# artiom-matvei/RLAO

Hardware: NVIDIA B200
Metric: closed-loop AO env-steps/sec (batched envs) (higher is better)
Workload: dtype f32

## Files before the change

### include/aoenv.h

```cpp
#ifndef AOENV_H_
#define AOENV_H_

#include <stdint.h>

#ifdef __cplusplus
extern "C" {
#endif

#define AOENV_MAX_LAYERS 8
#define AOENV_ABI_VERSION 1

int aoenv_abi_version(void);
const char* aoenv_last_error(void);
uint64_t aoenv_launch_count(void);
int aoenv_set_pdl(int enabled);


int aoenv_atm_gather(const float* win, int B, int M, int pitch, int64_t env_stride, int sx, int sy,
                     const int32_t* inner_rc, int nI, int nO, const float* xi,
                     uint64_t seed, uint64_t stream_id, float* zx, int ldz, void* zx_planes, int parts, void* stream);

int aoenv_atm_ring(float* win, int B, int M, int pitch, int64_t env_stride, int64_t win_offset, int nO, const float* X,
                   int ldx, uint64_t* ext, int32_t* flag, int force_rescan, void* stream);

int aoenv_atm_gather_multi(const void* const* wins, const int32_t* sx, const int32_t* sy, const uint64_t* seeds,
                           const uint64_t* stream_ids, int G, int B, int M, int pitch, int64_t env_stride,
                           const int32_t* inner_rc, int nI, int nO, const float* xi, float* zx, int ldz,
                           void* zx_planes, int parts, void* stream);
int aoenv_atm_ring_multi(void* const* wins, const int64_t* win_offsets, void* const* exts, int G, int B, int M,
                         int pitch, int64_t env_stride, int nO, const float* X, int ldx, int32_t* flag,
                         int force_rescan, void* stream);

int aoenv_atm_compact(const float* src_win, float* dst_win, int B, int M, int pitch, int64_t env_stride, uint64_t* ext,
                      int64_t pos_delta, void* stream);

int aoenv_vk_screens(uint64_t seed, uint32_t screen0, int S, int N, const float* amp, const float* inject, const void* wa_planes,
                     const void* wb_planes, int Kp, int parts, const float* sh_ex, const float* sh_ey, const float* h_amp,
                     const float* h_mx, const float* h_my, void* work_planes, float* work_a, int lda, float* work_b, int ldb,
                     float* dst, int pitch, int64_t env_stride, void* stream);

int aoenv_atm_phase(const float* const* h_canvas, const uint64_t* const* h_ext, const int32_t* h_org, int nLayer, int B,
                    int R, int M, int Mc, int pitch, int fp_off, const int32_t* h_row_off, const int32_t* h_col_off,
                    const float* h_wrow, const float* h_wcol, const float* h_weight, float opd_scale, float* opd_out,
                    void* stream);

typedef struct {
  double ratio[2];
  double buff[2];
  double vX, vY;
  uint64_t events;
  uint64_t philox_seed;
  int32_t not_done_once;
  int32_t cur;
  int32_t org[2];
} aoenv_layer_state_t;

typedef struct {
  int32_t nLayer, B, R, M, Mc, pitch, S, nI, nO, ldz, ldx, group_max, parts, fp_off, warp_kernel, use_tc;
  int64_t env_stride;
  uint64_t env_offset;
  double sampling_time, ps_loop;
  float opd_scale, reserved;
  float weight[AOENV_MAX_LAYERS];
  void* maps[AOENV_MAX_LAYERS][2];
  void* ext[AOENV_MAX_LAYERS];
  const void* inner_rc;
  void* zx;
  void* zx_planes;
  void* X;
  void* flag;
  const void* w_f32;
  aoenv_layer_state_t layer[AOENV_MAX_LAYERS];
} aoenv_atm_state_t;

int aoenv_atm_update(aoenv_atm_state_t* state, const void* w_planes, float* opd_out, void* stream);

#define AOENV_SKINNY_MAX_ROWS 8
int aoenv_gemm_tn(const float* X, int ldx, const float* W, int ldw, float* D, int ldd,
                  int M, int N, int K, float alpha, void* stream);

int aoenv_split_bf16(const float* src, int lds, int rows, int K, int parts, void* dst, int ldk, void* stream);
int aoenv_gemm_tn_tc(const void* Xs, const void* Ws, int ldk, int parts, float* D, int ldd, int MX, int NW, int K,
                     float alpha, void* stream);

int aoenv_dm_surface_separable(const float* coefs, int ldc, const int32_t* act_pos, int nA, int nAct, const float* gx,
                               const float* gy, const int32_t* band_x, const int32_t* band_y, const float* wx,
                               const int32_t* j0x, const float* wyp, const int32_t* i0y, int W, int B, int R, float* opd,
                               void* stream);

typedef struct {
  int32_t photon_noise;
  int32_t sensor_emccd;
  int32_t has_fwc;
  int32_t bits;
  float qe;
  float dark_electrons;
  float fwc;
  float gain;
  float readout_noise;
  uint32_t reserved;
  uint64_t seed;
  uint64_t frame_counter;
} aoenv_detector_t;

int aoenv_detector_integrate(float* frame, int B, int rows, int cols, const aoenv_detector_t* det, void* stream);

int aoenv_shwfs_camera(float* frame, const uint8_t* valid, int B, int nS, int n, const aoenv_detector_t* det, int shared_max,
                       int32_t* envmax, void* stream);

int aoenv_set_wfs6_variant(int variant);

int aoenv_shwfs_frame(const float* opd_a, const float* opd_b, const float* pupil, const float* amp,
                      const uint8_t* valid, int B, int nS, int n, float phase_scale,
                      const aoenv_detector_t* det, int shared_max,
                      float* frame, int32_t* envmax, double* stats, void* stream);

int aoenv_shwfs_slopes(const float* frame, const int32_t* envmax, int shared_max, const int32_t* valid_idx,
                       int nV, const float* ref_xy, float inv_units, float threshold_cog, int B, int nS, int n,
                       float* slopes, int lds, void* slope_planes, int parts, void* stream);

typedef struct {
  const float* rows;
  const float* wlr;
  const int32_t* ilr;
  int32_t nActP;
  int32_t WL;
  int32_t t_rows;
  int32_t reserved;
} aoenv_dm_sep_t;

int aoenv_shwfs_fused(const float* opd_a, const float* opd_b, const aoenv_dm_sep_t* dm, const uint8_t* pupil8, float amp0,
                      const int32_t* h_row_start, const int32_t* order, const int32_t* nlit, const int32_t* slot_of, int B,
                      int nS, int n, int cluster, int groups, float phase_scale, const float* ref_xy, int nV, float inv_units,
                      float threshold_cog, float* frame, float* slopes, int lds, void* slope_planes, int parts,
                      int32_t* envmax, double* stats, void* stream);
int aoenv_shwfs_frame_dm(const float* opd_a, const float* opd_b, const aoenv_dm_sep_t* dm, const int32_t* order,
                         const float* pupil, const float* amp, const uint8_t* valid, int B, int nS, int n, float phase_scale,
                         const aoenv_detector_t* det, int shared_max, float* frame, int32_t* envmax, double* stats,
                         void* stream);
int aoenv_shwfs_fused_smem(int nS, int n, int rows_max, int groups, int t_rows, int WL);
int aoenv_dm_rows(const float* coefs, int ldc, const int32_t* act_pos, int nA, int nAct, int nActP, const float* wx,
                  const int32_t* j0x, int W, int B, int R, float* rows, void* stream);

typedef struct {
  int32_t B, nS, n, nV, lds, nA, nAct, nAct2, ldc, ldr, W, rec_parts, use_tc, reserved;
  float phase_scale, inv_units, threshold_cog, leak;
  double n_pupil;
  const void *pupil, *amp, *valid, *order, *valid_idx, *ref_xy;
  void *frame, *envmax, *stats, *slopes, *slope_planes;
  aoenv_dm_sep_t dm;
  const void *rec_planes, *rec_f32;
  void* rec;
  const void* act_idx;
  void* dm_prev;
  const void *act_pos, *wx, *j0x;
} aoenv_sh_step_t;

int aoenv_sh_step(const aoenv_sh_step_t* c, int parts, const float* opd_a, const float* dm_rows_cur, const aoenv_detector_t* det,
                  const float* action, float* coefs_next, float* dm_rows_next, float* obs, float* reward, float* strehl,
                  float* total, float* residual, void* stream);

int aoenv_shwfs_measure_f64(const float* opd, const float* pupil, const float* amp, const uint8_t* valid,
                            const int32_t* valid_idx, int nV, const double* ref_xy, double inv_units, double threshold_cog,
                            int F, int nS, int n, double phase_scale, int shared_max, double* frame, uint64_t* envmax,
                            double* slopes, int lds, void* stream);

int aoenv_pyramid_supported(int N);
int aoenv_pyramid_frames(const float* opd_a, const float* opd_b, const float* pupil, const float* amp, const float* lin,
                         const float* mod, const float* mask_s, int B, int R, int N, int nTheta, int bin, float phase_scale,
                         float* work_x1, float* work_yt, float* intensity, float* frame, void* stream);


int aoenv_command_update(const float* action, const int32_t* act_idx, int B, int nA, int nAct2, float leak,
                         float* coefs, float* dm_prev, int ldc, void* stream);

int aoenv_observe(const float* rec, int ldr, const int32_t* act_idx, int B, int nA, int nAct2,
                  const double* stats, double n_pupil, float phase_scale,
                  float* obs, float* reward, float* strehl, float* total, float* residual, void* stream);

int aoenv_normal_fill(uint64_t seed, uint64_t counter, int rows, int cols, int ld, float sigma, float* out, void* planes,
                      int parts, void* stream);
int aoenv_vec_to_img(const float* vec, int ldv, const int32_t* act_idx, int B, int nA, int nAct2, float scale, float* img,
                     void* stream);

int aoenv_psf_peak(const float* opd_a, const float* opd_b, const float* pupil, const float* amp,
                   const void* w1_planes, const float* g2, int B, int R, int N, int os, int win, float phase_scale,
                   void* field_planes, int ldk, float* scratch, float* psf_win, float* psf_max, void* stream);

int aoenv_psf_image(const float* opd_a, const float* opd_b, const float* pupil, const float* amp, const void* w_planes, int B,
                    int R, int N, int os, int win, float phase_scale, void* field_planes, int ldk, float* work_t, void* planes_u,
                    float* work_f, float* psf, float* psf_max, void* stream);

#ifdef __cplusplus
}
#endif
#endif
```

### rlao_b200/Atmosphere.py

```python
import ctypes as C
import math
import os
import time

import numpy as np
import torch
from numpy.random import RandomState

from . import _lib, gemm
from .tools import vonkarman as vk


class _LayerView:

    def __init__(self, atm, index):
        self._atm, self._i = atm, index
        self._c = atm._cstate.layer[index]
        self._ratio = np.ctypeslib.as_array(self._c.ratio)
        self._buff = np.ctypeslib.as_array(self._c.buff)
        self.altitude = atm.altitude[index]
        self.windSpeed = atm._windSpeed[index]
        self.direction = atm._windDirection[index]
        self.vY = self.windSpeed * np.cos(np.deg2rad(self.direction))
        self.vX = self.windSpeed * np.sin(np.deg2rad(self.direction))
# ... 60 lines not shown

class Atmosphere:
    def __init__(self, telescope, r0, L0, windSpeed, fractionalR0, windDirection, altitude, mode=2, param=None,
                 asterism=None, rng="philox", seed=0, warp_kernel="lagrange018", env_offset=0, canvas_slack=96):
        if asterism is not None or mode != 2:
            raise NotImplementedError("asterisms / screen modes other than 2 are out of scope")
        if telescope.src is None:
            raise AttributeError("The telescope was not coupled to any source object! Make sure to couple it with an src object using src*tel")
        if rng not in ("philox", "reference"):
            raise ValueError("rng must be 'philox' or 'reference'")
        self.hasNotBeenInitialized = True
        self.telescope = telescope
        self.device = telescope.device
        self.n_envs = telescope.n_envs
        self.r0_def = 0.15
        self._r0 = r0
        self._L0 = L0
        self.fractionalR0 = list(fractionalR0)
        self.altitude = list(altitude)
        self.nLayer = len(self.fractionalR0)
        if self.nLayer > 8:
            raise ValueError("at most 8 layers (AOENV_MAX_LAYERS)")
        self._windSpeed = list(windSpeed)
        self._windDirection = list(windDirection)
        self.tag = "atmosphere"
        self.nExtra = 2
        self.wavelength = 500e-9
        self.user_defined_opd = False
        self.native_update = os.environ.get("AOENV_ATM_NATIVE", "1") != "0"
        self.pipelined = False
        self._prefetched, self._prefetch_event, self._side_stream, self._opd_next = False, None, None, None
        self.sm_partition = None
        self.mode = mode
        self.seeingArcsec = 206265 * (self.wavelength / r0)
        self.rng = rng
        self.seed = int(seed)
        self.env_offset = int(env_offset)
        self.warp_kernel = warp_kernel
        self.canvas_slack = max(1, int(canvas_slack))
        self.xi_queue = None
        self.xi_log = None
        self.screen_inject = None

    def initializeAtmosphere(self, telescope):
        tel = telescope
        self.fov, self.fov_rad = tel.fov, tel.fov_rad
        if tel.fov != 0 and any(a != 0 for a in self.altitude):
            raise NotImplementedError("fov > 0 with layers in altitude is out of scope (ground layers only)")
        dev, B, R = self.device, self.n_envs, tel.resolution
        if self.hasNotBeenInitialized:
            self.initial_r0 = self._r0
            self._ops = vk.VKOperators(R, tel.D, self._L0, self._r0, self.r0_def, dev)
            ops = self._ops
            self._M = ops.layer_res + self.nExtra
            self._S = (self.canvas_slack + 3) // 4 * 4
            self._Mc = self._M + self._S
            self._pitch = (self._Mc + 3) // 4 * 4
            self._env_stride = self._Mc * self._pitch
            self._nO, self._nI = ops.outer_rc.shape[0], ops.inner_rc.shape[0]
            self._K = (self._nI + self._nO + 15) // 16 * 16
            self._ldx = (self._nO + 3) // 4 * 4
            self._W = torch.zeros((self._nO, self._K), dtype=torch.float32, device=dev)
            self._W[:, :self._nI] = ops.A.to(torch.float32)
            self._W_op = gemm.Operator(self._W, parts=3)
            self._upload_B()
            self._inner_rc = torch.as_tensor(ops.inner_rc, dtype=torch.int32, device=dev).contiguous()
            self._maps = torch.zeros((self.nLayer, 2, B, self._Mc, self._pitch), dtype=torch.float32, device=dev)
            self._cstate = _lib.AtmState()
            self._cur = _CurView(self._cstate)
            self._org = _OrgView(self._cstate)
            self._ext = torch.zeros((self.nLayer, 3, B, 2), dtype=torch.int64, device=dev)
            G = self._group_max = min(self.nLayer, _lib.MAX_LAYERS)
            self._flag = torch.zeros((G * B,), dtype=torch.int32, device=dev)
            self._zx = torch.zeros((G * B, self._K), dtype=torch.float32, device=dev)
            self._zx_planes = torch.zeros((self._W_op.parts * G * B, self._K), dtype=torch.bfloat16, device=dev)
            self._X = torch.zeros((G * B, self._ldx), dtype=torch.float32, device=dev)
            self._opd = torch.zeros((B, R, R), dtype=torch.float32, device=dev)
            self._fp_off = 1 + (ops.layer_res // 2 - R // 2)
            self.ps_loop = ops.layer_D / ops.layer_res
            st = self._cstate
            st.nLayer, st.B, st.R, st.M, st.Mc, st.pitch, st.S = self.nLayer, B, R, self._M, self._Mc, self._pitch, self._S
            st.nI, st.nO, st.ldz, st.ldx, st.group_max, st.parts = self._nI, self._nO, self._K, self._ldx, G, self._W_op.parts
            st.fp_off, st.use_tc = self._fp_off, int(gemm.uses_tensor_cores())
            st.warp_kernel = {"lagrange018": 0, "catmull_rom": 1}.get(self.warp_kernel, -1)
            st.env_stride, st.env_offset = self._env_stride, self.env_offset
            st.sampling_time, st.ps_loop = float(tel.samplingTime), float(self.ps_loop)
            st.opd_scale = self.wavelength / 2 / math.pi
            for i in range(self.nLayer):
                st.weight[i] = math.sqrt(self.fractionalR0[i])
                st.maps[i][0], st.maps[i][1] = self._maps[i, 0].data_ptr(), self._maps[i, 1].data_ptr()
                st.ext[i] = self._ext[i].data_ptr()
            st.inner_rc, st.zx, st.zx_planes = self._inner_rc.data_ptr(), self._zx.data_ptr(), self._zx_planes.data_ptr()
            st.X, st.flag, st.w_f32 = self._X.data_ptr(), self._flag.data_ptr(), self._W.data_ptr()
            self._layers = [_LayerView(self, i) for i in range(self.nLayer)]
            for i, ly in enumerate(self._layers):
                setattr(self, "layer_" + str(i + 1), ly)
            self._new_screens(screen_seed=lambda i: i, ring_seed=lambda i: 42 + i * 1000)
        else:
            raise NotImplementedError("re-initialising an Atmosphere is not supported; build a new one")
        self.hasNotBeenInitialized = False
        self.generateNewPhaseScreen(seed=0)
        self.update()

    def _upload_B(self):
        self._W[:, self._nI:self._nI + self._nO] = self._ops.B.to(torch.float32)
        self._W_op.invalidate()

    def _host_xi(self, layer_index):
        ly = self._layers[layer_index]
        xi = np.stack([rs.normal(size=self._nO) for rs in ly.host_rng])
        return torch.as_tensor(xi, dtype=torch.float32, device=self.device)

    def _new_screens(self, screen_seed, ring_seed):
        ops, B, dev = self._ops, self.n_envs, self.device
        N, delta = ops.layer_res, ops.layer_D / ops.layer_res
        for i, ly in enumerate(self._layers):
            if self.rng == "reference":
                ph = np.stack([vk.screen_reference_rng(self._r0, self._L0, N, delta, screen_seed(i) + 104729 * (self.env_offset + e))
                               for e in range(B)])
                phase = torch.as_tensor(ph, dtype=torch.float32, device=dev)
                ly.host_rng = [RandomState(ring_seed(i) + 104729 * (self.env_offset + e)) for e in range(B)]
            else:
                phase = None
                ly.philox_seed = (self.seed * 1000003 + ring_seed(i)) & 0xFFFFFFFFFFFFFFFF
                ly.events = 0
            self._cur[i] = 0
            self._org[i] = self._fresh_origin(i)
            oy, ox = self._org[i]
            if phase is not None:
                self._maps[i, 0, :, oy + 1:oy + self._M - 1, ox + 1:ox + self._M - 1] = phase
            else:
                key = (float(self._r0), float(self._L0))
                if getattr(self, "_synth_key", None) != key:
                    self._synth, self._synth_key = vk.ScreenSynth(self._r0, self._L0, N, delta, dev), key
                sseed = (self.seed * 1000003 + screen_seed(i) * 7919 + 12345) & 0xFFFFFFFFFFFFFFFF
                dst = self._maps[i, 0].data_ptr() + 4 * ((oy + 1) * self._pitch + ox + 1)
                self._synth.generate(sseed, self.env_offset, B, dst, self._pitch, self._env_stride,
                                     inject=self.screen_inject[i] if self.screen_inject is not None else None)
            self._extrude(i, 0, 0, force_rescan=True)
            ly.notDoneOnce = True

    def _fresh_origin(self, i):
        ly, S = self._layers[i], self._S

        def pick(v, align):
            o = S if v > 0 else (0 if v < 0 else S // 2)
            return o // align * align
        return [pick(ly.vY, 1), pick(ly.vX, 4)]

    def _win_ptr(self, i, buf=None, org=None):
        buf = self._cur[i] if buf is None else buf
        oy, ox = self._org[i] if org is None else org
        return self._maps[i, buf].data_ptr() + 4 * (oy * self._pitch + ox)

    def _compact(self, i):
        oy, ox = self._org[i]
        foy, fox = self._fresh_origin(i)
        cur = self._cur[i]
        _lib.check(_lib.load().aoenv_atm_compact(self._win_ptr(i, cur, (oy, ox)), self._win_ptr(i, 1 - cur, (foy, fox)),
                                                 self.n_envs, self._M, self._pitch, self._env_stride, _lib.ptr(self._ext[i]),
                                                 (foy - oy) * self._pitch + (fox - ox), _lib.stream_ptr(self.device)),
                   "atm_compact")
        self._cur[i], self._org[i] = 1 - cur, [foy, fox]

    def _rescan_extrema(self, i):
        B, M, pitch = self.n_envs, self._M, self._pitch
        oy, ox = self._org[i]
        win = self._maps[i, self._cur[i], :, oy:oy + M, ox:ox + M]
        ring = torch.cat([win[:, 0, :], torch.stack([win[:, 1:M - 1, 0], win[:, 1:M - 1, M - 1]], dim=2).reshape(B, -1),
                          win[:, M - 1, :]], dim=1)
        self._X[:B, :self._nO] = ring
        _lib.check(_lib.load().aoenv_atm_ring(self._win_ptr(i), B, M, pitch, self._env_stride, oy * pitch + ox, self._nO,
                                              _lib.ptr(self._X), self._ldx, self._ext[i].data_ptr(), _lib.ptr(self._flag), 1,
                                              _lib.stream_ptr(self.device)), "atm_ring")

    def _extrude(self, i, sx, sy, force_rescan=False):
        self._extrude_group([(i, sx, sy)], force_rescan)

    def _extrude_group(self, group, force_rescan=False):
        lib = _lib.load()
        B, M, pitch, S, G = self.n_envs, self._M, self._pitch, self._S, len(group)
        st = _lib.stream_ptr(self.device)
        tc = gemm.uses_tensor_cores(G * B)
        xi = None
        wins, sxs, sys_, seeds, ids = [], [], [], [], []
        for i, sx, sy in group:
            ly = self._layers[i]
            sx, sy = int(sx), int(sy)
            oy, ox = self._org[i]
            if not (0 <= oy - sy <= S and 0 <= ox - sx <= S):
                self._compact(i)
                oy, ox = self._org[i]
                if not (0 <= oy - sy <= S and 0 <= ox - sx <= S):
                    raise RuntimeError("canvas_slack too small for this wind direction change")
            if self.xi_queue is not None or self.rng == "reference":
                assert G == 1, "injected innovations are consumed in the reference's order, one layer at a time"
                if self.xi_queue is not None:
                    xi = torch.as_tensor(next(self.xi_queue), dtype=torch.float32, device=self.device).reshape(B, self._nO).contiguous()
                else:
                    xi = self._host_xi(i)
            if self.xi_log is not None:
                self.xi_log.append(None if xi is None else xi.clone())
            wins.append(self._win_ptr(i))
            sxs.append(sx)
            sys_.append(sy)
            seeds.append(getattr(ly, "philox_seed", 0))
            ids.append(((ly.events << 8) | i) + (self.env_offset << 40))
            ly.events += 1
        planes = _lib.ptr(self._zx_planes) if tc else None
        zx = None if tc else _lib.ptr(self._zx)
        if G == 1:
            _lib.check(lib.aoenv_atm_gather(wins[0], B, M, pitch, self._env_stride, sxs[0], sys_[0], _lib.ptr(self._inner_rc),
                                            self._nI, self._nO, _lib.ptr(xi), C.c_uint64(seeds[0]), C.c_uint64(ids[0]),
                                            zx, self._K, planes, self._W_op.parts, st), "atm_gather")
        else:
            _lib.check(lib.aoenv_atm_gather_multi((C.c_void_p * G)(*[w.value if hasattr(w, "value") else w for w in wins]),
                                                  (C.c_int32 * G)(*sxs), (C.c_int32 * G)(*sys_), (C.c_uint64 * G)(*seeds),
                                                  (C.c_uint64 * G)(*ids), G, B, M, pitch, self._env_stride,
                                                  _lib.ptr(self._inner_rc), self._nI, self._nO, None, zx, self._K,
                                                  planes, self._W_op.parts, st), "atm_gather_multi")
        gemm.gemm_tn(self._zx, self._W_op, self._X, G * B, self._nO, backend="tc" if tc else "simt",
                     x_planes=self._zx_planes if tc else None)
        wins, offs, exts = [], [], []
        for i, sx, sy in group:
            oy, ox = self._org[i]
            self._org[i] = [oy - int(sy), ox - int(sx)]
            noy, nox = self._org[i]
            wins.append(self._win_ptr(i))
            offs.append(noy * pitch + nox)
            exts.append(self._ext[i].data_ptr())
        if G == 1:
            _lib.check(lib.aoenv_atm_ring(wins[0], B, M, pitch, self._env_stride, offs[0], self._nO, _lib.ptr(self._X), self._ldx,
                                          exts[0], _lib.ptr(self._flag), int(force_rescan), st), "atm_ring")
        else:
            _lib.check(lib.aoenv_atm_ring_multi((C.c_void_p * G)(*[w.value if hasattr(w, "value") else w for w in wins]),
                                                (C.c_int64 * G)(*offs), (C.c_void_p * G)(*exts), G, B, M, pitch, self._env_stride,
                                                self._nO, _lib.ptr(self._X), self._ldx, _lib.ptr(self._flag), int(force_rescan), st),
                       "atm_ring_multi")

    def _plan_layer(self, i):
        ly = self._layers[i]
        steps = []
        if ly.vX == 0 and ly.vY == 0:
            return steps
        if ly.notDoneOnce:
            ly.notDoneOnce = False
            ly.ratio = np.array([ly.vX * self.telescope.samplingTime / self.ps_loop,
                                 ly.vY * self.telescope.samplingTime / self.ps_loop])
            ly.buff = np.zeros(2)
        ratio = ly.ratio
        n = np.abs(ratio)
        n[np.isinf(n)] = 0
        n = n.astype(int)
        sgn = np.sign(ratio)
        for _ in range(n.min()):
            steps.append((sgn[0], sgn[1]))
        for _ in range(n.max() - n.min()):
            step = sgn.copy()
            step[n == n.min()] = 0
            steps.append((step[0], step[1]))
        ly.buff = ly.buff + (np.abs(ratio) % 1) * sgn
        if abs(ly.buff[0]) >= 1 or abs(ly.buff[1]) >= 1:
            step = np.sign(ly.buff)
            step[np.abs(ly.buff) < 1] = 0
            steps.append((step[0], step[1]))
        ly.buff = (np.abs(ly.buff) % 1) * np.sign(ly.buff)
        return steps

    def _update_layer(self, i):
        for sx, sy in self._plan_layer(i):
            self._extrude(i, sx, sy)

    def _update_layers(self):
        if self.xi_queue is not None or self.rng == "reference" or self.nLayer == 1:
            for i in range(self.nLayer):
                self._update_layer(i)
            return
        plans = [self._plan_layer(i) for i in range(self.nLayer)]
        for r in range(max((len(p_) for p_ in plans), default=0)):
            group = [(i, *plans[i][r]) for i in range(self.nLayer) if len(plans[i]) > r]
            for k in range(0, len(group), self._group_max):
                self._extrude_group(group[k:k + self._group_max])

    def _publish(self, out=None):
        out = self._opd if out is None else out
        L = self.nLayer
        maps = (C.c_void_p * L)(*[self._maps[i, self._cur[i]].data_ptr() for i in range(L)])
        exts = (C.c_void_p * L)(*[self._ext[i].data_ptr() for i in range(L)])
        org = (C.c_int32 * (2 * L))(*[v for i in range(L) for v in self._org[i]])
        roff, coff = (C.c_int32 * L)(), (C.c_int32 * L)()
        wr, wc, wt = (C.c_float * (4 * L))(), (C.c_float * (4 * L))(), (C.c_float * L)()
        for i, ly in enumerate(self._layers):
            oc, wcol = vk.cubic_tap_weights(float(ly.buff[0]), self.warp_kernel)
            orow, wrow = vk.cubic_tap_weights(float(ly.buff[1]), self.warp_kernel)
            roff[i], coff[i] = orow, oc
            for k in range(4):
                wr[4 * i + k], wc[4 * i + k] = wrow[k], wcol[k]
            wt[i] = math.sqrt(self.fractionalR0[i])
        _lib.check(_lib.load().aoenv_atm_phase(maps, exts, org, L, self.n_envs, self.telescope.resolution, self._M, self._Mc,
                                               self._pitch, self._fp_off, roff, coff, wr, wc, wt,
                                               C.c_float(self.wavelength / 2 / math.pi), _lib.ptr(out),
                                               _lib.stream_ptr(self.device)), "atm_phase")

    def _advance(self, out):
        if (self.native_update and self.rng == "philox" and self.xi_queue is None and self.xi_log is None
                and self._cstate.warp_kernel >= 0):
            tc = self._cstate.use_tc
            self._cstate.sampling_time, self._cstate.env_offset = float(self.telescope.samplingTime), self.env_offset
            _lib.check(_lib.load().aoenv_atm_update(C.byref(self._cstate), _lib.ptr(self._W_op.planes()) if tc else None,
                                                    _lib.ptr(out), _lib.stream_ptr(self.device)), "atm_update")
        else:
            self._update_layers()
            self._publish(out)

    PREFETCH_MIN_PIXELS = 1 << 25

    def can_prefetch(self):
        if self.pipelined != "force" and (not self.pipelined or self._opd is None
                                          or self._opd.numel() < self.PREFETCH_MIN_PIXELS):
            return False
        return (self.rng == "philox" and self.xi_queue is None and self.xi_log is None
                and not self.user_defined_opd and self._opd is not None and self._opd.is_cuda)

    def prefetch(self):
        if self._prefetched:
            return True
        if not self.can_prefetch():
            return False
        dev = self.device
        if self._side_stream is None:
            if self.sm_partition is not None:
                self._side_stream = self.sm_partition.side
            else:
                self._side_stream = torch.cuda.Stream(dev, priority=int(os.environ.get("AOENV_ATM_PREFETCH_PRIORITY", "0")))
            self._opd_next = torch.empty_like(self._opd)
        main, side = torch.cuda.current_stream(dev), self._side_stream
        side.wait_event(main.record_event())
        with torch.cuda.stream(side):
            self._advance(self._opd_next)
            self._prefetch_event = side.record_event()
        self._prefetched = True
        return True

    def _join_prefetch(self, consume):
        if not self._prefetched:
            return False
        torch.cuda.current_stream(self.device).wait_event(self._prefetch_event)
        self._prefetched = False
        if consume:
            self._opd, self._opd_next = self._opd_next, self._opd
        return True

    def update(self, OPD=None):
        if OPD is None:
            self.user_defined_opd = False
            if not self._join_prefetch(consume=True):
                self._advance(self._opd)
        else:
            self.user_defined_opd = True
            t = torch.as_tensor(OPD, dtype=torch.float32, device=self.device)
            self._opd = (t if t.ndim == 3 else t.unsqueeze(0).expand(self.n_envs, -1, -1)).contiguous().clone()
        if self.telescope.isPaired:
            self * self.telescope

    def generateNewPhaseScreen(self, seed=None):
        if seed is None:
            t = time.localtime()
            seed = t.tm_hour * 3600 + t.tm_min * 60 + t.tm_sec
        self._join_prefetch(consume=False)
        self._new_screens(screen_seed=lambda i: seed + i, ring_seed=lambda i: seed + i * 1000)
        for ly in self._layers:
            ly.buff = np.zeros(2)
        self._publish()
        if self.telescope.isPaired:
            self * self.telescope

    def __mul__(self, obj):
        tag = getattr(obj, "tag", None)
        if tag == "source":
            if obj.coordinates[0] > self.fov / 2:
                raise ValueError(f"The source object zenith ({obj.coordinates[0]}\") is outside of the telescope fov ({self.fov // 2}\")! "
                                 "You can:\n - Reduce the zenith of the source \n - Re-initialize the atmosphere object using a telescope "
                                 "with a larger fov")
            if obj.coordinates[0] != 0 and any(a != 0 for a in self.altitude):
                raise NotImplementedError("off-axis sources through layers in altitude (anisoplanatism) are out of scope")
            obj * self.telescope
            obj = self.telescope
        elif tag != "telescope":
            raise AttributeError("The atmosphere can be multiplied only with a Telescope or a Source object!")
        self.telescope = obj
        obj._set_lazy(self._opd, None)
        obj.isPaired = True
        return obj

    @property
    def OPD_no_pupil(self):
        return self._opd[0] if self.n_envs == 1 else self._opd

    @property
    def OPD(self):
        o = self._opd * self.telescope._pupil_f
        return o[0] if self.n_envs == 1 else o

    @property
    def r0(self):
        return self._r0

    @r0.setter
    def r0(self, val):
        self._r0 = val
        if not self.hasNotBeenInitialized:
            if self._prefetched:
                torch.cuda.current_stream(self.device).wait_event(self._prefetch_event)
            self.seeingArcsec = 206265 * (self.wavelength / val)
            self._ops.B = self._ops.innovation_factor(val)
            self._upload_B()

    @property
    def L0(self):
        return self._L0

    @L0.setter
    def L0(self, val):
        if not self.hasNotBeenInitialized and val != self._L0:
            raise NotImplementedError("changing L0 rebuilds every operator: construct a new Atmosphere")
        self._L0 = val

    def _refresh_wind(self):
        for i, ly in enumerate(self._layers):
            ly.windSpeed, ly.direction = self._windSpeed[i], self._windDirection[i]
            ly.vY = ly.windSpeed * np.cos(np.deg2rad(ly.direction))
            ly.vX = ly.windSpeed * np.sin(np.deg2rad(ly.direction))
            ly.ratio[0] = ly.vX * self.telescope.samplingTime / self.ps_loop
            ly.ratio[1] = ly.vY * self.telescope.samplingTime / self.ps_loop

    @property
    def windSpeed(self):
        return self._windSpeed

    @windSpeed.setter
    def windSpeed(self, val):
        if not self.hasNotBeenInitialized and len(val) != self.nLayer:
            print("Error! Wrong value for the wind-speed! Make sure that you inpute a wind-speed for each layer")
            return
        self._windSpeed = list(val)
        if not self.hasNotBeenInitialized:
            self._refresh_wind()

    @property
    def windDirection(self):
        return self._windDirection

    @windDirection.setter
    def windDirection(self, val):
        if not self.hasNotBeenInitialized and len(val) != self.nLayer:
            print("Error! Wrong value for the wind-speed! Make sure that you inpute a wind-speed for each layer")
            return
        self._windDirection = list(val)
        if not self.hasNotBeenInitialized:
            self._refresh_wind()
```

### rlao_b200/OOPAOEnv/OOPAOEnvRazor.py

```python
import contextlib
import ctypes
import importlib
import math
import os
import types

import numpy as np
import torch

from .. import _lib, gemm
from ..Atmosphere import Atmosphere
from ..DeformableMirror import DeformableMirror, DMSurfaceRef
from ..MisRegistration import MisRegistration
from ..ShackHartmann import ShackHartmann
from ..Source import Source
from ..Telescope import Telescope
from ..Zernike import Zernike
from ..calibration.CalibrationVault import CalibrationVault
from ..calibration.InteractionMatrix import InteractionMatrix
from ..tools import linalg


_NVTX = os.environ.get("AOENV_NVTX", "0") not in ("", "0")


@contextlib.contextmanager
def _range(name):
    if _NVTX:
        torch.cuda.nvtx.range_push(name)
        try:
            yield
        finally:
            torch.cuda.nvtx.range_pop()
    else:
        yield


class OOPAO:
    metadata = {"render.modes": ["rgb_array"]}

    def __init__(self):
        self.gainCL = None
        self.atm = self.wfs = self.dm = self.misReg = self.tel = self.source = None
        self.M2C_CL = self.calib_CL = self.reconstructor = None
        self.SR = self.total = self.residual = self.wfsSignal = self.OPD = None
        self.action_buffer = []
        self.done = False
        self.param_file = ""
        self.oopao_path = ""
        self.delay = 1
        self.F = 1
        self.name = "OOPAO"
        self.dm_mask = self.nActuator = self.xvalid = self.yvalid = None
        self.leak = 0.99
        self.n_envs = 1
        self.device = None
        self.psf_reward = None
        self.native_step = os.environ.get("AOENV_STEP_NATIVE", "1") != "0"
        self.prefetch_early = os.environ.get("AOENV_PREFETCH_EARLY", "1") != "0"
        self._native_key, self._native = None, None

    def set_params_file(self, param_file, oopao_path):
        self.param_file = param_file
        self.oopao_path = oopao_path

    def _load_param(self, args):
        if isinstance(self.param_file, dict):
            return dict(self.param_file)
        name = self.param_file or "rlao_b200.Conf.parameter_file_synthetic_SHWFS"
        try:
            config = importlib.import_module(name)
        except ModuleNotFoundError:
            config = importlib.import_module("rlao_b200." + name)
        return config.initializeParameterFile(args)

    def set_params(self, args=None, wfs_type="shackhartmann", modal_basis="zernike", gainCL=0.5, n_envs=1, device=None,
                   rng="philox", seed=0, env_offset=0, warp_kernel="lagrange018", canvas_slack=96):
        if wfs_type not in ("shackhartmann", "pyramid"):
            raise NotImplementedError(f"wfs_type {wfs_type!r}: only 'shackhartmann' and 'pyramid' are implemented")
        self.wfs_type = wfs_type
        args = args if args is not None else types.SimpleNamespace()
        self.gainCL = gainCL
        self.n_envs = int(n_envs)
        self.env_offset = int(env_offset)
        param = self._load_param(args)
        self.param = param
        self.tel = Telescope(resolution=param["resolution"], diameter=param["diameter"], samplingTime=param["samplingTime"],
                             centralObstruction=param["centralObstruction"], fov=param.get("fov", 0), n_envs=n_envs,
                             device=device)
        self.device = self.tel.device
        self.source = Source(optBand=param["opticalBand"], magnitude=param["magnitude"])
        self.source * self.tel
        self.atm = Atmosphere(telescope=self.tel, r0=param["r0"], L0=param["L0"], windSpeed=param["windSpeed"],
                              fractionalR0=param["fractionalR0"], windDirection=param["windDirection"],
                              altitude=param["altitude"], rng=rng, seed=seed, env_offset=env_offset,
                              warp_kernel=warp_kernel, canvas_slack=canvas_slack)
        self.atm.initializeAtmosphere(self.tel)
        self.atm.update()
        self.tel + self.atm
        nAct = param["nActuator"]
        self.nActuator = nAct
        if param.get("dm_geometry", "razor") == "cartesian":
            self.dm = DeformableMirror(telescope=self.tel, nSubap=param["nSubaperture"], mechCoupling=param["mechanicalCoupling"],
                                       misReg=MisRegistration(param))
            self.dm_mask = np.reshape(self.dm.validAct, (nAct, nAct)).astype(int)
        else:
            x = np.linspace(-self.tel.D / 2, self.tel.D / 2, nAct)
            X, Y = np.meshgrid(x, x)
            keep = np.asarray(param["boolActMask"]).astype(bool).reshape(-1)
            coords = np.stack([X.reshape(-1)[keep], Y.reshape(-1)[keep]], axis=1)
            self.dm = DeformableMirror(telescope=self.tel, nSubap=nAct, mechCoupling=param["mechanicalCoupling"],
                                       M4_param=param, coordinates=coords)
            self.dm_mask = np.asarray(param["boolActMask"]).astype(int)
        self.xvalid, self.yvalid = np.nonzero(self.dm_mask)
        self.tel - self.atm
        if wfs_type == "pyramid":
            from ..Pyramid import Pyramid
            self.wfs = Pyramid(nSubap=param["nSubaperture"], telescope=self.tel, lightRatio=param.get("lightThreshold", 0.1),
                               modulation=param.get("modulation", 3), binning=1,
                               n_pix_separation=param.get("n_pix_separation", 4), n_pix_edge=2,
                               postProcessing=param.get("postProcessing", "slopesMaps"))
        else:
            self.wfs = ShackHartmann(telescope=self.tel, nSubap=param["nSubaperture"], lightRatio=param.get("lightRatio", 0.5),
                                     threshold_cog=param.get("threshold_cog", 0.01), is_geometric=False,
                                     shannon_sampling=param.get("shannon_sampling", True))
        cam = self.wfs.cam
        cam.sensor = param.get("cam_sensor", cam.sensor)
        cam.FWC = param.get("cam_FWC", cam.FWC)
        cam.bits = param.get("cam_bits", cam.bits)
        cam.QE = param.get("cam_QE", cam.QE)
        cam.darkCurrent = param.get("cam_darkCurrent", cam.darkCurrent)
        cam.integrationTime = param["samplingTime"]
        cam.seed = seed
        self.wfs.env_offset = self.env_offset
        pf = os.environ.get("AOENV_ATM_PREFETCH", "1")
        self.atm.pipelined = "force" if pf == "force" else pf != "0"
        if wfs_type != "pyramid" and getattr(self.wfs, "inline_dm", False) and self.dm.fused_tables() is not None \
                and self.wfs._dm_windows(self.dm.fused_tables()) is not None:
            self.dm.lazy_surface = True
        self.tel * self.wfs
        nZ = param.get("nZernike", 50)
        if nZ and nZ > 0:
            Z = Zernike(self.tel, nZ)
            Z.computeZernike(self.tel)
            M2C = linalg.pinv(self.dm.modes[self.tel._pupil_idx, :].double()) @ Z.modes
        else:
            M2C = torch.eye(self.dm.nValidAct, dtype=torch.float64, device=self.device)
        calib_zonal = InteractionMatrix(ngs=self.source, atm=self.atm, tel=self.tel, dm=self.dm, wfs=self.wfs,
                                        M2C=torch.eye(self.dm.nValidAct, dtype=torch.float64, device=self.device),
                                        stroke=1e-9, nMeasurements=param.get("nMeasurements", 25), noise="off")
        self.calib_zonal = calib_zonal
        calib = CalibrationVault(calib_zonal.D @ M2C)
        self.tel.resetOPD()
        self.dm.coefs = 0
        self._dm_prev = torch.zeros((self.n_envs, self.dm._Kp), dtype=torch.float32, device=self.device)
        self._coefs_buf = torch.zeros((2, self.n_envs, self.dm._Kp), dtype=torch.float32, device=self.device)
        self._coefs_slot = 0
        self.source * self.tel * self.dm * self.wfs
        self.tel + self.atm
        self.calib_CL = calib
        self.M2C_CL = M2C
        nLoop = param.get("nLoop", None)
        self.SR = []
        self._nLoop = nLoop
        self.total = torch.zeros((nLoop, self.n_envs), dtype=torch.float32, device=self.device) if nLoop else None
        self.residual = torch.zeros((nLoop, self.n_envs), dtype=torch.float32, device=self.device) if nLoop else None
        cam.photonNoise = param.get("cam_photonNoise", True)
        cam.readoutNoise = param.get("cam_readoutNoise", 14 if wfs_type == "shackhartmann" else 0)
        self.set_reconstructor(M2C @ calib.M)
        self.F = M2C @ linalg.pinv(M2C)
        nA_, Kp_ = self.dm.nValidAct, self.dm._Kp
        self._F32 = torch.zeros((nA_, Kp_), dtype=torch.float32, device=self.device)
        self._F32[:, :nA_] = self.F.to(torch.float32)
        self._F_op = gemm.Operator(self._F32, parts=2)
        self.dm.free_float64()
        B, nA = self.n_envs, self.dm.nValidAct
        self._act_idx = torch.as_tensor((self.xvalid * nAct + self.yvalid).astype(np.int32), device=self.device)
        self._rec = torch.zeros((B, (nA + 3) // 4 * 4), dtype=torch.float32, device=self.device)
        self._obs = torch.zeros((B, nAct, nAct), dtype=torch.float32, device=self.device)
        self._reward = torch.zeros((B,), dtype=torch.float32, device=self.device)
        self._strehl = torch.zeros((B,), dtype=torch.float32, device=self.device)
        self._total_now = torch.zeros((B,), dtype=torch.float32, device=self.device)
        self._residual_now = torch.zeros((B,), dtype=torch.float32, device=self.device)
        self._phase_scale = 2 * math.pi / self.source.wavelength
        self._noise_seed = (seed * 7919 + 5) & 0xFFFFFFFFFFFFFFFF
        self._noise_calls = 0
        self._noise_z = torch.zeros((B, self.dm._Kp), dtype=torch.float32, device=self.device)
        self._noise_planes = torch.zeros((2, B, self.dm._Kp), dtype=torch.bfloat16, device=self.device)
        self._noise_vec = torch.zeros((B, (nA + 3) // 4 * 4), dtype=torch.float32, device=self.device)

    def set_reconstructor(self, R):
        self.reconstructor = torch.as_tensor(R, dtype=torch.float64, device=self.device)
        nA, nSig = self.reconstructor.shape
        self._Rm = torch.zeros((nA, self.wfs._lds), dtype=torch.float32, device=self.device)
        self._Rm[:, :nSig] = self.reconstructor.to(torch.float32)
        self._Rm_op = gemm.Operator(self._Rm, parts=2)

    @property
    def dm_prev(self):
        d = self._dm_prev[:, :self.dm.nValidAct]
        return d[0] if self.n_envs == 1 else d

    @dm_prev.setter
    def dm_prev(self, val):
        t = torch.as_tensor(val, dtype=torch.float32, device=self.device)
        self._dm_prev.zero_()
        self._dm_prev[:, :self.dm.nValidAct] = t

    def _sq(self, t):
        return t[0] if self.n_envs == 1 else t

    def _observe(self, with_stats):
        lib, st, B, nA = _lib.load(), _lib.stream_ptr(self.device), self.n_envs, self.dm.nValidAct
        sig = self.wfs._signal
        gemm.gemm_tn(sig, self._Rm_op, self._rec, B, nA,
                     x_planes=self.wfs._signal_planes if gemm.uses_tensor_cores(B) else None)
        _lib.check(lib.aoenv_observe(_lib.ptr(self._rec), self._rec.stride(0), _lib.ptr(self._act_idx), B, nA,
                                     self.nActuator ** 2, _lib.ptr(self.wfs._stats) if with_stats else None,
                                     float(self.tel.pixelArea), self._phase_scale, _lib.ptr(self._obs), _lib.ptr(self._reward),
                                     _lib.ptr(self._strehl), _lib.ptr(self._total_now), _lib.ptr(self._residual_now), st),
                   "observe")

    def _action_tensor(self, action):
        a = torch.as_tensor(action, dtype=torch.float32, device=self.device)
        nAct = self.nActuator
        if a.ndim == 2:
            a = a.unsqueeze(0).expand(self.n_envs, -1, -1)
        return a.reshape(self.n_envs, nAct * nAct).contiguous()

    def reset_soft(self):
        self.action_buffer = []
        self._observe(False)
        return self._sq(self._obs).clone()

    def reset(self):
        raise NotImplementedError("reset() rebuilds the whole simulation in the reference (set_params without arguments, "
                                  "OOPAOEnvRazor.py:66-71, which raises there too); use set_params(...) then reset_soft()")

    def reset_soft_wfs(self):
        self.action_buffer = []
        return self.wfs.cam.frame.clone()

    def _native_cfg(self):
        wfs, dm, tel = self.wfs, self.dm, self.tel
        if (not self.native_step or _NVTX or self.psf_reward is not None or type(wfs) is not ShackHartmann or wfs.use_fused
                or not wfs.inline_dm or not dm.lazy_surface or self.atm.user_defined_opd or dm._multi is not None
                or dm._coefs_matrix is not None):
            return None
        src = tel.src
        if wfs._flux_version != getattr(src, "_flux_version", 0) or wfs.current_nPhoton != src.nPhoton:
            return None
        key = (wfs._flux_version, id(wfs._amp), id(wfs._ref_xy), wfs.slopes_units, wfs.threshold_cog, float(self.leak),
               id(self._Rm_op), id(dm._sep), src.wavelength, id(self._coefs_buf))
        if self._native_key == key:
            return self._native
        self._native_key, self._native = key, None
        tables = dm.fused_tables()
        win = wfs._dm_windows(tables) if tables is not None else None
        if win is None or 2 * math.pi / src.wavelength != self._phase_scale:
            return None
        tc = gemm.uses_tensor_cores(self.n_envs)
        dm._rows_of(dm._slot)
        c = _lib.ShStepStruct()
        c.B, c.nS, c.n, c.nV, c.lds = self.n_envs, wfs.nSubap, wfs.n_pix_subap, wfs.nValidSubaperture, wfs._signal.stride(0)
        c.nA, c.nAct, c.nAct2 = dm.nValidAct, dm.nAct, self.nActuator ** 2
        c.ldc, c.ldr, c.W, c.rec_parts, c.use_tc = self._coefs_buf.stride(1), self._rec.stride(0), tables["W"], self._Rm_op.parts, int(tc)
        c.phase_scale, c.inv_units, c.threshold_cog, c.leak = self._phase_scale, 1.0 / wfs.slopes_units, wfs.threshold_cog, self.leak
        c.n_pupil = float(tel.pixelArea)
        keep = [tel._pupil_f, wfs._amp, wfs._valid_u8, wfs._lit_first, wfs._valid_idx, wfs._ref_xy, wfs._frame, wfs._envmax,
                wfs._stats, wfs._signal, wfs._signal_planes, win, self._Rm, self._Rm_op, self._rec, self._act_idx, self._dm_prev,
                tables]
        c.pupil, c.amp, c.valid, c.order = tel._pupil_f.data_ptr(), wfs._amp.data_ptr(), wfs._valid_u8.data_ptr(), wfs._lit_first.data_ptr()
        c.valid_idx, c.ref_xy, c.frame, c.envmax = wfs._valid_idx.data_ptr(), wfs._ref_xy.data_ptr(), wfs._frame.data_ptr(), wfs._envmax.data_ptr()
        c.stats, c.slopes, c.slope_planes = wfs._stats.data_ptr(), wfs._signal.data_ptr(), wfs._signal_planes.data_ptr()
        c.dm.wlr, c.dm.ilr, c.dm.nActP, c.dm.WL = win[2].data_ptr(), win[1].data_ptr(), dm._rows.shape[2], win[0]
        c.rec_planes = self._Rm_op.planes().data_ptr() if tc else None
        c.rec_f32, c.rec, c.act_idx, c.dm_prev = self._Rm.data_ptr(), self._rec.data_ptr(), self._act_idx.data_ptr(), self._dm_prev.data_ptr()
        c.act_pos, c.wx, c.j0x = tables["act_pos"].data_ptr(), tables["wx"].data_ptr(), tables["j0x"].data_ptr()
        self._native = (c, keep)
        return self._native

    def _step_native(self, i, action, native, action_ready=None, after_observe=None):
        c = native[0]
        dm, wfs, atm, B, dev = self.dm, self.wfs, self.atm, self.n_envs, self.device
        slot = dm._slot
        atm.update()
        self.tel._set_lazy(atm._opd, DMSurfaceRef(dm, slot))
        det = wfs.cam.as_struct(self.env_offset)
        nAct = self.nActuator
        obs = torch.empty((B, nAct, nAct), dtype=torch.float32, device=dev)
        reward = torch.empty((B,), dtype=torch.float32, device=dev)
        strehl = torch.empty((B,), dtype=torch.float32, device=dev)
        coefs = self._coefs_buf[self._coefs_slot]
        args = [atm._opd.data_ptr(), dm._rows[slot].data_ptr(), ctypes.byref(det) if det is not None else None, None,
                coefs.data_ptr(), dm._rows[slot ^ 1].data_ptr(), obs.data_ptr(), reward.data_ptr(), strehl.data_ptr(),
                self._total_now.data_ptr(), self._residual_now.data_ptr(), _lib.stream_ptr(dev)]
        step, cref = _lib.load().aoenv_sh_step, ctypes.byref(c)
        if atm.can_prefetch() or after_observe is not None or action_ready is not None:
            early = atm.sm_partition is not None or (self.prefetch_early and after_observe is None and action_ready is None)
            if early:
                atm.prefetch()
            _lib.check(step(cref, 1, *args), "sh_step")
            if not early:
                atm.prefetch()
            _lib.check(step(cref, 2, *args), "sh_step")
            if after_observe is not None:
                after_observe(self._sq(obs), self._sq(reward), self._sq(strehl))
            if action_ready is not None:
                torch.cuda.current_stream(dev).wait_event(action_ready)
            args[3] = self._action_tensor(action).data_ptr()
            _lib.check(step(cref, 4, *args), "sh_step")
        else:
            act = self._action_tensor(action)
            args[3] = act.data_ptr()
            _lib.check(step(cref, 7, *args), "sh_step")
        self._coefs_slot ^= 1
        dm._coefs, dm._multi, dm._coefs_matrix, dm._slot = coefs, None, None, slot ^ 1
        dm._coefs_of[slot ^ 1], dm._rows_valid[slot ^ 1], dm._valid[slot ^ 1] = coefs, True, False
        wfs.cam.frame = wfs._frame[0] if B == 1 else wfs._frame
        wfs._signal_is_multi = False
        self._obs, self._reward, self._strehl = obs, reward, strehl
        if self.total is not None and i is not None and 0 <= i < self._nLoop:
            self.total[i] = self._total_now
            self.residual[i] = self._residual_now
        s = self._sq(strehl)
        self.SR.append(s)
        self.wfsSignal = wfs.signal
        return self._sq(obs), self._sq(reward), s, False, {"strehl": s}

    def step(self, i, action):
        native = self._native_cfg()
        if native is not None and self.dm._rows_valid[self.dm._slot]:
            return self._step_native(i, action, native)
        obs, reward, strehl, done, info = self._measure_frame(i)
        self._apply_command(action)
        strehl = strehl.clone()
        self.SR[-1] = strehl
        return obs.clone(), reward.clone(), strehl, done, {"strehl": strehl}

    def _step_views(self, i, action, action_ready=None, after_observe=None):
        native = self._native_cfg()
        if native is not None and self.dm._rows_valid[self.dm._slot]:
            return self._step_native(i, action, native, action_ready, after_observe)
        out = self._measure_frame(i, after_observe)
        self._apply_command(action, action_ready)
        return out

    def _measure_frame(self, i, after_observe=None, atmosphere_done=False):
        if not atmosphere_done:
            with _range("aoenv.atmosphere"):
                self.atm.update()
        else:
            self.atm._join_prefetch(consume=True)
        dm_surface = self.dm.surface_ref()
        self.tel._set_lazy(self.atm._opd, dm_surface)
        with _range("aoenv.wfs"):
            self.wfs._measure_terms(self.atm._opd, dm_surface, self.env_offset)
        if not atmosphere_done:
            with _range("aoenv.atmosphere_next"):
                self.atm.prefetch()
        with _range("aoenv.reconstruct"):
            self._observe(True)
        if self.total is not None and i is not None and 0 <= i < self._nLoop:
            self.total[i] = self._total_now
            self.residual[i] = self._residual_now
        strehl = self._sq(self._strehl)
        if self.psf_reward is not None:
            strehl = self.psf_strehl(*self.psf_reward)
        if after_observe is not None:
            after_observe(self._sq(self._obs), self._sq(self._reward), strehl)
        self.SR.append(strehl if self.psf_reward is not None else strehl.clone())
        self.wfsSignal = self.wfs.signal
        return self._sq(self._obs), self._sq(self._reward), strehl, False, {"strehl": strehl}

    def _apply_command(self, action, action_ready=None):
        lib, st, B = _lib.load(), _lib.stream_ptr(self.device), self.n_envs
        if action_ready is not None:
            torch.cuda.current_stream(self.device).wait_event(action_ready)
        action = self._action_tensor(action)
        coefs = self._coefs_buf[self._coefs_slot]
        self._coefs_slot ^= 1
        with _range("aoenv.command"):
            _lib.check(lib.aoenv_command_update(_lib.ptr(action), _lib.ptr(self._act_idx), B, self.dm.nValidAct,
                                                self.nActuator ** 2, ctypes.c_float(self.leak), _lib.ptr(coefs), _lib.ptr(self._dm_prev),
                                                coefs.stride(0), st), "command_update")
            self.dm._set_coefs_batch(coefs)

    def state_dict(self):
        atm = self.atm
        nxt = None
        if atm._prefetched:
            torch.cuda.current_stream(self.device).wait_event(atm._prefetch_event)
            nxt = atm._opd_next.detach().cpu().clone()
        layers = []
        for i, ly in enumerate(atm._layers):
            layers.append(dict(map=ly.mapShift.detach().cpu().clone(), buff=ly.buff.copy(), ratio=ly.ratio.copy(),
                               notDoneOnce=ly.notDoneOnce, events=ly.events, philox_seed=getattr(ly, "philox_seed", 0),
                               ext=None))
        return dict(version=1, n_envs=self.n_envs, rng=atm.rng, layers=layers, atm_opd=atm._opd.detach().cpu().clone(),
                    atm_opd_next=nxt,
                    coefs=self.dm._coefs.detach().cpu().clone(), dm_prev=self._dm_prev.detach().cpu().clone(),
                    cam_frame_counter=self.wfs.cam.frame_counter, noise_calls=self._noise_calls,
                    SR=[s.detach().cpu().clone() for s in self.SR],
                    total=None if self.total is None else self.total.detach().cpu().clone(),
                    residual=None if self.residual is None else self.residual.detach().cpu().clone())

    def load_state_dict(self, st):
        if st.get("version") != 1 or st["n_envs"] != self.n_envs or st["rng"] != self.atm.rng:
            raise ValueError("state_dict of another environment (n_envs / rng / version differ)")
        if self.atm.rng != "philox":
            raise NotImplementedError("host MT19937 streams (rng='reference') are not checkpointed; use rng='philox'")
        atm, dev = self.atm, self.device
        atm._join_prefetch(consume=False)
        for i, (ly, s_) in enumerate(zip(atm._layers, st["layers"])):
            atm._cur[i] = 0
            atm._org[i] = atm._fresh_origin(i)
            oy, ox = atm._org[i]
            m = s_["map"].to(dev)
            atm._maps[i, 0, :, oy:oy + atm._M, ox:ox + atm._M] = m if m.ndim == 3 else m.unsqueeze(0)
            ly.buff, ly.ratio, ly.notDoneOnce = s_["buff"].copy(), s_["ratio"].copy(), s_["notDoneOnce"]
            ly.events, ly.philox_seed = s_["events"], s_["philox_seed"]
            atm._rescan_extrema(i)
        atm._opd.copy_(st["atm_opd"].to(dev))
        if st.get("atm_opd_next") is not None:
            if atm._opd_next is None:
                atm._opd_next = torch.empty_like(atm._opd)
                atm._side_stream = torch.cuda.Stream(dev)
            atm._opd_next.copy_(st["atm_opd_next"].to(dev))
            atm._prefetched, atm._prefetch_event = True, torch.cuda.current_stream(dev).record_event()
        coefs = st["coefs"].to(dev)
        self._dm_prev.copy_(st["dm_prev"].to(dev))
        self._coefs_buf[self._coefs_slot].copy_(coefs)
        self.dm._set_coefs_batch(self._coefs_buf[self._coefs_slot])
        self._coefs_slot ^= 1
        self.wfs.cam.frame_counter, self._noise_calls = st["cam_frame_counter"], st["noise_calls"]
        self.SR = [s.to(dev) for s in st["SR"]]
        if st["total"] is not None and self.total is not None:
            self.total.copy_(st["total"].to(dev))
            self.residual.copy_(st["residual"].to(dev))
        self.tel._set_lazy(atm._opd, self.dm.surface_ref())

    def step_wfs(self, i, action):
        self._measure_frame(i)
        frame = self.wfs.cam.frame.clone()
        leak, self.leak = self.leak, 1.0
        try:
            self._apply_command(torch.as_tensor(action, dtype=torch.float32, device=self.device) * 1e6)
        finally:
            self.leak = leak
        strehl = self.SR[-1]
        reward = self._sq(-torch.linalg.vector_norm(frame.reshape(self.n_envs, -1).float(), dim=1))
        return frame, reward, strehl, False, {"strehl": strehl}

    def _get_reward(self, slopes=None, type="volt"):
        if getattr(self, "S2V", None) is not None and type != "sh":
            v = torch.as_tensor(slopes, dtype=torch.float64, device=self.device) @ torch.as_tensor(self.S2V, dtype=torch.float64, device=self.device).T
            return -torch.linalg.vector_norm(v, dim=-1)
        return self.get_strehl()

    def compute_dm_proj(self):
        modes = self.dm.modes.double()
        self.dm_proj = torch.linalg.solve(modes.T @ modes, modes.T)
        return self.dm_proj

    def OPD_on_dm(self):
        if getattr(self, "dm_proj", None) is None:
            self.compute_dm_proj()
        res = self.tel.resolution
        opd = (self.tel._materialise() * self.tel._pupil_f).double().reshape(self.n_envs, res * res)
        out = ((opd @ self.dm_proj.T) @ self.dm.modes.double().T).reshape(self.n_envs, res, res)
        return self._sq(out)

    def set_modalBasis(self, mode="zernike"):
        if mode != "zernike":
            raise NotImplementedError("only the Zernike basis is built by the reference (OOPAOEnvRazor.py:394)")
        paired = self.tel.isPaired
        self.tel - self.atm
        Z = Zernike(self.tel, 50)
        Z.computeZernike(self.tel)
        M2C = linalg.pinv(self.dm.modes[self.tel._pupil_idx, :].double()) @ Z.modes
        eye = torch.eye(self.dm.nValidAct, dtype=torch.float64, device=self.device)
        self.imat = InteractionMatrix(ngs=self.source, atm=self.atm, tel=self.tel, dm=self.dm, wfs=self.wfs, M2C=eye,
                                      stroke=1e-9, nMeasurements=25, noise="off")
        self.calib_CL = CalibrationVault(self.imat.D @ M2C)
        self.M2C_CL = M2C
        self.tel.resetOPD()
        self.dm.coefs = 0
        self.source * self.tel * self.dm * self.wfs
        if paired:
            self.tel + self.atm

    def set_wfs(self, param, type="pyramid"):
        self.tel - self.atm
        if type == "pyramid":
            from ..Pyramid import Pyramid
            if param.get("psfCentering", True) is not True:
                raise NotImplementedError("Pyramid(psfCentering=False) is out of scope")
            self.wfs = Pyramid(nSubap=param["nSubaperture"], telescope=self.tel, modulation=param["modulation"],
                               lightRatio=param["lightThreshold"], n_pix_separation=param["n_pix_separation"],
                               postProcessing=param["postProcessing"])
        elif type == "shackhartmann":
            self.wfs = ShackHartmann(telescope=self.tel, nSubap=param["nSubaperture"], lightRatio=param.get("lightRatio", 0.5),
                                     threshold_cog=param.get("threshold_cog", 0.01), is_geometric=False,
                                     shannon_sampling=param.get("shannon_sampling", True))
        else:
            raise NotImplementedError(f"wfs type {type!r}")
        self.wfs_type = type
        self.tel * self.wfs

    def calculate_strehl_AVG(self):
        if len(self.SR) == 0:
            return float("nan")
        s = torch.stack([x.reshape(-1) for x in self.SR]).double()
        tot = torch.stack([s.sum(), torch.tensor(float(s.numel()), dtype=torch.float64, device=s.device)])
        import torch.distributed as dist
        if dist.is_available() and dist.is_initialized():
            dist.all_reduce(tot)
        self.SR = []
        return float(tot[0] / tot[1])

    def integrator(self):
        return -self.gainCL * self.vec_to_img(self.wfs.signal.double() @ self.reconstructor.T)

    def get_slopes(self):
        return self.wfs.signal

    def get_strehl(self):
        ph = self.tel._materialise() * self.tel._pupil_f * self._phase_scale
        v = ph.reshape(ph.shape[0], -1)[:, self.tel._pupil_idx].double().var(dim=1, unbiased=False)
        return self._sq(torch.exp(-v).float())

    def sample_noise(self, sigma, use_torch=True):
        lib, st, B, nA = _lib.load(), _lib.stream_ptr(self.device), self.n_envs, self.dm.nValidAct
        tc = gemm.uses_tensor_cores(B)
        _lib.check(lib.aoenv_normal_fill(ctypes.c_uint64(self._noise_seed + (self.env_offset << 20)), ctypes.c_uint64(self._noise_calls),
                                         B, nA, self.dm._Kp, ctypes.c_float(float(sigma)), _lib.ptr(self._noise_z),
                                         _lib.ptr(self._noise_planes) if tc else None, 2, st), "normal_fill")
        self._noise_calls += 1
        gemm.gemm_tn(self._noise_z, self._F_op, self._noise_vec, B, nA, x_planes=self._noise_planes if tc else None)
        img = torch.empty((B, self.nActuator, self.nActuator), dtype=torch.float32, device=self.device)
        _lib.check(lib.aoenv_vec_to_img(_lib.ptr(self._noise_vec), self._noise_vec.stride(0), _lib.ptr(self._act_idx), B, nA,
                                        self.nActuator ** 2, ctypes.c_float(1.0), _lib.ptr(img), st), "vec_to_img")
        return self._sq(img)

    def vec_to_img(self, action_vec, use_torch=True):
        v = torch.as_tensor(action_vec, device=self.device)
        lead = v.shape[:-1]
        img = torch.zeros(lead + (self.nActuator, self.nActuator), dtype=v.dtype, device=self.device)
        img[..., torch.as_tensor(self.xvalid, device=self.device), torch.as_tensor(self.yvalid, device=self.device)] = v
        return img

    def img_to_vec(self, action):
        a = torch.as_tensor(action, device=self.device)
        return a[..., torch.as_tensor(self.xvalid, device=self.device), torch.as_tensor(self.yvalid, device=self.device)]

    def change_mag(self, mag):
        self.source.nPhoton = self.source.zeroPoint * 10 ** (-0.4 * mag)
        self.source.magnitude = mag
        self.source * self.tel * self.wfs

    def psf_strehl(self, zeroPaddingFactor=4, window=32):
        from ..psf import psf_peak
        if not hasattr(self, "_psf_model_max") or self._psf_model_key != (zeroPaddingFactor, window):
            zero = torch.zeros((1, self.tel.resolution, self.tel.resolution), dtype=torch.float32, device=self.device)
            self._psf_model_max = psf_peak(self.tel, zero, None, zeroPaddingFactor, window)[0]
            self._psf_model_key = (zeroPaddingFactor, window)
        a, b = self.tel._terms()
        return self._sq(psf_peak(self.tel, a, b, zeroPaddingFactor, window) / self._psf_model_max)
```

### rlao_b200/_lib.py

```python
import ctypes as C
import os

import torch

_HERE = os.path.dirname(os.path.abspath(__file__))
LIB_PATH = os.path.join(_HERE, "libaoenv_b200.so")


class AOEnvLibraryError(RuntimeError):
    pass


class DetectorStruct(C.Structure):
    _fields_ = [
        ("photon_noise", C.c_int32), ("sensor_emccd", C.c_int32), ("has_fwc", C.c_int32), ("bits", C.c_int32),
        ("qe", C.c_float), ("dark_electrons", C.c_float), ("fwc", C.c_float), ("gain", C.c_float),
        ("readout_noise", C.c_float), ("reserved", C.c_uint32), ("seed", C.c_uint64), ("frame_counter", C.c_uint64),
    ]


class DmSepStruct(C.Structure):
    _fields_ = [
        ("rows", C.c_void_p), ("wlr", C.c_void_p), ("ilr", C.c_void_p),
        ("nActP", C.c_int32), ("WL", C.c_int32), ("t_rows", C.c_int32), ("reserved", C.c_int32),
    ]


MAX_LAYERS = 8


class LayerState(C.Structure):
    _fields_ = [
        ("ratio", C.c_double * 2), ("buff", C.c_double * 2), ("vX", C.c_double), ("vY", C.c_double),
        ("events", C.c_uint64), ("philox_seed", C.c_uint64),
        ("not_done_once", C.c_int32), ("cur", C.c_int32), ("org", C.c_int32 * 2),
    ]


class ShStepStruct(C.Structure):
    _fields_ = [(k, C.c_int32) for k in ("B", "nS", "n", "nV", "lds", "nA", "nAct", "nAct2", "ldc", "ldr", "W", "rec_parts",
                                         "use_tc", "reserved")] + [
        ("phase_scale", C.c_float), ("inv_units", C.c_float), ("threshold_cog", C.c_float), ("leak", C.c_float),
        ("n_pupil", C.c_double)] + [(k, C.c_void_p) for k in ("pupil", "amp", "valid", "order", "valid_idx", "ref_xy", "frame",
                                                              "envmax", "stats", "slopes", "slope_planes")] + [
        ("dm", DmSepStruct)] + [(k, C.c_void_p) for k in ("rec_planes", "rec_f32", "rec", "act_idx", "dm_prev", "act_pos",
                                                           "wx", "j0x")]


class AtmState(C.Structure):
    _fields_ = [(k, C.c_int32) for k in ("nLayer", "B", "R", "M", "Mc", "pitch", "S", "nI", "nO", "ldz", "ldx", "group_max",
                                         "parts", "fp_off", "warp_kernel", "use_tc")] + [
        ("env_stride", C.c_int64), ("env_offset", C.c_uint64), ("sampling_time", C.c_double), ("ps_loop", C.c_double),
        ("opd_scale", C.c_float), ("reserved", C.c_float), ("weight", C.c_float * MAX_LAYERS),
        ("maps", (C.c_void_p * 2) * MAX_LAYERS), ("ext", C.c_void_p * MAX_LAYERS), ("inner_rc", C.c_void_p),
        ("zx", C.c_void_p), ("zx_planes", C.c_void_p), ("X", C.c_void_p), ("flag", C.c_void_p), ("w_f32", C.c_void_p),
        ("layer", LayerState * MAX_LAYERS),
    ]

_vp, _i, _f, _u64, _d, _i64 = C.c_void_p, C.c_int, C.c_float, C.c_uint64, C.c_double, C.c_int64

PROTOTYPES = {
    "aoenv_atm_gather": [_vp, _i, _i, _i, _i64, _i, _i, _vp, _i, _i, _vp, _u64, _u64, _vp, _i, _vp, _i, _vp],
    "aoenv_atm_ring": [_vp, _i, _i, _i, _i64, _i64, _i, _vp, _i, _vp, _vp, _i, _vp],
    "aoenv_atm_gather_multi": [_vp, _vp, _vp, _vp, _vp, _i, _i, _i, _i, _i64, _vp, _i, _i, _vp, _vp, _i, _vp, _i, _vp],
    "aoenv_atm_ring_multi": [_vp, _vp, _vp, _i, _i, _i, _i, _i64, _i, _vp, _i, _vp, _i, _vp],
    "aoenv_atm_compact": [_vp, _vp, _i, _i, _i, _i64, _vp, _i64, _vp],
    "aoenv_vk_screens": [_u64, C.c_uint32, _i, _i, _vp, _vp, _vp, _vp, _i, _i, _vp, _vp, _vp, _vp, _vp, _vp, _vp, _i, _vp, _i,
                         _vp, _i, _i64, _vp],
    "aoenv_atm_update": [_vp, _vp, _vp, _vp],
    "aoenv_sh_step": [_vp, _i] + [_vp] * 12,
    "aoenv_atm_phase": [_vp, _vp, _vp, _i, _i, _i, _i, _i, _i, _i, _vp, _vp, _vp, _vp, _vp, _f, _vp, _vp],
    "aoenv_gemm_tn": [_vp, _i, _vp, _i, _vp, _i, _i, _i, _i, _f, _vp],
    "aoenv_split_bf16": [_vp, _i, _i, _i, _i, _vp, _i, _vp],
    "aoenv_gemm_tn_tc": [_vp, _vp, _i, _i, _vp, _i, _i, _i, _i, _f, _vp],
    "aoenv_dm_surface_separable": [_vp, _i, _vp, _i, _i, _vp, _vp, _vp, _vp, _vp, _vp, _vp, _vp, _i, _i, _i, _vp, _vp],
    "aoenv_set_wfs6_variant": [_i],
    "aoenv_detector_integrate": [_vp, _i, _i, _i, _vp, _vp],
    "aoenv_shwfs_camera": [_vp, _vp, _i, _i, _i, _vp, _i, _vp, _vp],
    "aoenv_shwfs_frame": [_vp, _vp, _vp, _vp, _vp, _i, _i, _i, _f, _vp, _i, _vp, _vp, _vp, _vp],
    "aoenv_shwfs_frame_dm": [_vp, _vp, _vp, _vp, _vp, _vp, _vp, _i, _i, _i, _f, _vp, _i, _vp, _vp, _vp, _vp],
    "aoenv_shwfs_slopes": [_vp, _vp, _i, _vp, _i, _vp, _f, _f, _i, _i, _i, _vp, _i, _vp, _i, _vp],
    "aoenv_shwfs_fused": [_vp, _vp, _vp, _vp, _f, _vp, _vp, _vp, _vp, _i, _i, _i, _i, _i, _f, _vp, _i, _f, _f, _vp, _vp, _i, _vp, _i,
                          _vp, _vp, _vp],
    "aoenv_shwfs_fused_smem": [_i, _i, _i, _i, _i, _i],
    "aoenv_dm_rows": [_vp, _i, _vp, _i, _i, _i, _vp, _vp, _i, _i, _i, _vp, _vp],
    "aoenv_shwfs_measure_f64": [_vp, _vp, _vp, _vp, _vp, _i, _vp, _d, _d, _i, _i, _i, _d, _i, _vp, _vp, _vp, _i, _vp],
    "aoenv_normal_fill": [_u64, _u64, _i, _i, _i, _f, _vp, _vp, _i, _vp],
    "aoenv_vec_to_img": [_vp, _i, _vp, _i, _i, _i, _f, _vp, _vp],
    "aoenv_pyramid_supported": [_i],
    "aoenv_pyramid_frames": [_vp, _vp, _vp, _vp, _vp, _vp, _vp, _i, _i, _i, _i, _i, _f, _vp, _vp, _vp, _vp, _vp],
    "aoenv_command_update": [_vp, _vp, _i, _i, _i, _f, _vp, _vp, _i, _vp],
    "aoenv_observe": [_vp, _i, _vp, _i, _i, _i, _vp, _d, _f, _vp, _vp, _vp, _vp, _vp, _vp],
    "aoenv_psf_image": [_vp, _vp, _vp, _vp, _vp, _i, _i, _i, _i, _i, _f, _vp, _i, _vp, _vp, _vp, _vp, _vp, _vp],
    "aoenv_psf_peak": [_vp, _vp, _vp, _vp, _vp, _vp, _i, _i, _i, _i, _i, _f, _vp, _i, _vp, _vp, _vp, _vp],
}

_lib = None


def load():
    global _lib
    if _lib is not None:
        return _lib
    if not os.path.exists(LIB_PATH):
        raise AOEnvLibraryError(
            f"{LIB_PATH} not found: the CUDA extension has not been built. Build it with "
            "`bash rlao_b200/csrc/build.sh` (needs nvcc with sm_100a support). rlao_b200 has no CPU fallback.")
    lib = C.CDLL(LIB_PATH)
    lib.aoenv_abi_version.restype = C.c_int
    lib.aoenv_last_error.restype = C.c_char_p
    lib.aoenv_launch_count.restype = C.c_uint64
    lib.aoenv_set_pdl.argtypes, lib.aoenv_set_pdl.restype = [C.c_int], C.c_int
    for name, args in PROTOTYPES.items():
        fn = getattr(lib, name)
        fn.argtypes = args
        fn.restype = C.c_int
    _lib = lib
    return lib


def check(rc, what=""):
    if rc != 0:
        raise RuntimeError(f"libaoenv_b200 {what} failed ({rc}): {load().aoenv_last_error().decode()}")


def ptr(t):
    return None if t is None else t.data_ptr()


_raw_stream = getattr(torch._C, "_cuda_getCurrentRawStream", None)


def stream_ptr(device=None):
    if _raw_stream is not None:
        if device is None:
            idx = torch.cuda.current_device()
        else:
            idx = device.index if isinstance(device, torch.device) else torch.device(device).index
            if idx is None:
                idx = torch.cuda.current_device()
        return _raw_stream(idx)
    return torch.cuda.current_stream(device).cuda_stream


def launch_count():
    return int(load().aoenv_launch_count())


def require_cuda(device):
    if not torch.cuda.is_available():
        raise AOEnvLibraryError("rlao_b200 needs a CUDA device (B200, sm_100a); there is no CPU fallback")
    dev = torch.device(device if device is not None else "cuda:0")
    if dev.type != "cuda":
        raise AOEnvLibraryError(f"rlao_b200 objects live on CUDA devices, got {dev}")
    return dev
```

### rlao_b200/csrc/atm.cu

```cuda
#include "common.cuh"
#include "tma.cuh"

namespace aoenv {

struct AtmGroup {
  float* win[AOENV_MAX_LAYERS];
  unsigned long long* ext[AOENV_MAX_LAYERS];
  unsigned long long seed[AOENV_MAX_LAYERS], stream_id[AOENV_MAX_LAYERS];
  uint32_t win_offset[AOENV_MAX_LAYERS];
  int sx[AOENV_MAX_LAYERS], sy[AOENV_MAX_LAYERS];
};

__global__ void __launch_bounds__(256)
atm_gather_kernel(const __grid_constant__ AtmGroup grp, int M, int pitch, size_t env_stride,
                  const int2* __restrict__ inner_rc, int nI, int nO, const float* __restrict__ xi,
                  float* __restrict__ zx, int ldz, __nv_bfloat16* __restrict__ planes, int parts) {
  pdl_enter();
  const int b = blockIdx.y, g = blockIdx.z;
  const int k = blockIdx.x * blockDim.x + threadIdx.x;
  if (k >= ldz) return;
  const size_t row = (size_t)g * gridDim.y + b;
  float v = 0.f;
  if (k < nI) {
    const int2 rc = __ldg(&inner_rc[k]);
    const float* __restrict__ map = grp.win[g];
    v = __ldg(&map[(size_t)b * env_stride + (size_t)(rc.x - grp.sy[g]) * pitch + (rc.y - grp.sx[g])]);
  } else if (k < nI + nO) {
    const int j = k - nI;
    if (xi != nullptr) {
      v = __ldg(&xi[row * nO + j]);
    } else {
      const unsigned long long stream_id = grp.stream_id[g];
      Philox rng(grp.seed[g]);
      const uint4 r = rng((uint32_t)j, (uint32_t)b, (uint32_t)stream_id, (uint32_t)(stream_id >> 32));
      v = box_muller(r.x, r.y).x;
    }
  }
  if (zx != nullptr) zx[row * ldz + k] = v;
  if (planes != nullptr) store_bf16_planes(planes, (size_t)gridDim.z * gridDim.y * ldz, row * ldz + k, parts, v);
}

__device__ __forceinline__ uint32_t key_of(float f) { return (uint32_t)float_to_ordered(f) ^ 0x80000000u; }
__device__ __forceinline__ float value_of(unsigned long long packed) {
  return ordered_to_float((int32_t)((uint32_t)(packed >> 32) ^ 0x80000000u));
}
__device__ __forceinline__ unsigned long long pack(float f, uint32_t pos) { return ((unsigned long long)key_of(f) << 32) | pos; }

__device__ __forceinline__ void block_reduce_ext(unsigned long long& lo, unsigned long long& hi) {
  __shared__ unsigned long long s_lo[32], s_hi[32];
#pragma unroll
  for (int o = 16; o > 0; o >>= 1) {
    const unsigned long long l2 = __shfl_xor_sync(0xffffffffu, lo, o), h2 = __shfl_xor_sync(0xffffffffu, hi, o);
    lo = l2 < lo ? l2 : lo;
    hi = h2 > hi ? h2 : hi;
  }
  const int w = threadIdx.x >> 5, l = threadIdx.x & 31;
  if (l == 0) { s_lo[w] = lo; s_hi[w] = hi; }
  __syncthreads();
  if (w == 0) {
    const int nw = (blockDim.x + 31) >> 5;
    lo = l < nw ? s_lo[l] : ~0ull;
    hi = l < nw ? s_hi[l] : 0ull;
#pragma unroll
    for (int o = 16; o > 0; o >>= 1) {
      const unsigned long long l2 = __shfl_xor_sync(0xffffffffu, lo, o), h2 = __shfl_xor_sync(0xffffffffu, hi, o);
      lo = l2 < lo ? l2 : lo;
      hi = h2 > hi ? h2 : hi;
    }
  }
}

__global__ void __launch_bounds__(256)
atm_ring_kernel(const __grid_constant__ AtmGroup grp, int M, int pitch, size_t env_stride,
                const float* __restrict__ X, int ldx, int32_t* __restrict__ flag, int force_rescan) {
  pdl_enter();
  const int b = blockIdx.x, g = blockIdx.y;
  const size_t row = (size_t)g * gridDim.x + b;
  const uint32_t win_offset = grp.win_offset[g];
  unsigned long long* __restrict__ ext = grp.ext[g];
  float* __restrict__ w = grp.win[g] + (size_t)b * env_stride;
  const float* __restrict__ xb = X + row * ldx;
  const int nO = 4 * M - 4;
  unsigned long long* __restrict__ ext_prev = ext + 4 * (size_t)gridDim.x + 2 * b;
  const unsigned long long prev = *ext_prev;
  const int oy = win_offset / pitch, ox = win_offset % pitch;
  int line_r[2], line_c[2], nr = 0, nc = 0;
  {
    const int py = (int)((uint32_t)prev / (uint32_t)pitch), px = (int)((uint32_t)prev % (uint32_t)pitch);
    const int dy = oy - py, dx = ox - px;
    if ((prev >> 32) != 1ull || force_rescan || dy < -1 || dy > 1 || dx < -1 || dx > 1) {
      line_r[0] = 1; line_r[1] = M - 2; nr = 2;
      line_c[0] = 1; line_c[1] = M - 2; nc = 2;
    } else {
      if (dy != 0) line_r[nr++] = dy < 0 ? 1 : M - 2;
      if (dx != 0) line_c[nc++] = dx < 0 ? 1 : M - 2;
    }
  }
  const int nE = (nr + nc) * (M - 2);
  constexpr int kEdge = 8;
  float ev[kEdge];
  uint32_t erel[kEdge];
#pragma unroll
  for (int i = 0; i < kEdge; ++i) {
    const int k = threadIdx.x + i * 256;
    erel[i] = 0;
    ev[i] = 0.f;
    if (k < nE) {
      const int side = k / (M - 2), t = 1 + k % (M - 2);
      const int r = side < nr ? line_r[side] : t, c = side < nr ? t : line_c[side - nr];
      erel[i] = (uint32_t)(r * pitch + c);
      ev[i] = w[erel[i]];
    }
  }
  unsigned long long lo = ~0ull, hi = 0ull;
  for (int k = threadIdx.x; k < nO; k += blockDim.x) {
    int r, c;
    if (k < M) { r = 0; c = k; }
    else if (k >= M + 2 * (M - 2)) { r = M - 1; c = k - (M + 2 * (M - 2)); }
    else { const int t = k - M; r = 1 + (t >> 1); c = (t & 1) ? M - 1 : 0; }
    const float v = __ldg(&xb[k]);
    const uint32_t rel = (uint32_t)(r * pitch + c);
    w[rel] = v;
    const unsigned long long pk = pack(v, win_offset + rel);
    lo = pk < lo ? pk : lo;
    hi = pk > hi ? pk : hi;
  }
  unsigned long long ilo = ~0ull, ihi = 0ull;
#pragma unroll
  for (int i = 0; i < kEdge; ++i) {
    if (threadIdx.x + i * 256 < nE) {
      const unsigned long long pk = pack(ev[i], win_offset + erel[i]);
      ilo = pk < ilo ? pk : ilo;
      ihi = pk > ihi ? pk : ihi;
    }
  }
  for (int k = threadIdx.x + kEdge * 256; k < nE; k += 256) {
    const int side = k / (M - 2), t = 1 + k % (M - 2);
    const int r = side < nr ? line_r[side] : t, c = side < nr ? t : line_c[side - nr];
    const uint32_t rel = (uint32_t)(r * pitch + c);
    const unsigned long long pk = pack(w[rel], win_offset + rel);
    ilo = pk < ilo ? pk : ilo;
    ihi = pk > ihi ? pk : ihi;
  }
  block_reduce_ext(lo, hi);
  __syncthreads();
  block_reduce_ext(ilo, ihi);
  if (threadIdx.x == 0) {
    unsigned long long* __restrict__ ext_in = ext + 2 * (size_t)gridDim.x;
    const unsigned long long old_lo = ext_in[2 * b], old_hi = ext_in[2 * b + 1];
    *ext_prev = (1ull << 32) | win_offset;
    auto retained = [&](unsigned long long pk) {
      const uint32_t pos = (uint32_t)pk;
      const int r = (int)(pos / pitch) - oy, c = (int)(pos % pitch) - ox;
      return r >= 1 && r <= M - 2 && c >= 1 && c <= M - 2;
    };
    const bool ok = !force_rescan && retained(old_lo) && retained(old_hi);
    if (ok) {
      ilo = old_lo < ilo ? old_lo : ilo;
      ihi = old_hi > ihi ? old_hi : ihi;
    }
    ext_in[2 * b] = ilo;
    ext_in[2 * b + 1] = ihi;
    ext[2 * b] = ilo < lo ? ilo : lo;
    ext[2 * b + 1] = ihi > hi ? ihi : hi;
    flag[row] = ok ? 0 : 1;
  }
}

__global__ void __launch_bounds__(256)
atm_rescan_kernel(const __grid_constant__ AtmGroup grp, int M, int pitch, size_t env_stride,
                  const int32_t* __restrict__ flag, int rows_per_block) {
  pdl_enter();
  const int b = blockIdx.y, g = blockIdx.z;
  if (__ldg(&flag[(size_t)g * gridDim.y + b]) == 0) return;
  const uint32_t win_offset = grp.win_offset[g];
  unsigned long long* __restrict__ ext = grp.ext[g];
  const float* __restrict__ w = grp.win[g] + (size_t)b * env_stride;
  const int r_begin = 1 + blockIdx.x * rows_per_block;
  const int r_end = min(M - 1, r_begin + rows_per_block);
  const int mis = (int)((reinterpret_cast<uintptr_t>(w) >> 2) & 3);
  const int nvec = (M - 1 + mis + 3) >> 2;
  const int tx = threadIdx.x & 63, ty = threadIdx.x >> 6;
  float vlo = INFINITY, vhi = -INFINITY;
  uint32_t plo = 0, phi = 0;
  constexpr int kRows = 4;
  for (int r0 = r_begin + ty * kRows; r0 < r_end; r0 += 4 * kRows) {
    for (int v4 = tx; v4 < nvec; v4 += 64) {
      const int c0 = 4 * v4 - mis;
      float4 q[kRows];
#pragma unroll
      for (int i = 0; i < kRows; ++i)
        q[i] = (r0 + i < r_end) ? __ldg(reinterpret_cast<const float4*>(w + (size_t)(r0 + i) * pitch + c0)) : make_float4(0.f, 0.f, 0.f, 0.f);
#pragma unroll
      for (int i = 0; i < kRows; ++i) {
        if (r0 + i >= r_end) break;
        const uint32_t base = (uint32_t)((r0 + i) * pitch + c0);
        const float e[4] = {q[i].x, q[i].y, q[i].z, q[i].w};
#pragma unroll
        for (int k = 0; k < 4; ++k) {
          const int c = c0 + k;
          if (c >= 1 && c < M - 1) {
            if (e[k] < vlo) { vlo = e[k]; plo = base + k; }
            if (e[k] > vhi) { vhi = e[k]; phi = base + k; }
          }
        }
      }
    }
  }
  unsigned long long lo = vlo < INFINITY ? pack(vlo, win_offset + plo) : ~0ull;
  unsigned long long hi = vhi > -INFINITY ? pack(vhi, win_offset + phi) : 0ull;
  block_reduce_ext(lo, hi);
  if (threadIdx.x == 0 && r_begin < r_end) {
    unsigned long long* __restrict__ ext_in = ext + 2 * (size_t)gridDim.y;
    atomicMin(&ext_in[2 * b], lo);
    atomicMax(&ext_in[2 * b + 1], hi);
    atomicMin(&ext[2 * b], lo);
    atomicMax(&ext[2 * b + 1], hi);
  }
}

__global__ void __launch_bounds__(256)
atm_compact_kernel(const float* __restrict__ src, float* __restrict__ dst, int M, int pitch, size_t env_stride,
                   unsigned long long* __restrict__ ext, int pos_delta, int rows_per_block) {
  pdl_enter();
  const int b = blockIdx.y;
  const float* __restrict__ s = src + (size_t)b * env_stride;
  float* __restrict__ d = dst + (size_t)b * env_stride;
  const int r_begin = blockIdx.x * rows_per_block;
  const int r_end = min(M, r_begin + rows_per_block);
  const int nvec = (M + 3) >> 2;
  const int tx = threadIdx.x & 63, ty = threadIdx.x >> 6;
  for (int r = r_begin + ty; r < r_end; r += 4) {
    const float* __restrict__ sr = s + (size_t)r * pitch;
    float* __restrict__ dr = d + (size_t)r * pitch;
    for (int v4 = tx; v4 < nvec; v4 += 64) {
      const int c = v4 << 2;
      if (c + 3 < M) {
        *reinterpret_cast<float4*>(dr + c) = make_float4(__ldg(sr + c), __ldg(sr + c + 1), __ldg(sr + c + 2), __ldg(sr + c + 3));
      } else {
        for (int k = 0; c + k < M; ++k) dr[c + k] = __ldg(sr + c + k);
      }
    }
  }
  if (blockIdx.x == 0 && threadIdx.x < 5) {
    const size_t i = (size_t)(threadIdx.x >> 1) * 2 * gridDim.y + 2 * b + (threadIdx.x & 1);
    const unsigned long long e = ext[i];
    ext[i] = (e & 0xffffffff00000000ull) | (uint32_t)((int)(uint32_t)e + pos_delta);
  }
}

struct AtmPhaseParams {
  CUtensorMap map[AOENV_MAX_LAYERS];
  const unsigned long long* ext[AOENV_MAX_LAYERS];
  int row0[AOENV_MAX_LAYERS];
  int col0[AOENV_MAX_LAYERS];
  float wrow[AOENV_MAX_LAYERS][4];
  float wcol[AOENV_MAX_LAYERS][4];
  float weight[AOENV_MAX_LAYERS];
  int nLayer;
};

constexpr int kPhTileW = 128, kPhTileH = 32, kPhThreadsX = 32, kPhThreadsY = 4, kPhRows = 8;
constexpr int kPhBoxW = kPhTileW + 8, kPhBoxH = kPhTileH + 3;
constexpr uint32_t kPhBoxBytes = kPhBoxW * kPhBoxH * sizeof(float);
constexpr int kPhBufFloats = (kPhBoxW * kPhBoxH + 31) / 32 * 32;

__device__ __forceinline__ const CUtensorMap* layer_map(const AtmPhaseParams& p, int l) {
  switch (l) {
    case 0: return &p.map[0];
    case 1: return &p.map[1];
    case 2: return &p.map[2];
    case 3: return &p.map[3];
    case 4: return &p.map[4];
    case 5: return &p.map[5];
    case 6: return &p.map[6];
    default: return &p.map[7];
  }
}

template <int MIS>
__device__ __forceinline__ void phase_rows(const float* __restrict__ tbase, float wc0, float wc1, float wc2, float wc3,
                                           float (&h)[kPhRows + 3][4]) {
#pragma unroll
  for (int t = 0; t < kPhRows + 3; ++t) {
    const float* __restrict__ trow = tbase + t * kPhBoxW;
    const float4 a = *reinterpret_cast<const float4*>(trow);
    const float4 b = *reinterpret_cast<const float4*>(trow + 4);
    const float4 c = *reinterpret_cast<const float4*>(trow + 8);
    const float v[12] = {a.x, a.y, a.z, a.w, b.x, b.y, b.z, b.w, c.x, c.y, c.z, c.w};
#pragma unroll
    for (int k = 0; k < 4; ++k)
      h[t][k] = wc0 * v[MIS + k] + wc1 * v[MIS + k + 1] + wc2 * v[MIS + k + 2] + wc3 * v[MIS + k + 3];
  }
}

__global__ void __launch_bounds__(kPhThreadsX * kPhThreadsY)
atm_phase_kernel(const __grid_constant__ AtmPhaseParams p, int R, float opd_scale, float* __restrict__ opd_out) {
  pdl_enter();
  __shared__ __align__(128) float tile[2][kPhBufFloats];
  __shared__ __align__(8) uint64_t bar[2];
  const int b = blockIdx.z;
  const int j0 = blockIdx.x * kPhTileW, i0 = blockIdx.y * kPhTileH;
  const int tx = threadIdx.x, ty = threadIdx.y;
  const bool leader = (tx == 0 && ty == 0);
  if (leader) {
    tma::mbar_init(&bar[0], 1);
    tma::mbar_init(&bar[1], 1);
    tma::mbar_fence_init();
  }
  __syncthreads();
  if (leader) {
    tma::mbar_expect_tx(&bar[0], kPhBoxBytes);
    tma::load_3d(layer_map(p, 0), &bar[0], &tile[0][0], (p.col0[0] + j0) & ~3, p.row0[0] + i0, b);
  }
  float acc[kPhRows][4];
#pragma unroll
  for (int r = 0; r < kPhRows; ++r)
#pragma unroll
    for (int c = 0; c < 4; ++c) acc[r][c] = 0.f;

  for (int l = 0; l < p.nLayer; ++l) {
    const int buf = l & 1;
    if (leader && l + 1 < p.nLayer) {
      tma::mbar_expect_tx(&bar[buf ^ 1], kPhBoxBytes);
      tma::load_3d(layer_map(p, l + 1), &bar[buf ^ 1], &tile[buf ^ 1][0], (p.col0[l + 1] + j0) & ~3, p.row0[l + 1] + i0, b);
    }
    const float lo = value_of(__ldg(&p.ext[l][2 * b + 0]));
    const float hi = value_of(__ldg(&p.ext[l][2 * b + 1]));
    const float wc0 = p.wcol[l][0], wc1 = p.wcol[l][1], wc2 = p.wcol[l][2], wc3 = p.wcol[l][3];
    const float wr0 = p.wrow[l][0], wr1 = p.wrow[l][1], wr2 = p.wrow[l][2], wr3 = p.wrow[l][3];
    const float w = p.weight[l];
    tma::mbar_wait(&bar[buf], (l >> 1) & 1);
    float h[kPhRows + 3][4];
    const float* __restrict__ tbase = &tile[buf][(ty * kPhRows) * kPhBoxW + tx * 4];
    switch ((p.col0[l] + j0) & 3) {
      case 0: phase_rows<0>(tbase, wc0, wc1, wc2, wc3, h); break;
      case 1: phase_rows<1>(tbase, wc0, wc1, wc2, wc3, h); break;
      case 2: phase_rows<2>(tbase, wc0, wc1, wc2, wc3, h); break;
      default: phase_rows<3>(tbase, wc0, wc1, wc2, wc3, h); break;
    }
#pragma unroll
    for (int t = 0; t < kPhRows; ++t)
#pragma unroll
      for (int c = 0; c < 4; ++c) {
        float v = wr0 * h[t][c] + wr1 * h[t + 1][c] + wr2 * h[t + 2][c] + wr3 * h[t + 3][c];
        v = fminf(fmaxf(v, lo), hi);
        acc[t][c] += w * v;
      }
    __syncthreads();
  }
  float* __restrict__ out = opd_out + (size_t)b * R * R;
  const int jc = j0 + tx * 4;
#pragma unroll
  for (int t = 0; t < kPhRows; ++t) {
    const int i = i0 + ty * kPhRows + t;
    if (i >= R || jc >= R) continue;
    float* __restrict__ o = out + (size_t)i * R + jc;
    if (jc + 3 < R && ((R & 3) == 0)) {
      *reinterpret_cast<float4*>(o) = make_float4(acc[t][0] * opd_scale, acc[t][1] * opd_scale, acc[t][2] * opd_scale, acc[t][3] * opd_scale);
    } else {
#pragma unroll
      for (int c = 0; c < 4; ++c)
        if (jc + c < R) o[c] = acc[t][c] * opd_scale;
    }
  }
}

}

using namespace aoenv;

static int rows_per_block_for(int B, int M) {
  int chunks = (4 * kNumSMs + B - 1) / B;
  if (chunks < 1) chunks = 1;
  if (chunks > M) chunks = M;
  return (M + chunks - 1) / chunks;
}

extern "C" {

int aoenv_atm_gather_multi(const void* const* wins, const int32_t* sx, const int32_t* sy, const uint64_t* seeds,
                           const uint64_t* stream_ids, int G, int B, int M, int pitch, int64_t env_stride,
                           const int32_t* inner_rc, int nI, int nO, const float* xi, float* zx, int ldz, void* zx_planes,
                           int parts, void* stream) {
  AOENV_CHECK_ARG(G > 0 && G <= AOENV_MAX_LAYERS, "atm_gather: %d layers in one group (max %d)", G, AOENV_MAX_LAYERS);
  AOENV_CHECK_ARG(B > 0 && B <= 65535 && M > 6 && pitch >= M && env_stride >= (int64_t)M * pitch, "atm_gather: bad shape B=%d M=%d pitch=%d", B, M, pitch);
  AOENV_CHECK_ARG(ldz >= nI + nO, "atm_gather: ldz=%d < nI+nO=%d", ldz, nI + nO);
  AOENV_CHECK_ARG(zx_planes == nullptr || parts == 2 || parts == 3, "atm_gather: parts must be 2 or 3");
  AOENV_CHECK_ARG(zx != nullptr || zx_planes != nullptr, "atm_gather: neither zx nor zx_planes given");
  AtmGroup grp{};
  for (int g = 0; g < G; ++g) {
    AOENV_CHECK_ARG(sx[g] >= -1 && sx[g] <= 1 && sy[g] >= -1 && sy[g] <= 1, "atm_gather: shift must be in {-1,0,1}");
    grp.win[g] = (float*)wins[g];
    grp.sx[g] = sx[g];
    grp.sy[g] = sy[g];
    grp.seed[g] = seeds ? seeds[g] : 0;
    grp.stream_id[g] = stream_ids ? stream_ids[g] : 0;
  }
  dim3 grid((ldz + 255) / 256, B, G);
  AOENV_LAUNCH(atm_gather_kernel, grid, 256, 0, (cudaStream_t)stream, grp, M, pitch, (size_t)env_stride, (const int2*)inner_rc, nI, nO,
                                                            xi, zx, ldz, (__nv_bfloat16*)zx_planes, parts);
  AOENV_LAUNCH_CHECK("atm_gather");
  return 0;
}

int aoenv_atm_gather(const float* win, int B, int M, int pitch, int64_t env_stride, int sx, int sy,
                     const int32_t* inner_rc, int nI, int nO, const float* xi, uint64_t seed, uint64_t stream_id,
                     float* zx, int ldz, void* zx_planes, int parts, void* stream) {
  const void* wins[1] = {win};
  const int32_t sxs[1] = {sx}, sys[1] = {sy};
  const uint64_t seeds[1] = {seed}, ids[1] = {stream_id};
  return aoenv_atm_gather_multi(wins, sxs, sys, seeds, ids, 1, B, M, pitch, env_stride, inner_rc, nI, nO, xi, zx, ldz,
                                zx_planes, parts, stream);
}

int aoenv_atm_ring_multi(void* const* wins, const int64_t* win_offsets, void* const* exts, int G, int B, int M, int pitch,
                         int64_t env_stride, int nO, const float* X, int ldx, int32_t* flag, int force_rescan, void* stream) {
  AOENV_CHECK_ARG(G > 0 && G <= AOENV_MAX_LAYERS, "atm_ring: %d layers in one group (max %d)", G, AOENV_MAX_LAYERS);
  AOENV_CHECK_ARG(B > 0 && B <= 65535 && M > 6 && pitch >= M && pitch % 4 == 0 && env_stride % 4 == 0,
                  "atm_ring: bad shape (pitch and env_stride must be multiples of 4 floats)");
  AOENV_CHECK_ARG(nO == 4 * M - 4 && ldx >= nO, "atm_ring: ring has %d pixels, got nO=%d ldx=%d", 4 * M - 4, nO, ldx);
  AtmGroup grp{};
  for (int g = 0; g < G; ++g) {
    AOENV_CHECK_ARG(win_offsets[g] >= 0 && win_offsets[g] + (int64_t)M * pitch <= env_stride + pitch && env_stride < (1ll << 32),
                    "atm_ring: window leaves the canvas");
    grp.win[g] = (float*)wins[g];
    grp.ext[g] = (unsigned long long*)exts[g];
    grp.win_offset[g] = (uint32_t)win_offsets[g];
  }
  cudaStream_t s = (cudaStream_t)stream;
  AOENV_LAUNCH(atm_ring_kernel, dim3(B, G), 256, 0, s, grp, M, pitch, (size_t)env_stride, X, ldx, flag, force_rescan);
  AOENV_LAUNCH_CHECK("atm_ring");
  const int rpb = 32;
  dim3 grid((M - 2 + rpb - 1) / rpb, B, G);
  AOENV_LAUNCH(atm_rescan_kernel, grid, 256, 0, s, grp, M, pitch, (size_t)env_stride, flag, rpb);
  AOENV_LAUNCH_CHECK("atm_rescan");
  return 0;
}

int aoenv_atm_ring(float* win, int B, int M, int pitch, int64_t env_stride, int64_t win_offset, int nO, const float* X,
                   int ldx, uint64_t* ext, int32_t* flag, int force_rescan, void* stream) {
  void* wins[1] = {win};
  void* exts[1] = {ext};
  const int64_t offs[1] = {win_offset};
  return aoenv_atm_ring_multi(wins, offs, exts, 1, B, M, pitch, env_stride, nO, X, ldx, flag, force_rescan, stream);
}

int aoenv_atm_compact(const float* src_win, float* dst_win, int B, int M, int pitch, int64_t env_stride, uint64_t* ext,
                      int64_t pos_delta, void* stream) {
  AOENV_CHECK_ARG(B > 0 && B <= 65535 && M > 6 && pitch >= M && pitch % 4 == 0, "atm_compact: bad shape");
  AOENV_CHECK_ARG((reinterpret_cast<uintptr_t>(dst_win) & 15) == 0, "atm_compact: destination window must be 16-byte aligned");
  const int rpb = rows_per_block_for(B, M);
  dim3 grid((M + rpb - 1) / rpb, B);
  AOENV_LAUNCH(atm_compact_kernel, grid, 256, 0, (cudaStream_t)stream, src_win, dst_win, M, pitch, (size_t)env_stride,
                                                             reinterpret_cast<unsigned long long*>(ext), (int)pos_delta, rpb);
  AOENV_LAUNCH_CHECK("atm_compact");
  return 0;
}

int aoenv_atm_phase(const float* const* h_canvas, const uint64_t* const* h_ext, const int32_t* h_org, int nLayer, int B,
                    int R, int M, int Mc, int pitch, int fp_off, const int32_t* h_row_off, const int32_t* h_col_off,
                    const float* h_wrow, const float* h_wcol, const float* h_weight, float opd_scale, float* opd_out,
                    void* stream) {
  AOENV_CHECK_ARG(nLayer >= 1 && nLayer <= AOENV_MAX_LAYERS, "atm_phase: nLayer=%d out of range", nLayer);
  AOENV_CHECK_ARG(B > 0 && B <= 65535, "atm_phase: B=%d out of range (1..65535)", B);
  AOENV_CHECK_ARG(pitch % 4 == 0 && pitch >= Mc && Mc >= M, "atm_phase: bad canvas Mc=%d pitch=%d", Mc, pitch);
  tma::EncodeTiledFn enc = tma::get_encode();
  if (!enc) return fail(-4, "cuTensorMapEncodeTiled is not available from the CUDA driver");
  AtmPhaseParams p;
  p.nLayer = nLayer;
  for (int l = 0; l < nLayer; ++l) {
    const int oy = h_org[2 * l], ox = h_org[2 * l + 1];
    AOENV_CHECK_ARG(oy >= 0 && ox >= 0 && oy + M <= Mc && ox + M <= pitch, "atm_phase: window of layer %d leaves the canvas", l);
    const int lo_r = fp_off + h_row_off[l], hi_r = fp_off + R - 1 + h_row_off[l] + 3;
    const int lo_c = fp_off + h_col_off[l], hi_c = fp_off + R - 1 + h_col_off[l] + 3;
    AOENV_CHECK_ARG(lo_r >= 0 && lo_c >= 0 && hi_r < M && hi_c < M, "atm_phase: taps of layer %d leave the map", l);
    AOENV_CHECK_ARG((reinterpret_cast<uintptr_t>(h_canvas[l]) & 15) == 0, "atm_phase: canvas must be 16-byte aligned");
    static thread_local tma::MapCache<2 * AOENV_MAX_LAYERS> cache;
    const tma::MapKey key{h_canvas[l], ((unsigned long long)(unsigned)pitch << 32) | (unsigned)Mc, (unsigned long long)(unsigned)B};
    const int mrc = cache.get(key, &p.map[l], [&](CUtensorMap* out) {
      cuuint64_t dims[3] = {(cuuint64_t)pitch, (cuuint64_t)Mc, (cuuint64_t)B};
      cuuint64_t strides[2] = {(cuuint64_t)pitch * 4, (cuuint64_t)Mc * pitch * 4};
      cuuint32_t box[3] = {(cuuint32_t)kPhBoxW, (cuuint32_t)kPhBoxH, 1};
      cuuint32_t estr[3] = {1, 1, 1};
      CUresult r = enc(out, CU_TENSOR_MAP_DATA_TYPE_FLOAT32, 3, const_cast<float*>(h_canvas[l]), dims, strides, box, estr,
                       CU_TENSOR_MAP_INTERLEAVE_NONE, CU_TENSOR_MAP_SWIZZLE_NONE, CU_TENSOR_MAP_L2_PROMOTION_L2_128B,
                       CU_TENSOR_MAP_FLOAT_OOB_FILL_NONE);
      if (r != CUDA_SUCCESS) return fail(-4, "atm_phase: cuTensorMapEncodeTiled failed (%d)", (int)r);
      return 0;
    });
    if (mrc) return mrc;
    p.ext[l] = reinterpret_cast<const unsigned long long*>(h_ext[l]);
    p.row0[l] = oy + fp_off + h_row_off[l];
    p.col0[l] = ox + fp_off + h_col_off[l];
    for (int k = 0; k < 4; ++k) {
      p.wrow[l][k] = h_wrow[4 * l + k];
      p.wcol[l][k] = h_wcol[4 * l + k];
    }
    p.weight[l] = h_weight[l];
  }
  dim3 block(kPhThreadsX, kPhThreadsY);
  dim3 grid((R + kPhTileW - 1) / kPhTileW, (R + kPhTileH - 1) / kPhTileH, B);
  AOENV_LAUNCH(atm_phase_kernel, grid, block, 0, (cudaStream_t)stream, p, R, opd_scale, opd_out);
  AOENV_LAUNCH_CHECK("atm_phase");
  return 0;
}

}
```

### rlao_b200/csrc/step.cu

```cuda
#include <math.h>
#include <string.h>

#include "common.cuh"

using namespace aoenv;

namespace {

struct Step { int sx, sy; };

inline double sign_of(double v) { return v > 0 ? 1.0 : (v < 0 ? -1.0 : 0.0); }

int plan_layer(const aoenv_atm_state_t& st, aoenv_layer_state_t& ly, Step* steps, int max_steps) {
  int count = 0;
  if (ly.vX == 0.0 && ly.vY == 0.0) return 0;
  if (ly.not_done_once) {
    ly.not_done_once = 0;
    ly.ratio[0] = ly.vX * st.sampling_time / st.ps_loop;
    ly.ratio[1] = ly.vY * st.sampling_time / st.ps_loop;
    ly.buff[0] = ly.buff[1] = 0.0;
  }
  double a[2] = {fabs(ly.ratio[0]), fabs(ly.ratio[1])};
  long n[2];
  for (int k = 0; k < 2; ++k) n[k] = isinf(a[k]) ? 0 : (long)a[k];
  const double sg[2] = {sign_of(ly.ratio[0]), sign_of(ly.ratio[1])};
  const long nmin = n[0] < n[1] ? n[0] : n[1], nmax = n[0] < n[1] ? n[1] : n[0];
  for (long r = 0; r < nmin && count < max_steps; ++r) steps[count++] = {(int)sg[0], (int)sg[1]};
  for (long r = 0; r < nmax - nmin && count < max_steps; ++r)
    steps[count++] = {n[0] == nmin ? 0 : (int)sg[0], n[1] == nmin ? 0 : (int)sg[1]};
  if (nmax > max_steps) return -1;
  for (int k = 0; k < 2; ++k) ly.buff[k] += fmod(fabs(ly.ratio[k]), 1.0) * sg[k];
  if (fabs(ly.buff[0]) >= 1.0 || fabs(ly.buff[1]) >= 1.0) {
    if (count >= max_steps) return -1;
    steps[count++] = {fabs(ly.buff[0]) < 1.0 ? 0 : (int)sign_of(ly.buff[0]), fabs(ly.buff[1]) < 1.0 ? 0 : (int)sign_of(ly.buff[1])};
  }
  for (int k = 0; k < 2; ++k) ly.buff[k] = fmod(fabs(ly.buff[k]), 1.0) * sign_of(ly.buff[k]);
  return count;
}

inline int pick_origin(double v, int S, int align) {
  const int o = v > 0 ? S : (v < 0 ? 0 : S / 2);
  return o / align * align;
}

inline float* window(const aoenv_atm_state_t& st, int i, int buf, int oy, int ox) {
  return (float*)st.maps[i][buf] + ((size_t)oy * st.pitch + ox);
}

void tap_weights(double buff, int kernel, int* off, float* w) {
  const double f = floor(-buff), frac = -buff - f;
  *off = (int)f - 1;
  double x, v[4];
  if (kernel == 0) {
    x = (frac + 1.0) / 3.0;
    v[0] = 1.0 + x * (-5.5 + x * (9.0 + x * -4.5));
    v[1] = x * (9.0 + x * (-22.5 + x * 13.5));
    v[2] = x * (-4.5 + x * (18.0 + x * -13.5));
    v[3] = x * (1.0 + x * (-4.5 + x * 4.5));
  } else {
    x = frac;
    v[0] = 0.5 * x * (-1.0 + x * (2.0 - x));
    v[1] = 1.0 + 0.5 * x * x * (-5.0 + 3.0 * x);
    v[2] = 0.5 * x * (1.0 + x * (4.0 - 3.0 * x));
    v[3] = 0.5 * x * x * (x - 1.0);
  }
  for (int k = 0; k < 4; ++k) w[k] = (float)v[k];
}

int extrude_group(aoenv_atm_state_t& st, const int* layers, const Step* steps, int G, const void* w_planes, void* stream) {
  const void* wins[AOENV_MAX_LAYERS];
  int32_t sxs[AOENV_MAX_LAYERS], sys_[AOENV_MAX_LAYERS];
  uint64_t seeds[AOENV_MAX_LAYERS], ids[AOENV_MAX_LAYERS];
  const int S = st.S;
  for (int g = 0; g < G; ++g) {
    const int i = layers[g];
    aoenv_layer_state_t& ly = st.layer[i];
    const int sx = steps[g].sx, sy = steps[g].sy;
    if (!(0 <= ly.org[0] - sy && ly.org[0] - sy <= S && 0 <= ly.org[1] - sx && ly.org[1] - sx <= S)) {
      const int foy = pick_origin(ly.vY, S, 1), fox = pick_origin(ly.vX, S, 4);
      int rc = aoenv_atm_compact(window(st, i, ly.cur, ly.org[0], ly.org[1]), window(st, i, 1 - ly.cur, foy, fox), st.B, st.M,
                                 st.pitch, st.env_stride, (uint64_t*)st.ext[i],
                                 (int64_t)(foy - ly.org[0]) * st.pitch + (fox - ly.org[1]), stream);
      if (rc) return rc;
      ly.cur = 1 - ly.cur;
      ly.org[0] = foy;
      ly.org[1] = fox;
      if (!(0 <= foy - sy && foy - sy <= S && 0 <= fox - sx && fox - sx <= S))
        return fail(-2, "atm_update: canvas slack too small for this wind direction change");
    }
    wins[g] = window(st, i, ly.cur, ly.org[0], ly.org[1]);
    sxs[g] = sx;
    sys_[g] = sy;
    seeds[g] = ly.philox_seed;
    ids[g] = ((ly.events << 8) | (uint64_t)i) + (st.env_offset << 40);
    ly.events += 1;
  }
  const bool tc = st.use_tc && G * st.B > AOENV_SKINNY_MAX_ROWS;
  int rc = aoenv_atm_gather_multi(wins, sxs, sys_, seeds, ids, G, st.B, st.M, st.pitch, st.env_stride, (const int32_t*)st.inner_rc,
                                  st.nI, st.nO, nullptr, tc ? nullptr : (float*)st.zx, st.ldz, tc ? st.zx_planes : nullptr,
                                  st.parts, stream);
  if (rc) return rc;
  if (tc)
    rc = aoenv_gemm_tn_tc(st.zx_planes, w_planes, st.ldz, st.parts, (float*)st.X, st.ldx, G * st.B, st.nO, st.ldz, 1.0f, stream);
  else
    rc = aoenv_gemm_tn((const float*)st.zx, st.ldz, (const float*)st.w_f32, st.ldz, (float*)st.X, st.ldx, G * st.B, st.nO, st.ldz,
                       1.0f, stream);
  if (rc) return rc;
  void* wins2[AOENV_MAX_LAYERS];
  int64_t offs[AOENV_MAX_LAYERS];
  void* exts[AOENV_MAX_LAYERS];
  for (int g = 0; g < G; ++g) {
    aoenv_layer_state_t& ly = st.layer[layers[g]];
    ly.org[0] -= steps[g].sy;
    ly.org[1] -= steps[g].sx;
    wins2[g] = window(st, layers[g], ly.cur, ly.org[0], ly.org[1]);
    offs[g] = (int64_t)ly.org[0] * st.pitch + ly.org[1];
    exts[g] = st.ext[layers[g]];
  }
  return aoenv_atm_ring_multi(wins2, offs, exts, G, st.B, st.M, st.pitch, st.env_stride, st.nO, (const float*)st.X, st.ldx,
                              (int32_t*)st.flag, 0, stream);
}

}

extern "C" {

int aoenv_atm_update(aoenv_atm_state_t* state, const void* w_planes, float* opd_out, void* stream) {
  AOENV_CHECK_ARG(state != nullptr && opd_out != nullptr, "atm_update: null state / output");
  aoenv_atm_state_t& st = *state;
  const int L = st.nLayer;
  AOENV_CHECK_ARG(L >= 1 && L <= AOENV_MAX_LAYERS && st.group_max >= 1, "atm_update: %d layers", L);
  AOENV_CHECK_ARG(!st.use_tc || w_planes != nullptr, "atm_update: the operator planes are missing");
  constexpr int kMaxSteps = 64;
  static thread_local Step plans[AOENV_MAX_LAYERS][kMaxSteps];
  int count[AOENV_MAX_LAYERS], rounds = 0;
  for (int i = 0; i < L; ++i) {
    count[i] = plan_layer(st, st.layer[i], plans[i], kMaxSteps);
    if (count[i] < 0) return fail(-2, "atm_update: more than %d add_row steps in one frame (layer %d)", kMaxSteps, i);
    if (count[i] > rounds) rounds = count[i];
  }
  for (int r = 0; r < rounds; ++r) {
    int layers[AOENV_MAX_LAYERS], G = 0;
    Step steps[AOENV_MAX_LAYERS];
    for (int i = 0; i < L; ++i)
      if (count[i] > r) {
        layers[G] = i;
        steps[G++] = plans[i][r];
      }
    for (int k = 0; k < G; k += st.group_max) {
      const int g = G - k < st.group_max ? G - k : st.group_max;
      const int rc = extrude_group(st, layers + k, steps + k, g, w_planes, stream);
      if (rc) return rc;
    }
  }
  const float* canv[AOENV_MAX_LAYERS];
  const uint64_t* exts[AOENV_MAX_LAYERS];
  int32_t org[2 * AOENV_MAX_LAYERS], roff[AOENV_MAX_LAYERS], coff[AOENV_MAX_LAYERS];
  float wr[4 * AOENV_MAX_LAYERS], wc[4 * AOENV_MAX_LAYERS];
  for (int i = 0; i < L; ++i) {
    const aoenv_layer_state_t& ly = st.layer[i];
    canv[i] = (const float*)st.maps[i][ly.cur];
    exts[i] = (const uint64_t*)st.ext[i];
    org[2 * i] = ly.org[0];
    org[2 * i + 1] = ly.org[1];
    tap_weights(ly.buff[0], st.warp_kernel, &coff[i], &wc[4 * i]);
    tap_weights(ly.buff[1], st.warp_kernel, &roff[i], &wr[4 * i]);
  }
  return aoenv_atm_phase(canv, exts, org, L, st.B, st.R, st.M, st.Mc, st.pitch, st.fp_off, roff, coff, wr, wc, st.weight,
                         st.opd_scale, opd_out, stream);
}

}

extern "C" int aoenv_sh_step(const aoenv_sh_step_t* c, int parts, const float* opd_a, const float* dm_rows_cur,
                             const aoenv_detector_t* det, const float* action, float* coefs_next, float* dm_rows_next,
                             float* obs, float* reward, float* strehl, float* total, float* residual, void* stream) {
  AOENV_CHECK_ARG(c != nullptr && parts >= 1 && parts <= 7, "sh_step: bad arguments");
  AOENV_CHECK_ARG(!(parts & 1) || (opd_a != nullptr && dm_rows_cur != nullptr), "sh_step: null wavefront argument");
  AOENV_CHECK_ARG(!(parts & 2) || (obs != nullptr && reward != nullptr && strehl != nullptr), "sh_step: null output argument");
  AOENV_CHECK_ARG(!(parts & 4) || (action != nullptr && coefs_next != nullptr && dm_rows_next != nullptr), "sh_step: null command argument");
  const bool tc = c->use_tc && c->B > AOENV_SKINNY_MAX_ROWS;
  int rc = 0;
  if (parts & 1) {
    aoenv_dm_sep_t dm = c->dm;
    dm.rows = dm_rows_cur;
    rc = aoenv_shwfs_frame_dm(opd_a, nullptr, &dm, (const int32_t*)c->order, (const float*)c->pupil, (const float*)c->amp,
                              (const uint8_t*)c->valid, c->B, c->nS, c->n, c->phase_scale, det, 0, (float*)c->frame,
                              (int32_t*)c->envmax, (double*)c->stats, stream);
    if (rc) return rc;
    rc = aoenv_shwfs_slopes((const float*)c->frame, (const int32_t*)c->envmax, 0, (const int32_t*)c->valid_idx, c->nV,
                            (const float*)c->ref_xy, c->inv_units, c->threshold_cog, c->B, c->nS, c->n, (float*)c->slopes, c->lds,
                            tc ? c->slope_planes : nullptr, 2, stream);
    if (rc) return rc;
  }
  if (parts & 2) {
    if (tc)
      rc = aoenv_gemm_tn_tc(c->slope_planes, c->rec_planes, c->lds, c->rec_parts, (float*)c->rec, c->ldr, c->B, c->nA, c->lds,
                            1.0f, stream);
    else
      rc = aoenv_gemm_tn((const float*)c->slopes, c->lds, (const float*)c->rec_f32, c->lds, (float*)c->rec, c->ldr, c->B, c->nA,
                         c->lds, 1.0f, stream);
    if (rc) return rc;
    rc = aoenv_observe((const float*)c->rec, c->ldr, (const int32_t*)c->act_idx, c->B, c->nA, c->nAct2, (const double*)c->stats,
                       c->n_pupil, c->phase_scale, obs, reward, strehl, total, residual, stream);
    if (rc) return rc;
  }
  if (parts & 4) {
    rc = aoenv_command_update(action, (const int32_t*)c->act_idx, c->B, c->nA, c->nAct2, c->leak, coefs_next, (float*)c->dm_prev,
                              c->ldc, stream);
    if (rc) return rc;
    rc = aoenv_dm_rows(coefs_next, c->ldc, (const int32_t*)c->act_pos, c->nA, c->nAct, c->dm.nActP, (const float*)c->wx,
                       (const int32_t*)c->j0x, c->W, c->B, c->nS * c->n, dm_rows_next, stream);
  }
  return rc;
}
```

### rlao_b200/csrc/wfs.cu

```cuda
#include <stdlib.h>
#include <mutex>

#include "common.cuh"
#include "wfs_twiddles.inc"

namespace aoenv {

constexpr int kMaxN = 8;
__constant__ float2 c_tw[2 * kMaxN * kMaxN];
__constant__ double2 c_twd[2 * kMaxN * kMaxN];
static int g_tw_n[64] = {0};
static std::mutex g_tw_mutex;

static int ensure_twiddles(int n, cudaStream_t stream) {
  int dev = 0;
  cudaGetDevice(&dev);
  std::lock_guard<std::mutex> lock(g_tw_mutex);
  if (dev < 64 && g_tw_n[dev] == n) return 0;
  const int N = 2 * n;
  float2 h[2 * kMaxN * kMaxN];
  double2 hd[2 * kMaxN * kMaxN];
  for (int u = 0; u < N; ++u)
    for (int a = 0; a < n; ++a) {
      const long m = ((long)(a + n / 2) * (2 * u + N + 1)) % (2L * N);
      const double ang = -M_PI * (double)m / (double)N;
      hd[u * n + a] = make_double2(cos(ang), sin(ang));
      h[u * n + a] = make_float2((float)cos(ang), (float)sin(ang));
    }
  cudaError_t e = cudaMemcpyToSymbol(c_tw, h, sizeof(float2) * N * n);
  if (e == cudaSuccess) e = cudaMemcpyToSymbol(c_twd, hd, sizeof(double2) * N * n);
  if (e != cudaSuccess) return fail(-3, "twiddle upload: %s", cudaGetErrorString(e));
  if (dev < 64) g_tw_n[dev] = n;
  (void)stream;
  return 0;
}

struct PixelRng {
  Philox ph;
  uint32_t c0, c1, c2, c3hi;
  __device__ __forceinline__ PixelRng(uint64_t seed, uint32_t pixel, uint32_t env, uint64_t frame)
      : ph(seed), c0(pixel), c1(env), c2((uint32_t)frame), c3hi(((uint32_t)(frame >> 32)) << 16) {}
  __device__ __forceinline__ uint4 block(uint32_t i) const { return ph(c0, c1, c2, c3hi | (i & 0xffffu)); }
};

__constant__ float c_logfact[10] = {0.f, 0.f, 0.6931471806f, 1.7917594692f, 3.1780538303f, 4.7874917428f,
                                    6.5792512120f, 8.5251613611f, 10.6046029027f, 12.8018274801f};
__device__ __forceinline__ float log_factorial(float k) {
  if (k < 10.f) return c_logfact[(int)k];
  const float r = __frcp_rn(k);
  return (k + 0.5f) * __logf(k) - k + 0.9189385332f + r * (0.0833333333f - 0.00277777778f * r * r);
}

struct RcpTable { float v[64]; };
constexpr RcpTable make_rcp() {
  RcpTable t{};
  t.v[0] = 0.f;
  for (int k = 1; k < 64; ++k) t.v[k] = 1.0f / (float)k;
  return t;
}
__constant__ RcpTable c_rcp_table = make_rcp();

__device__ __forceinline__ float poisson_small(float lam, float u) {
  if (!(lam > 0.f)) return 0.f;
  float p = __expf(-lam), F = p;
#pragma unroll
  for (int j = 1; j <= 16; ++j) {
    if (!(u > F)) return (float)(j - 1);
    p *= lam * (1.0f / (float)j);
    F += p;
  }
  int k = 16;
  while (u > F && k < 63) {
    ++k;
    p *= lam * c_rcp_table.v[k];
    F += p;
  }
  return (float)k;
}
__device__ __noinline__ float poisson_small_loop(float lam, float u) {
  float p = __expf(-lam), F = p;
  int k = 0;
  while (u > F && k < 63) {
    ++k;
    p *= lam * c_rcp_table.v[k];
    F += p;
  }
  return (float)k;
}

struct Ptrs {
  float lam, loglam, bb, a, invalpha, vr;
  __device__ __forceinline__ explicit Ptrs(float l) : lam(l) {
    const float slam = sqrtf(l);
    loglam = __logf(l);
    bb = 0.931f + 2.53f * slam;
    a = -0.059f + 0.02483f * bb;
    invalpha = 1.1239f + __fdividef(1.1328f, bb - 3.4f);
    vr = 0.9277f - __fdividef(3.6224f, bb - 2.f);
  }
  __device__ __forceinline__ bool attempt(uint32_t w0, uint32_t w1, float& k) const {
    const float U = u32_to_unit(w0) - 0.5f;
    const float V = u32_to_unit(w1);
    const float us = 0.5f - fabsf(U);
    k = floorf((__fdividef(2.f * a, us) + bb) * U + lam + 0.43f);
    if (us >= 0.07f && V <= vr) return true;
    if (k < 0.f || (us < 0.013f && V > us)) return false;
    return __logf(V * invalpha * __frcp_rn(__fdividef(a, us * us) + bb)) <= -lam + k * loglam - log_factorial(k);
  }
};
constexpr int kPtrsMaxAttempts = 15;

__device__ __forceinline__ float poisson_draw(float lam, uint32_t w0, uint32_t w1, const PixelRng& rng, uint32_t retry_block) {
  if (!(lam > 0.f)) return 0.f;
  if (lam < 12.f) return poisson_small_loop(lam, u32_to_unit(w0) * 0.99999994f);
  const Ptrs pt(lam);
  for (int it = 0; it < kPtrsMaxAttempts; ++it) {
    if (it > 0) {
      const uint4 r = rng.block(retry_block + (uint32_t)it);
      w0 = r.x;
      w1 = r.y;
    }
    float k;
    if (pt.attempt(w0, w1, k)) return k;
  }
  return rintf(lam);
}

__device__ __forceinline__ float detector_finish(float photons, float dark, float ron, const aoenv_detector_t& d, uint32_t stages) {
  float x = photons;
  if (stages & 1u) x *= d.qe;
  if (stages & 2u) {
    x += dark;
    if (d.has_fwc) x = fminf(fmaxf(x, 0.f), d.fwc);
    if (d.sensor_emccd) x *= d.gain;
  }
  if (stages & 4u) {
    x += ron;
    if (!d.sensor_emccd) x *= d.gain;
    if (d.bits > 0) {
      const float full = (float)((1u << d.bits) - 1u);
      x = truncf(x / d.fwc * full);
      x = fminf(x, full);
    }
  }
  return x;
}

constexpr int kDetPerLane = 8;
struct DetQueued { float lam, ron; uint32_t w0, w1; int pix; };

__device__ __forceinline__ uint32_t spare_word(const uint4& r) {
  return (r.x & 0xffu) | ((r.y & 0xffu) << 8) | ((r.z & 0xffu) << 16) | (r.w << 24);
}

__global__ void __launch_bounds__(256)
shwfs_detector_kernel(float* __restrict__ frame, const uint8_t* __restrict__ valid, int nS, int n, float inv_R, float inv_n,
                      const __grid_constant__ aoenv_detector_t det, int shared_max, int32_t* __restrict__ envmax,
                      int n_pixels) {
  pdl_enter();
  __shared__ DetQueued queue[8][kDetPerLane * 32];
  const int R = nS * n, P = n_pixels > 0 ? n_pixels : R * R;
  const int b = blockIdx.y, lane = threadIdx.x & 31, warp = threadIdx.x >> 5;
  const int first = (blockIdx.x * 8 + warp) * (kDetPerLane * 32);
  float* __restrict__ img = frame + (size_t)b * P;
  DetQueued* __restrict__ q = queue[warp];
  int queued = 0;
  float vmax = -INFINITY;
  const uint32_t stages = det.reserved ? det.reserved : 7u;
  const bool photon_noise = det.photon_noise && (stages & 1u);
  const bool has_dark = det.dark_electrons > 0.f && (stages & 2u);
  const bool has_ron = det.readout_noise != 0.f && (stages & 4u);
  const float dark_p0 = has_dark ? __expf(-det.dark_electrons) : 1.f;

  auto is_lit = [&](int pix) {
    if (valid == nullptr) return envmax != nullptr;
    const int y = (int)(((float)pix + 0.5f) * inv_R);
    const int x = pix - y * R;
    const int li = (int)(((float)y + 0.5f) * inv_n), lj = (int)(((float)x + 0.5f) * inv_n);
    return valid[li * nS + lj] != 0;
  };
  auto track = [&](int pix, float val) {
    if (val > vmax && is_lit(pix)) vmax = val;
  };
  auto dark_draw = [&](const uint4& r0, const PixelRng& rng) {
    if (!has_dark) return 0.f;
    const uint32_t w = spare_word(r0);
    const float u = u32_to_unit(w) * 0.99999994f;
    if (!(u > dark_p0)) return 0.f;
    if (det.dark_electrons < 12.f) return poisson_small_loop(det.dark_electrons, u);
    const uint4 r1 = rng.block(1);
    return poisson_draw(det.dark_electrons, r1.x, r1.y, rng, 32);
  };

#pragma unroll 2
  for (int j = 0; j < kDetPerLane; ++j) {
    const int pix = first + j * 32 + lane;
    const bool in = pix < P;
    const float lam = in ? img[pix] : 0.f;
    const PixelRng rng(det.seed, (uint32_t)pix, (uint32_t)b, det.frame_counter);
    const uint4 r0 = rng.block(0);
    float ron = 0.f;
    if (has_ron)
      ron = rintf(sqrtf(-2.0f * __logf(u32_to_unit(r0.z))) * __cosf(6.283185307179586f * u32_to_unit(r0.w)) * det.readout_noise);
    const float dark = dark_draw(r0, rng);
    const bool ptrs = in && photon_noise && lam >= 12.f;
    if (!ptrs && in) {
      const float photons = photon_noise ? poisson_small(lam, u32_to_unit(r0.x) * 0.99999994f) : lam;
      const float val = detector_finish(photons, dark, ron, det, stages);
      img[pix] = val;
      track(pix, val);
    }
    const unsigned m = __ballot_sync(0xffffffffu, ptrs);
    if (ptrs) {
      const uint32_t dk = (uint32_t)fminf(dark, 65535.f);
      q[queued + __popc(m & ((1u << lane) - 1u))] = {lam, ron, (r0.x & ~0xffu) | (dk & 0xffu), (r0.y & ~0xffu) | (dk >> 8), pix};
    }
    queued += __popc(m);
  }
  __syncwarp();
  for (int round = 0; queued > 0; ++round) {
    int kept = 0;
    for (int e0 = 0; e0 < queued; e0 += 32) {
      const int e = e0 + lane;
      const bool have = e < queued;
      DetQueued it = q[have ? e : 0];
      bool rejected = false;
      if (have) {
        const float dark = (float)((it.w0 & 0xffu) | ((it.w1 & 0xffu) << 8));
        if (round > 0) {
          const PixelRng rng(det.seed, (uint32_t)it.pix, (uint32_t)b, det.frame_counter);
          const uint4 r = rng.block(16u + (uint32_t)round);
          it.w0 = (r.x & ~0xffu) | (it.w0 & 0xffu);
          it.w1 = (r.y & ~0xffu) | (it.w1 & 0xffu);
        }
        const Ptrs pt(it.lam);
        float photons;
        bool ok = pt.attempt(it.w0, it.w1, photons);
        if (!ok && round == kPtrsMaxAttempts - 1) { photons = rintf(it.lam); ok = true; }
        if (ok) {
          const float val = detector_finish(photons, dark, it.ron, det, stages);
          img[it.pix] = val;
          track(it.pix, val);
        }
        rejected = !ok;
      }
      __syncwarp();
      const unsigned m = __ballot_sync(0xffffffffu, rejected);
      if (rejected) q[kept + __popc(m & ((1u << lane) - 1u))] = it;
      kept += __popc(m);
    }
    __syncwarp();
    queued = kept;
  }
  if (envmax != nullptr) {
    vmax = warp_max(vmax);
    if (lane == 0 && vmax > -INFINITY) atomicMax(&envmax[shared_max ? 0 : b], float_to_ordered(vmax));
  }
}

template <int n, int WL = 0>
__global__ void __launch_bounds__(128)
shwfs_frame_kernel(const float* __restrict__ opd_a, const float* __restrict__ opd_b, const float* __restrict__ pupil,
                   const float* __restrict__ amp, const uint8_t* __restrict__ valid, int nS, float phase_scale,
                   int track_max, int shared_max, float* __restrict__ frame,
                   int32_t* __restrict__ envmax, double* __restrict__ stats, const __grid_constant__ aoenv_dm_sep_t dm,
                   const int32_t* __restrict__ order) {
  constexpr int N = 2 * n;
  pdl_enter();
  const int R = nS * n;
  const int b = blockIdx.y;
  const int k0 = blockIdx.x * blockDim.x + threadIdx.x;
  const bool active = k0 < nS * nS;
  const int k = (active && order != nullptr) ? __ldg(&order[k0]) : k0;
  const int li = active ? k / nS : 0, lj = active ? k % nS : 0;
  const bool lit = active && valid[k] != 0;
  const float phase_turns = phase_scale * 0.15915494309189535f;

  float2 er2[n][n / 2], ei2[n][n / 2];
  float f0 = 0.f, f1 = 0.f, f2 = 0.f, f3 = 0.f;
  if (active) {
    const size_t tile = (size_t)(li * n) * R + lj * n;
    const float* __restrict__ pa = opd_a + (size_t)b * R * R + tile;
    const float* __restrict__ pb = (WL == 0 && opd_b) ? opd_b + (size_t)b * R * R + tile : nullptr;
    const size_t centre = (size_t)b * R * R + (size_t)(R / 2) * R + R / 2;
    const float ka = stats ? __ldg(opd_a + centre) : 0.f;
    const float kt = stats ? (pb ? ka + __ldg(opd_b + centre) : ka) : 0.f;
    float2 dmv[WL > 0 ? n : 1][n / 2];
    if (WL > 0) {
      constexpr int half = (WL + 1) / 2, hp = (half + 3) / 4 * 4;
#pragma unroll
      for (int bb = 0; bb < n; ++bb)
#pragma unroll
        for (int a2 = 0; a2 < n / 2; ++a2) dmv[WL > 0 ? bb : 0][a2] = make_float2(0.f, 0.f);
      const float* __restrict__ trow = dm.rows + ((size_t)b * dm.nActP + __ldg(&dm.ilr[li])) * R + lj * n;
      const float* __restrict__ wrow = dm.wlr + (size_t)(li * n) * (2 * hp);
#pragma unroll
      for (int g = 0; g < 2 * hp / 4; ++g) {
        float4 w4[n];
#pragma unroll
        for (int bb = 0; bb < n; ++bb) w4[bb] = __ldg(reinterpret_cast<const float4*>(wrow + (size_t)bb * (2 * hp)) + g);
#pragma unroll
        for (int e = 0; e < 4; ++e) {
          const int j = 4 * g + e, hh = j / hp, kk = j % hp;
          if (kk >= half) continue;
          const int t = hh * half + kk;
          if (t >= WL) continue;
          float2 tv[n / 2];
#pragma unroll
          for (int a2 = 0; a2 < n / 2; ++a2) tv[a2] = __ldg(reinterpret_cast<const float2*>(trow + (size_t)t * R) + a2);
#pragma unroll
          for (int bb = 0; bb < n; ++bb) {
            const float w = e == 0 ? w4[bb].x : (e == 1 ? w4[bb].y : (e == 2 ? w4[bb].z : w4[bb].w));
#pragma unroll
            for (int a2 = 0; a2 < n / 2; ++a2) dmv[WL > 0 ? bb : 0][a2] = fma2(dup2(w), tv[a2], dmv[WL > 0 ? bb : 0][a2]);
          }
        }
      }
    }
#pragma unroll
    for (int bb = 0; bb < n; ++bb) {
#pragma unroll
      for (int a2 = 0; a2 < n / 2; ++a2) {
        const int o2 = bb * R + 2 * a2;
        const float2 av = __ldg(reinterpret_cast<const float2*>(pa + o2));
        const float2 bv = WL > 0 ? dmv[WL > 0 ? bb : 0][a2]
                                 : (pb ? __ldg(reinterpret_cast<const float2*>(pb + o2)) : make_float2(0.f, 0.f));
        const float2 pv = __ldg(reinterpret_cast<const float2*>(pupil + tile + o2));
        const float2 mv = lit ? __ldg(reinterpret_cast<const float2*>(amp + tile + o2)) : make_float2(0.f, 0.f);
#pragma unroll
        for (int e = 0; e < 2; ++e) {
          const int aa = 2 * a2 + e;
          const float a = e ? av.y : av.x;
          const float t = a + (e ? bv.y : bv.x);
          const float pu = e ? pv.y : pv.x;
          const float in_pupil = pu > 0.f ? 1.f : 0.f;
          const float da = (a - ka) * in_pupil, dt = (t - kt) * in_pupil;
          f0 += da; f1 = fmaf(da, da, f1); f2 += dt; f3 = fmaf(dt, dt, f3);
          const float turns = t * pu * phase_turns;
          const float ang = (turns - ((turns + 12582912.0f) - 12582912.0f)) * 6.283185307179586f;
          const float sn = __sinf(ang), cs = __cosf(ang);
          const float am = e ? mv.y : mv.x;
          if ((bb & 1) == 0) { er2[aa][bb >> 1].x = am * cs; ei2[aa][bb >> 1].x = am * sn; }
          else { er2[aa][bb >> 1].y = am * cs; ei2[aa][bb >> 1].y = am * sn; }
        }
      }
    }
  }
  double s0 = (double)f0, s1 = (double)f1, s2 = (double)f2, s3 = (double)f3;

  if (stats != nullptr) {
    s0 = warp_sum(s0); s1 = warp_sum(s1); s2 = warp_sum(s2); s3 = warp_sum(s3);
    if ((threadIdx.x & 31) == 0) {
      double* __restrict__ st = stats + (size_t)b * 4;
      atomicAdd(st, s0); atomicAdd(st + 1, s1); atomicAdd(st + 2, s2); atomicAdd(st + 3, s3);
    }
  }

  float vmax = -INFINITY;
  if (active) {
    float* __restrict__ fout = frame + (size_t)b * R * R + (size_t)(li * n) * R + lj * n;
    const float norm = 1.0f / (float)(N * N);
    constexpr int h = n / 2;
#pragma unroll 1
    for (int pp = 0; pp < h; ++pp) {
      float2 acc[n];
#pragma unroll
      for (int q = 0; q < n; ++q) acc[q] = make_float2(0.f, 0.f);
      if (lit) {
#pragma unroll
        for (int du = 0; du < 2; ++du) {
          const int u = 2 * pp + du;
          float2 pr[h], pi[h], qr[h], qi[h];
#pragma unroll
          for (int k = 0; k < h; ++k) { pr[k] = pi[k] = qr[k] = qi[k] = make_float2(0.f, 0.f); }
#pragma unroll
          for (int aa = 0; aa < n; ++aa) {
            const float2 g = c_tw[u * n + aa];
            const float2 gx = dup2(g.x), gy = dup2(g.y), ngy = dup2(-g.y);
            if (((aa + h) & 1) == 0) {
#pragma unroll
              for (int k = 0; k < h; ++k) {
                pr[k] = fma2(gx, er2[aa][k], fma2(ngy, ei2[aa][k], pr[k]));
                pi[k] = fma2(gx, ei2[aa][k], fma2(gy, er2[aa][k], pi[k]));
              }
            } else {
#pragma unroll
              for (int k = 0; k < h; ++k) {
                qr[k] = fma2(gx, er2[aa][k], fma2(ngy, ei2[aa][k], qr[k]));
                qi[k] = fma2(gx, ei2[aa][k], fma2(gy, er2[aa][k], qi[k]));
              }
            }
          }
          float2 yr[n], yi[n];
#pragma unroll
          for (int bb = 0; bb < n; ++bb) {
            const float p_r = (bb & 1) ? pr[bb >> 1].y : pr[bb >> 1].x, q_r = (bb & 1) ? qr[bb >> 1].y : qr[bb >> 1].x;
            const float p_i = (bb & 1) ? pi[bb >> 1].y : pi[bb >> 1].x, q_i = (bb & 1) ? qi[bb >> 1].y : qi[bb >> 1].x;
            yr[bb] = make_float2(p_r + q_r, p_r - q_r);
            yi[bb] = make_float2(p_i + q_i, p_i - q_i);
          }
#pragma unroll
          for (int v = 0; v < n; ++v) {
            float2 er_ = make_float2(0.f, 0.f), ei_ = er_, or_ = er_, oi_ = er_;
#pragma unroll
            for (int bb = 0; bb < n; ++bb) {
              const float gx = WfsTw<n>::re(v * n + bb), gy = WfsTw<n>::im(v * n + bb);
              if (((bb + h) & 1) == 0) {
                er_ = fma2(yr[bb], dup2(gx), fma2(yi[bb], dup2(-gy), er_));
                ei_ = fma2(yr[bb], dup2(gy), fma2(yi[bb], dup2(gx), ei_));
              } else {
                or_ = fma2(yr[bb], dup2(gx), fma2(yi[bb], dup2(-gy), or_));
                oi_ = fma2(yr[bb], dup2(gy), fma2(yi[bb], dup2(gx), oi_));
              }
            }
            const float2 f0r = add2(er_, or_), f0i = add2(ei_, oi_);
            const float2 f1r = sub2(er_, or_), f1i = sub2(ei_, oi_);
            acc[v >> 1] = add2(acc[v >> 1], fma2(f0r, f0r, mul2(f0i, f0i)));
            acc[(v >> 1) + h] = add2(acc[(v >> 1) + h], fma2(f1r, f1r, mul2(f1i, f1i)));
          }
        }
      }
#pragma unroll
      for (int r2 = 0; r2 < 2; ++r2) {
        const int p = pp + r2 * h;
#pragma unroll
        for (int q = 0; q < n; ++q) {
          const float val = (r2 == 0 ? acc[q].x : acc[q].y) * norm;
          fout[(size_t)p * R + q] = val;
          if (lit) vmax = fmaxf(vmax, val);
        }
      }
    }
  }
  if (track_max) {
    vmax = warp_max(vmax);
    if ((threadIdx.x & 31) == 0 && vmax > -INFINITY) atomicMax(&envmax[shared_max ? 0 : b], float_to_ordered(vmax));
  }
}

struct C2 { float2 r, i; };
__device__ __forceinline__ C2 cadd(const C2& a, const C2& b) { return {add2(a.r, b.r), add2(a.i, b.i)}; }
__device__ __forceinline__ C2 csub(const C2& a, const C2& b) { return {sub2(a.r, b.r), sub2(a.i, b.i)}; }
__device__ __forceinline__ C2 cmulc(const C2& a, float wr, float wi) {
  return {fma2(a.r, dup2(wr), mul2(a.i, dup2(-wi))), fma2(a.r, dup2(wi), mul2(a.i, dup2(wr)))};
}
__device__ __forceinline__ void dft3(const C2& z0, const C2& z1, const C2& z2, C2& y0, C2& y1, C2& y2) {
  constexpr float c = 0.8660254037844386f;
  const C2 t = cadd(z1, z2), d = csub(z1, z2);
  y0 = cadd(z0, t);
  const C2 m = {fma2(dup2(-0.5f), t.r, z0.r), fma2(dup2(-0.5f), t.i, z0.i)};
  y1 = {fma2(dup2(c), d.i, m.r), fma2(dup2(-c), d.r, m.i)};
  y2 = {fma2(dup2(-c), d.i, m.r), fma2(dup2(c), d.r, m.i)};
}
template <int K1>
__device__ __forceinline__ void dft6_half(const C2 (&z)[6], C2& y0, C2& y1, C2& y2) {
  const C2 s0 = K1 == 0 ? cadd(z[0], z[3]) : csub(z[0], z[3]);
  const C2 s1 = K1 == 0 ? cadd(z[2], z[5]) : csub(z[2], z[5]);
  const C2 s2 = K1 == 0 ? cadd(z[4], z[1]) : csub(z[4], z[1]);
  dft3(s0, s1, s2, y0, y1, y2);
}
__device__ __forceinline__ void twiddle6(const C2 (&z)[6], C2 (&w)[6]) {
  constexpr float c = 0.8660254037844386f;
  w[0] = z[0];
  w[1] = cmulc(z[1], c, -0.5f);
  w[2] = cmulc(z[2], 0.5f, -c);
  w[3] = {z[3].i, mul2(z[3].r, dup2(-1.0f))};
  w[4] = cmulc(z[4], -0.5f, -c);
  w[5] = cmulc(z[5], -c, -0.5f);
}
__host__ __device__ constexpr int dft6_row(int k1, int k2) { return (3 * k1 + 4 * k2) % 6; }

template <int K1>
__device__ __forceinline__ void wfs6_pass1(const float* __restrict__ sF, C2 (&Hp)[3][6]) {
  constexpr float c = 0.8660254037844386f;
#pragma unroll
  for (int b = 0; b < 6; ++b) {
    C2 z[6];
#pragma unroll
    for (int a = 0; a < 6; ++a) {
      const float xr = sF[(2 * (a * 6 + b)) * 128], xi = sF[(2 * (a * 6 + b) + 1) * 128];
      float wr, wi;
      if (a == 0) { wr = xr; wi = xi; }
      else if (a == 1) { wr = fmaf(xr, c, xi * 0.5f); wi = fmaf(xi, c, xr * -0.5f); }
      else if (a == 2) { wr = fmaf(xr, 0.5f, xi * c); wi = fmaf(xi, 0.5f, xr * -c); }
      else if (a == 3) { wr = xi; wi = -xr; }
      else if (a == 4) { wr = fmaf(xr, -0.5f, xi * c); wi = fmaf(xi, -0.5f, xr * -c); }
      else { wr = fmaf(xr, -c, xi * 0.5f); wi = fmaf(xi, -c, xr * -0.5f); }
      z[a] = {make_float2(xr, wr), make_float2(xi, wi)};
    }
    dft6_half<K1>(z, Hp[0][b], Hp[1][b], Hp[2][b]);
  }
}

template <int K1>
__device__ __forceinline__ void wfs6_pass2(const C2 (&Hp)[3][6], float norm, float* __restrict__ fout, int R, float& vmax) {
#pragma unroll
  for (int k2 = 0; k2 < 3; ++k2) {
    const int p = dft6_row(K1, k2);
    C2 yw[6];
    twiddle6(Hp[k2], yw);
    float row[6];
#pragma unroll
    for (int q1 = 0; q1 < 2; ++q1) {
      C2 e[3], o[3];
      if (q1 == 0) { dft6_half<0>(Hp[k2], e[0], e[1], e[2]); dft6_half<0>(yw, o[0], o[1], o[2]); }
      else { dft6_half<1>(Hp[k2], e[0], e[1], e[2]); dft6_half<1>(yw, o[0], o[1], o[2]); }
#pragma unroll
      for (int q2 = 0; q2 < 3; ++q2) {
        const float2 i0 = fma2(e[q2].r, e[q2].r, mul2(e[q2].i, e[q2].i));
        const float2 i1 = fma2(o[q2].r, o[q2].r, mul2(o[q2].i, o[q2].i));
        const float2 t = add2(i0, i1);
        row[dft6_row(q1, q2)] = (t.x + t.y) * norm;
      }
    }
#pragma unroll
    for (int q = 0; q < 6; ++q) {
      fout[(size_t)p * R + q] = row[q];
      vmax = fmaxf(vmax, row[q]);
    }
  }
}

__global__ void __launch_bounds__(128, 3)
shwfs_frame6_kernel(const float* __restrict__ opd_a, const float* __restrict__ opd_b, const float* __restrict__ pupil,
                    const float* __restrict__ amp, const uint8_t* __restrict__ valid, int nS, float phase_scale,
                    int track_max, int shared_max, float* __restrict__ frame, int32_t* __restrict__ envmax,
                    double* __restrict__ stats) {
  constexpr int n = 6, N = 12;
  __shared__ float sF_all[2 * n * n * 128];
  float* __restrict__ sF = sF_all + threadIdx.x;
  const int R = nS * n;
  const int b = blockIdx.y;
  const int k = blockIdx.x * blockDim.x + threadIdx.x;
  const bool active = k < nS * nS;
  const int li = active ? k / nS : 0, lj = active ? k % nS : 0;
  const bool lit = active && valid[k] != 0;
  const float phase_turns = phase_scale * 0.15915494309189535f;
  float f0 = 0.f, f1 = 0.f, f2 = 0.f, f3 = 0.f;
  if (active) {
    const size_t tile = (size_t)(li * n) * R + lj * n;
    const float* __restrict__ pa = opd_a + (size_t)b * R * R + tile;
    const float* __restrict__ pb = opd_b ? opd_b + (size_t)b * R * R + tile : nullptr;
    const size_t centre = (size_t)b * R * R + (size_t)(R / 2) * R + R / 2;
    const float ka = stats ? __ldg(opd_a + centre) : 0.f;
    const float kt = stats ? (opd_b ? ka + __ldg(opd_b + centre) : ka) : 0.f;
#pragma unroll
    for (int bb = 0; bb < n; ++bb) {
#pragma unroll
      for (int aa = 0; aa < n; ++aa) {
        const int o = bb * R + aa;
        const float a = __ldg(pa + o);
        const float t = pb ? a + __ldg(pb + o) : a;
        const float pu = __ldg(pupil + tile + o);
        const float in_pupil = pu > 0.f ? 1.f : 0.f;
        const float da = (a - ka) * in_pupil, dt = (t - kt) * in_pupil;
        f0 += da; f1 = fmaf(da, da, f1); f2 += dt; f3 = fmaf(dt, dt, f3);
        if (lit) {
          constexpr double kTurn = -13.0 / 24.0;
          const double cst = kTurn * (double)(aa + bb + n);
          const float cfrac = (float)(cst - (double)(long long)(cst - 0.5));
          const float turns = fmaf(t * pu, phase_turns, cfrac);
          const float ang = (turns - ((turns + 12582912.0f) - 12582912.0f)) * 6.283185307179586f;
          const float am = __ldg(amp + tile + o);
          sF[(2 * (aa * n + bb)) * 128] = am * __cosf(ang);
          sF[(2 * (aa * n + bb) + 1) * 128] = am * __sinf(ang);
        }
      }
    }
  }
  if (stats != nullptr) {
    double s0 = warp_sum((double)f0), s1 = warp_sum((double)f1), s2 = warp_sum((double)f2), s3 = warp_sum((double)f3);
    if ((threadIdx.x & 31) == 0) {
      double* __restrict__ st = stats + (size_t)b * 4;
      atomicAdd(st, s0); atomicAdd(st + 1, s1); atomicAdd(st + 2, s2); atomicAdd(st + 3, s3);
    }
  }
  float vmax = -INFINITY;
  if (active) {
    float* __restrict__ fout = frame + (size_t)b * R * R + (size_t)(li * n) * R + lj * n;
    if (lit) {
      const float norm = 1.0f / (float)(N * N);
      C2 Hp[3][6];
      wfs6_pass1<0>(sF, Hp);
      wfs6_pass2<0>(Hp, norm, fout, R, vmax);
      wfs6_pass1<1>(sF, Hp);
      wfs6_pass2<1>(Hp, norm, fout, R, vmax);
    } else {
#pragma unroll
      for (int p = 0; p < n; ++p)
#pragma unroll
        for (int q = 0; q < n; ++q) fout[(size_t)p * R + q] = 0.f;
    }
  }
  if (track_max) {
    vmax = warp_max(vmax);
    if ((threadIdx.x & 31) == 0 && vmax > -INFINITY) atomicMax(&envmax[shared_max ? 0 : b], float_to_ordered(vmax));
  }
}

constexpr int kS6Lenslets = 10;
constexpr int kS6Warps = 4;

__device__ __forceinline__ void dft6_both(const C2 (&z)[6], C2 (&y)[2][3]) {
  dft6_half<0>(z, y[0][0], y[0][1], y[0][2]);
  dft6_half<1>(z, y[1][0], y[1][1], y[1][2]);
}

__global__ void __launch_bounds__(kS6Warps * 32, 4)
shwfs_frame6s_kernel(const float* __restrict__ opd_a, const float* __restrict__ opd_b, const float* __restrict__ pupil,
                     const float* __restrict__ amp, const uint8_t* __restrict__ valid, int nS, float phase_scale,
                     int track_max, int shared_max, float* __restrict__ frame, int32_t* __restrict__ envmax,
                     double* __restrict__ stats) {
  constexpr int n = 6, N = 12;
  constexpr float c = 0.8660254037844386f;
  __shared__ float xch[kS6Warps][48][33];
  const int R = nS * n;
  const int b = blockIdx.y;
  const int lane = threadIdx.x & 31, warp = threadIdx.x >> 5;
  const int slot = lane / 3, t = lane - slot * 3;
  const int k = (blockIdx.x * kS6Warps + warp) * kS6Lenslets + slot;
  const bool active = slot < kS6Lenslets && k < nS * nS;
  const int li = active ? k / nS : 0, lj = active ? k - li * nS : 0;
  const bool lit = active && valid[k] != 0;
  const float phase_turns = phase_scale * 0.15915494309189535f;
  const size_t tile = (size_t)(li * n) * R + lj * n;
  float f0 = 0.f, f1 = 0.f, f2 = 0.f, f3 = 0.f;
  C2 y[2][2][3];
// ... 122 lines not shown
                         const float* __restrict__ amp, const uint8_t* __restrict__ valid, int nS, float phase_scale,
                         int track_max, int shared_max, float* __restrict__ frame, int32_t* __restrict__ envmax,
                         double* __restrict__ stats) {
  constexpr int N = 2 * n, T = n / 2, h = n / 2, LPW = 32 / T, S = LPW + 1;
  __shared__ float2 xch[4][4 * T * n][S];
  const int R = nS * n;
  const int b = blockIdx.y;
  const int lane = threadIdx.x & 31, warp = threadIdx.x >> 5;
  const int slot = lane / T, t = lane - slot * T;
  const int k = (blockIdx.x * 4 + warp) * LPW + slot;
  const bool active = slot < LPW && k < nS * nS;
  const int li = active ? k / nS : 0, lj = active ? k - li * nS : 0;
  const bool lit = active && valid[k] != 0;
  const float phase_turns = phase_scale * 0.15915494309189535f;
  const size_t tile = (size_t)(li * n) * R + lj * n;
  float f0 = 0.f, f1 = 0.f, f2 = 0.f, f3 = 0.f;
  float2 er2[n], ei2[n];
  if (active) {
    const float* __restrict__ pa = opd_a + (size_t)b * R * R + tile;
    const float* __restrict__ pb = opd_b ? opd_b + (size_t)b * R * R + tile : nullptr;
    const size_t centre = (size_t)b * R * R + (size_t)(R / 2) * R + R / 2;
    const float ka = stats ? __ldg(opd_a + centre) : 0.f;
    const float kt = stats ? (opd_b ? ka + __ldg(opd_b + centre) : ka) : 0.f;
#pragma unroll
    for (int e = 0; e < 2; ++e) {
      const int bb = 2 * t + e;
#pragma unroll
      for (int a2 = 0; a2 < h; ++a2) {
        const int o2 = bb * R + 2 * a2;
        const float2 av = __ldg(reinterpret_cast<const float2*>(pa + o2));
        const float2 bv = pb ? __ldg(reinterpret_cast<const float2*>(pb + o2)) : make_float2(0.f, 0.f);
        const float2 pv = __ldg(reinterpret_cast<const float2*>(pupil + tile + o2));
        const float2 mv = lit ? __ldg(reinterpret_cast<const float2*>(amp + tile + o2)) : make_float2(0.f, 0.f);
#pragma unroll
        for (int h2 = 0; h2 < 2; ++h2) {
          const int aa = 2 * a2 + h2;
          const float a = h2 ? av.y : av.x;
          const float tt = a + (h2 ? bv.y : bv.x);
          const float pu = h2 ? pv.y : pv.x;
          const float in_pupil = pu > 0.f ? 1.f : 0.f;
          const float da = (a - ka) * in_pupil, dt = (tt - kt) * in_pupil;
          f0 += da; f1 = fmaf(da, da, f1); f2 += dt; f3 = fmaf(dt, dt, f3);
          const float turns = tt * pu * phase_turns;
          const float ang = (turns - ((turns + 12582912.0f) - 12582912.0f)) * 6.283185307179586f;
          const float am = h2 ? mv.y : mv.x;
          const float cs = am * __cosf(ang), sn = am * __sinf(ang);
          if (e == 0) { er2[aa].x = cs; ei2[aa].x = sn; } else { er2[aa].y = cs; ei2[aa].y = sn; }
        }
      }
    }
  }
  if (stats != nullptr) {
    double s0 = warp_sum((double)f0), s1 = warp_sum((double)f1), s2 = warp_sum((double)f2), s3 = warp_sum((double)f3);
    if (lane == 0) {
      double* __restrict__ st = stats + (size_t)b * 4;
      atomicAdd(st, s0); atomicAdd(st + 1, s1); atomicAdd(st + 2, s2); atomicAdd(st + 3, s3);
    }
  }
  float2 (*x)[S] = xch[warp];
  const bool any_lit = __any_sync(0xffffffffu, lit);
  float vmax = -INFINITY;
  if (any_lit) {
    if (lit) {
#pragma unroll
      for (int u = 0; u < n; ++u) {
        float2 pr = make_float2(0.f, 0.f), pi = pr, qr = pr, qi = pr;
#pragma unroll
        for (int aa = 0; aa < n; ++aa) {
          const float gx = WfsTw<n>::re(u * n + aa), gy = WfsTw<n>::im(u * n + aa);
          if (((aa + h) & 1) == 0) {
            pr = fma2(dup2(gx), er2[aa], fma2(dup2(-gy), ei2[aa], pr));
            pi = fma2(dup2(gx), ei2[aa], fma2(dup2(gy), er2[aa], pi));
          } else {
            qr = fma2(dup2(gx), er2[aa], fma2(dup2(-gy), ei2[aa], qr));
            qi = fma2(dup2(gx), ei2[aa], fma2(dup2(gy), er2[aa], qi));
          }
        }
        x[(0 * T + t) * n + u][slot] = pr;
        x[(1 * T + t) * n + u][slot] = pi;
        x[(2 * T + t) * n + u][slot] = qr;
        x[(3 * T + t) * n + u][slot] = qi;
      }
    }
    __syncwarp();
    if (lit) {
      float* __restrict__ fout = frame + (size_t)b * R * R + tile;
      const float norm = 1.0f / (float)(N * N);
      float2 acc[n];
#pragma unroll
      for (int q = 0; q < n; ++q) acc[q] = make_float2(0.f, 0.f);
#pragma unroll
      for (int du = 0; du < 2; ++du) {
        const int u = 2 * t + du;
        float2 yr[n], yi[n];
#pragma unroll
        for (int kk = 0; kk < T; ++kk) {
          const float2 pr = x[(0 * T + kk) * n + u][slot], pi = x[(1 * T + kk) * n + u][slot];
          const float2 qr = x[(2 * T + kk) * n + u][slot], qi = x[(3 * T + kk) * n + u][slot];
          yr[2 * kk] = make_float2(pr.x + qr.x, pr.x - qr.x);
          yr[2 * kk + 1] = make_float2(pr.y + qr.y, pr.y - qr.y);
          yi[2 * kk] = make_float2(pi.x + qi.x, pi.x - qi.x);
          yi[2 * kk + 1] = make_float2(pi.y + qi.y, pi.y - qi.y);
        }
#pragma unroll
        for (int v = 0; v < n; ++v) {
          float2 er_ = make_float2(0.f, 0.f), ei_ = er_, or_ = er_, oi_ = er_;
#pragma unroll
          for (int bb = 0; bb < n; ++bb) {
            const float gx = WfsTw<n>::re(v * n + bb), gy = WfsTw<n>::im(v * n + bb);
            if (((bb + h) & 1) == 0) {
              er_ = fma2(yr[bb], dup2(gx), fma2(yi[bb], dup2(-gy), er_));
              ei_ = fma2(yr[bb], dup2(gy), fma2(yi[bb], dup2(gx), ei_));
            } else {
              or_ = fma2(yr[bb], dup2(gx), fma2(yi[bb], dup2(-gy), or_));
              oi_ = fma2(yr[bb], dup2(gy), fma2(yi[bb], dup2(gx), oi_));
            }
          }
          const float2 f0r = add2(er_, or_), f0i = add2(ei_, oi_);
          const float2 f1r = sub2(er_, or_), f1i = sub2(ei_, oi_);
          acc[v >> 1] = add2(acc[v >> 1], fma2(f0r, f0r, mul2(f0i, f0i)));
          acc[(v >> 1) + h] = add2(acc[(v >> 1) + h], fma2(f1r, f1r, mul2(f1i, f1i)));
        }
      }
#pragma unroll
      for (int q2 = 0; q2 < h; ++q2) {
        const float2 lo = make_float2(acc[2 * q2].x * norm, acc[2 * q2 + 1].x * norm);
        const float2 hi = make_float2(acc[2 * q2].y * norm, acc[2 * q2 + 1].y * norm);
        *reinterpret_cast<float2*>(fout + (size_t)t * R + 2 * q2) = lo;
        *reinterpret_cast<float2*>(fout + (size_t)(t + h) * R + 2 * q2) = hi;
        vmax = fmaxf(vmax, fmaxf(fmaxf(lo.x, lo.y), fmaxf(hi.x, hi.y)));
      }
    }
  }
  if (active && !lit) {
    float* __restrict__ fout = frame + (size_t)b * R * R + tile;
#pragma unroll
    for (int e = 0; e < 2; ++e)
#pragma unroll
      for (int q2 = 0; q2 < h; ++q2) *reinterpret_cast<float2*>(fout + (size_t)(2 * t + e) * R + 2 * q2) = make_float2(0.f, 0.f);
  }
  if (track_max) {
    vmax = warp_max(vmax);
    if (lane == 0 && vmax > -INFINITY) atomicMax(&envmax[shared_max ? 0 : b], float_to_ordered(vmax));
  }
}

template <int n>
__global__ void __launch_bounds__(128)
shwfs_slopes_kernel(const float* __restrict__ frame, const int32_t* __restrict__ envmax, int shared_max,
                    const int32_t* __restrict__ valid_idx, int nV, const float* __restrict__ ref_xy, float inv_units,
                    float threshold_cog, int nS, float* __restrict__ slopes, int lds,
                    __nv_bfloat16* __restrict__ planes, int parts) {
  const int b = blockIdx.y;
  pdl_enter();
  const int t = blockIdx.x * blockDim.x + threadIdx.x;
  if (t >= nV) return;
  const int R = nS * n;
  const int k = __ldg(&valid_idx[t]);
  const int li = k / nS, lj = k - li * nS;
  const float thr = threshold_cog * ordered_to_float(__ldg(&envmax[shared_max ? 0 : b]));
  const float* __restrict__ f = frame + (size_t)b * R * R + (size_t)(li * n) * R + lj * n;
  float2 v[n][n / 2];
#pragma unroll
  for (int p = 0; p < n; ++p)
#pragma unroll
    for (int h = 0; h < n / 2; ++h) v[p][h] = __ldg(reinterpret_cast<const float2*>(f + (size_t)p * R) + h);
  float s = 0.f, sx = 0.f, sy = 0.f;
#pragma unroll
  for (int p = 0; p < n; ++p)
#pragma unroll
    for (int q = 0; q < n; ++q) {
      float x = (q & 1) ? v[p][q >> 1].y : v[p][q >> 1].x;
      x = x < thr ? 0.f : x;
      s += x;
      sx = fmaf(x, (float)p, sx);
      sy = fmaf(x, (float)q, sy);
    }
  float cx = sx / s, cy = sy / s;
  if (!isfinite(cx)) cx = 0.f;
  if (!isfinite(cy)) cy = 0.f;
  const float sx_ = (cx - __ldg(&ref_xy[t])) * inv_units, sy_ = (cy - __ldg(&ref_xy[nV + t])) * inv_units;
  slopes[(size_t)b * lds + t] = sx_;
  slopes[(size_t)b * lds + nV + t] = sy_;
  if (planes != nullptr) {
    store_bf16_planes(planes, (size_t)gridDim.y * lds, (size_t)b * lds + t, parts, sx_);
    store_bf16_planes(planes, (size_t)gridDim.y * lds, (size_t)b * lds + nV + t, parts, sy_);
  }
}

template <int n>
__global__ void __launch_bounds__(64)
shwfs_frame_f64_kernel(const float* __restrict__ opd, const float* __restrict__ pupil, const float* __restrict__ amp,
                       const uint8_t* __restrict__ valid, int nS, double phase_scale, int shared_max,
                       double* __restrict__ frame, unsigned long long* __restrict__ envmax) {
  constexpr int N = 2 * n;
  const int R = nS * n;
  const int b = blockIdx.y;
  const int k = blockIdx.x * blockDim.x + threadIdx.x;
  if (k >= nS * nS) return;
  const int li = k / nS, lj = k % nS;
  const bool lit = valid[k] != 0;
  const size_t tile = (size_t)(li * n) * R + lj * n;
  double* __restrict__ fout = frame + (size_t)b * R * R + tile;
  if (!lit) {
    for (int p = 0; p < n; ++p)
      for (int q = 0; q < n; ++q) fout[(size_t)p * R + q] = 0.0;
    return;
  }
  double er[n][n], ei[n][n];
  const float* __restrict__ pa = opd + (size_t)b * R * R + tile;
#pragma unroll
  for (int bb = 0; bb < n; ++bb)
#pragma unroll
    for (int aa = 0; aa < n; ++aa) {
      const int o = bb * R + aa;
      double sn, cs;
      sincos((double)__ldg(pa + o) * (double)__ldg(pupil + tile + o) * phase_scale, &sn, &cs);
      const double am = (double)__ldg(amp + tile + o);
      er[aa][bb] = am * cs;
      ei[aa][bb] = am * sn;
    }
  double vmax = 0.0;
  const double norm = 1.0 / (double)(N * N);
  for (int p = 0; p < n; ++p) {
    double acc[n];
#pragma unroll
    for (int q = 0; q < n; ++q) acc[q] = 0.0;
    for (int du = 0; du < 2; ++du) {
      const int u = 2 * p + du;
      double yr[n], yi[n];
#pragma unroll
      for (int bb = 0; bb < n; ++bb) { yr[bb] = 0.0; yi[bb] = 0.0; }
#pragma unroll
      for (int aa = 0; aa < n; ++aa) {
        const double2 g = c_twd[u * n + aa];
#pragma unroll
        for (int bb = 0; bb < n; ++bb) {
          yr[bb] += g.x * er[aa][bb] - g.y * ei[aa][bb];
          yi[bb] += g.x * ei[aa][bb] + g.y * er[aa][bb];
        }
      }
#pragma unroll
      for (int v = 0; v < N; ++v) {
        double fr = 0.0, fi = 0.0;
#pragma unroll
        for (int bb = 0; bb < n; ++bb) {
          const double2 g = c_twd[v * n + bb];
          fr += yr[bb] * g.x - yi[bb] * g.y;
          fi += yr[bb] * g.y + yi[bb] * g.x;
        }
        acc[v >> 1] += fr * fr + fi * fi;
      }
    }
#pragma unroll
    for (int q = 0; q < n; ++q) {
      const double val = acc[q] * norm;
      fout[(size_t)p * R + q] = val;
      vmax = fmax(vmax, val);
    }
  }
  atomicMax(&envmax[shared_max ? 0 : b], (unsigned long long)__double_as_longlong(vmax));
}

__global__ void __launch_bounds__(128)
shwfs_slopes_f64_kernel(const double* __restrict__ frame, const unsigned long long* __restrict__ envmax, int shared_max,
                        const int32_t* __restrict__ valid_idx, int nV, const double* __restrict__ ref_xy,
                        double inv_units, double threshold_cog, int nS, int n, double* __restrict__ slopes, int lds) {
  const int b = blockIdx.y;
  const int t = blockIdx.x * blockDim.x + threadIdx.x;
  if (t >= nV) return;
  const int R = nS * n;
  const int k = __ldg(&valid_idx[t]);
  const int li = k / nS, lj = k % nS;
  const double thr = threshold_cog * __longlong_as_double((long long)envmax[shared_max ? 0 : b]);
  const double* __restrict__ f = frame + (size_t)b * R * R + (size_t)(li * n) * R + lj * n;
  double s = 0.0, sx = 0.0, sy = 0.0;
  for (int p = 0; p < n; ++p)
    for (int q = 0; q < n; ++q) {
      double v = f[(size_t)p * R + q];
      v = v < thr ? 0.0 : v;
      s += v;
      sx += v * (double)p;
      sy += v * (double)q;
    }
  double cx = sx / s, cy = sy / s;
  if (!isfinite(cx)) cx = 0.0;
  if (!isfinite(cy)) cy = 0.0;
  slopes[(size_t)b * lds + t] = (cx - ref_xy[t]) * inv_units;
  slopes[(size_t)b * lds + nV + t] = (cy - ref_xy[nV + t]) * inv_units;
}

__global__ void envmax_init_kernel(int32_t* __restrict__ envmax, int count, double* __restrict__ stats, int n_stats) {
  pdl_enter();
  const int i = blockIdx.x * blockDim.x + threadIdx.x;
  if (i < count) envmax[i] = float_to_ordered(-INFINITY);
  if (stats != nullptr && i < n_stats) stats[i] = 0.0;
}

}

using namespace aoenv;

constexpr int kDefaultFrameVariant = 0;
static std::atomic<int> g_wfs6_factorised{[] {
  const char* e = getenv("AOENV_WFS_FRAME");
  if (e && e[0] == 'f') return 1;
  if (e && e[0] == 's') return (e[5] == '6') ? 2 : 3;
  if (e && e[0] == 't') return 0;
  return kDefaultFrameVariant;
}()};

extern "C" {

int aoenv_set_wfs6_variant(int variant) {
  return g_wfs6_factorised.exchange(variant < 0 || variant > 3 ? kDefaultFrameVariant : variant);
}

static int shwfs_frame_impl(const float* opd_a, const float* opd_b, const aoenv_dm_sep_t* dm_in, const int32_t* order, const float* pupil,
                            const float* amp, const uint8_t* valid, int B, int nS, int n, float phase_scale,
                            const aoenv_detector_t* det, int shared_max, float* frame, int32_t* envmax, double* stats,
                            void* stream) {
  AOENV_CHECK_ARG(B > 0 && B <= 65535 && nS > 0, "shwfs_frame: bad shape B=%d nS=%d", B, nS);
  aoenv_dm_sep_t dm{};
  if (dm_in != nullptr) {
    dm = *dm_in;
    AOENV_CHECK_ARG(opd_b == nullptr, "shwfs_frame_dm: give either the separable DM or an explicit second OPD term");
    AOENV_CHECK_ARG(dm.rows != nullptr && dm.wlr != nullptr && dm.ilr != nullptr && dm.nActP > 0, "shwfs_frame_dm: bad DM tables");
    AOENV_CHECK_ARG(dm.WL == 14 || dm.WL == 18, "shwfs_frame_dm: DM window of %d actuator rows (14 or 18)", dm.WL);
    AOENV_CHECK_ARG((reinterpret_cast<uintptr_t>(dm.rows) & 7) == 0 && (reinterpret_cast<uintptr_t>(dm.wlr) & 15) == 0,
                    "shwfs_frame_dm: DM tables must be 16-byte aligned");
  }
  AOENV_CHECK_ARG(n == 4 || n == 6 || n == 8, "shwfs_frame: %d pixels per lenslet is not a compiled size (4, 6, 8)", n);
  cudaStream_t s = (cudaStream_t)stream;
  if (det) {
    AOENV_CHECK_ARG(!(det->bits > 0 && !det->has_fwc), "shwfs_frame: ADC without a full-well capacity is not supported");
    AOENV_CHECK_ARG(det->bits >= 0 && det->bits < 31, "shwfs_frame: bits=%d", det->bits);
  }
  int rc = ensure_twiddles(n, s);
  if (rc) return rc;
  AOENV_LAUNCH(envmax_init_kernel, dim3((4 * B + 255) / 256), 256, 0, s, envmax, shared_max ? 1 : B, stats, stats ? 4 * B : 0);
  AOENV_LAUNCH_CHECK("envmax_init");
  dim3 grid((nS * nS + 127) / 128, B);
  const int variant = g_wfs6_factorised.load(std::memory_order_relaxed);
  if (variant == 3 && dm.WL == 0) {
    const int per_block = 4 * (32 / (n / 2));
    dim3 g3((nS * nS + per_block - 1) / per_block, B);
    if (n == 4) shwfs_frame_split_kernel<4><<<g3, 128, 0, s>>>(opd_a, opd_b, pupil, amp, valid, nS, phase_scale, det == nullptr, shared_max, frame, envmax, stats);
    else if (n == 6) shwfs_frame_split_kernel<6><<<g3, 128, 0, s>>>(opd_a, opd_b, pupil, amp, valid, nS, phase_scale, det == nullptr, shared_max, frame, envmax, stats);
    else shwfs_frame_split_kernel<8><<<g3, 128, 0, s>>>(opd_a, opd_b, pupil, amp, valid, nS, phase_scale, det == nullptr, shared_max, frame, envmax, stats);
  } else
#define AOENV_WFS_CASE(NN)                                                                                   \
  case NN:                                                                                                   \
    if (dm.WL == 14)                                                                                         \
      AOENV_LAUNCH((shwfs_frame_kernel<NN, 14>), grid, 128, 0, s, opd_a, opd_b, pupil, amp, valid, nS, phase_scale, \
                   (int)(det == nullptr), shared_max, frame, envmax, stats, dm, order);                             \
    else if (dm.WL == 18)                                                                                    \
      AOENV_LAUNCH((shwfs_frame_kernel<NN, 18>), grid, 128, 0, s, opd_a, opd_b, pupil, amp, valid, nS, phase_scale, \
                   (int)(det == nullptr), shared_max, frame, envmax, stats, dm, order);                             \
    else                                                                                                     \
      AOENV_LAUNCH((shwfs_frame_kernel<NN, 0>), grid, 128, 0, s, opd_a, opd_b, pupil, amp, valid, nS, phase_scale,  \
                   (int)(det == nullptr), shared_max, frame, envmax, stats, dm, order);                             \
    break;
  switch (n) {
    AOENV_WFS_CASE(4)
    AOENV_WFS_CASE(8)
    case 6:
      if (dm.WL != 0) {
        if (dm.WL == 14) {
          AOENV_LAUNCH((shwfs_frame_kernel<6, 14>), grid, 128, 0, s, opd_a, opd_b, pupil, amp, valid, nS, phase_scale,
                       (int)(det == nullptr), shared_max, frame, envmax, stats, dm, order);
        } else
          AOENV_LAUNCH((shwfs_frame_kernel<6, 18>), grid, 128, 0, s, opd_a, opd_b, pupil, amp, valid, nS, phase_scale,
                       (int)(det == nullptr), shared_max, frame, envmax, stats, dm, order);
      } else if (variant == 2) {
        dim3 g3((nS * nS + kS6Warps * kS6Lenslets - 1) / (kS6Warps * kS6Lenslets), B);
        shwfs_frame6s_kernel<<<g3, kS6Warps * 32, 0, s>>>(opd_a, opd_b, pupil, amp, valid, nS, phase_scale, det == nullptr,
                                                          shared_max, frame, envmax, stats);
      } else if (variant == 1)
        shwfs_frame6_kernel<<<grid, 128, 0, s>>>(opd_a, opd_b, pupil, amp, valid, nS, phase_scale, det == nullptr, shared_max,
                                                 frame, envmax, stats);
      else
        AOENV_LAUNCH((shwfs_frame_kernel<6, 0>), grid, 128, 0, s, opd_a, opd_b, pupil, amp, valid, nS, phase_scale,
                     (int)(det == nullptr), shared_max, frame, envmax, stats, dm, order);
      break;
  }
#undef AOENV_WFS_CASE
  AOENV_LAUNCH_CHECK("shwfs_frame");
  if (det) {
    const int R = nS * n;
    AOENV_CHECK_ARG(R * R < (1 << 24), "shwfs_frame: frame of %d x %d pixels is too large for the camera pass", R, R);
    dim3 gd((R * R + 8 * kDetPerLane * 32 - 1) / (8 * kDetPerLane * 32), B);
    AOENV_LAUNCH(shwfs_detector_kernel, gd, 256, 0, s, frame, valid, nS, n, 1.0f / (float)R, 1.0f / (float)n, *det, shared_max, envmax, 0);
    AOENV_LAUNCH_CHECK("shwfs_detector");
  }
  return 0;
}

int aoenv_shwfs_frame(const float* opd_a, const float* opd_b, const float* pupil, const float* amp,
                      const uint8_t* valid, int B, int nS, int n, float phase_scale, const aoenv_detector_t* det,
                      int shared_max, float* frame, int32_t* envmax, double* stats, void* stream) {
  return shwfs_frame_impl(opd_a, opd_b, nullptr, nullptr, pupil, amp, valid, B, nS, n, phase_scale, det, shared_max, frame, envmax, stats, stream);
}

int aoenv_shwfs_frame_dm(const float* opd_a, const float* opd_b, const aoenv_dm_sep_t* dm, const int32_t* order,
                         const float* pupil, const float* amp, const uint8_t* valid, int B, int nS, int n, float phase_scale,
                         const aoenv_detector_t* det, int shared_max, float* frame, int32_t* envmax, double* stats,
                         void* stream) {
  return shwfs_frame_impl(opd_a, opd_b, dm, order, pupil, amp, valid, B, nS, n, phase_scale, det, shared_max, frame, envmax, stats, stream);
}

int aoenv_shwfs_camera(float* frame, const uint8_t* valid, int B, int nS, int n, const aoenv_detector_t* det, int shared_max,
                       int32_t* envmax, void* stream) {
  AOENV_CHECK_ARG(B > 0 && B <= 65535 && nS > 0 && n > 0, "shwfs_camera: bad shape B=%d nS=%d", B, nS);
  AOENV_CHECK_ARG(det != nullptr && valid != nullptr && envmax != nullptr, "shwfs_camera: detector, lenslet mask and envmax are required");
  AOENV_CHECK_ARG(!(det->bits > 0 && !det->has_fwc), "shwfs_camera: ADC without a full-well capacity is not supported");
  AOENV_CHECK_ARG(det->bits >= 0 && det->bits < 31, "shwfs_camera: bits=%d", det->bits);
  const int R = nS * n;
  AOENV_CHECK_ARG(R * R < (1 << 24), "shwfs_camera: frame of %d x %d pixels is too large for the camera pass", R, R);
  cudaStream_t s = (cudaStream_t)stream;
  AOENV_LAUNCH(envmax_init_kernel, dim3((B + 255) / 256), 256, 0, s, envmax, shared_max ? 1 : B, (double*)nullptr, 0);
  AOENV_LAUNCH_CHECK("envmax_init");
  dim3 gd((R * R + 8 * kDetPerLane * 32 - 1) / (8 * kDetPerLane * 32), B);
  shwfs_detector_kernel<<<gd, 256, 0, s>>>(frame, valid, nS, n, 1.0f / (float)R, 1.0f / (float)n, *det, shared_max, envmax, 0);
  AOENV_LAUNCH_CHECK("shwfs_detector");
  return 0;
}

int aoenv_detector_integrate(float* frame, int B, int rows, int cols, const aoenv_detector_t* det, void* stream) {
  AOENV_CHECK_ARG(B > 0 && B <= 65535 && rows > 0 && cols > 0 && (long long)rows * cols < (1 << 24), "detector_integrate: bad shape");
  AOENV_CHECK_ARG(det != nullptr, "detector_integrate: no detector given");
  AOENV_CHECK_ARG(!(det->bits > 0 && !det->has_fwc), "detector_integrate: ADC without a full-well capacity is not supported");
  AOENV_CHECK_ARG(det->bits >= 0 && det->bits < 31, "detector_integrate: bits=%d", det->bits);
  const int P = rows * cols;
  dim3 gd((P + 8 * kDetPerLane * 32 - 1) / (8 * kDetPerLane * 32), B);
  shwfs_detector_kernel<<<gd, 256, 0, (cudaStream_t)stream>>>(frame, nullptr, 1, 1, 1.0f, 1.0f, *det, 0, nullptr, P);
  AOENV_LAUNCH_CHECK("detector_integrate");
  return 0;
}

int aoenv_shwfs_slopes(const float* frame, const int32_t* envmax, int shared_max, const int32_t* valid_idx, int nV,
                       const float* ref_xy, float inv_units, float threshold_cog, int B, int nS, int n, float* slopes,
                       int lds, void* slope_planes, int parts, void* stream) {
  AOENV_CHECK_ARG(B > 0 && B <= 65535 && nV > 0 && lds >= 2 * nV, "shwfs_slopes: bad shape B=%d nV=%d lds=%d", B, nV, lds);
  AOENV_CHECK_ARG(n == 4 || n == 6 || n == 8, "shwfs_slopes: %d pixels per lenslet is not a compiled size (4, 6, 8)", n);
  AOENV_CHECK_ARG((reinterpret_cast<uintptr_t>(frame) & 7) == 0, "shwfs_slopes: frame must be 8-byte aligned");
  dim3 grid((nV + 127) / 128, B);
#define AOENV_SLOPES_CASE(NN)                                                                                          \
  case NN:                                                                                                             \
    AOENV_LAUNCH(shwfs_slopes_kernel<NN>, grid, 128, 0, (cudaStream_t)stream, frame, envmax, shared_max, valid_idx, nV, \
                 ref_xy, inv_units, threshold_cog, nS, slopes, lds, (__nv_bfloat16*)slope_planes, parts);              \
    break;
  switch (n) {
    AOENV_SLOPES_CASE(4)
    AOENV_SLOPES_CASE(6)
    AOENV_SLOPES_CASE(8)
  }
#undef AOENV_SLOPES_CASE
  AOENV_LAUNCH_CHECK("shwfs_slopes");
  return 0;
}

int aoenv_shwfs_measure_f64(const float* opd, const float* pupil, const float* amp, const uint8_t* valid,
                            const int32_t* valid_idx, int nV, const double* ref_xy, double inv_units, double threshold_cog,
                            int F, int nS, int n, double phase_scale, int shared_max, double* frame, uint64_t* envmax,
                            double* slopes, int lds, void* stream) {
  AOENV_CHECK_ARG(F > 0 && F <= 65535 && nS > 0 && nV > 0 && lds >= 2 * nV, "shwfs_measure_f64: bad shape");
  AOENV_CHECK_ARG(n == 4 || n == 6 || n == 8, "shwfs_measure_f64: %d pixels per lenslet is not a compiled size (4, 6, 8)", n);
  cudaStream_t s = (cudaStream_t)stream;
  int rc = ensure_twiddles(n, s);
  if (rc) return rc;
  cudaError_t e = cudaMemsetAsync(envmax, 0, sizeof(uint64_t) * (shared_max ? 1 : (size_t)F), s);
  if (e != cudaSuccess) return fail(-3, "shwfs_measure_f64 memset: %s", cudaGetErrorString(e));
  dim3 grid((nS * nS + 63) / 64, F);
  unsigned long long* em = reinterpret_cast<unsigned long long*>(envmax);
  switch (n) {
    case 4: shwfs_frame_f64_kernel<4><<<grid, 64, 0, s>>>(opd, pupil, amp, valid, nS, phase_scale, shared_max, frame, em); break;
    case 6: shwfs_frame_f64_kernel<6><<<grid, 64, 0, s>>>(opd, pupil, amp, valid, nS, phase_scale, shared_max, frame, em); break;
    case 8: shwfs_frame_f64_kernel<8><<<grid, 64, 0, s>>>(opd, pupil, amp, valid, nS, phase_scale, shared_max, frame, em); break;
  }
  AOENV_LAUNCH_CHECK("shwfs_frame_f64");
  dim3 g2((nV + 127) / 128, F);
  shwfs_slopes_f64_kernel<<<g2, 128, 0, s>>>(frame, em, shared_max, valid_idx, nV, ref_xy, inv_units, threshold_cog, nS, n,
                                             slopes, lds);
  AOENV_LAUNCH_CHECK("shwfs_slopes_f64");
  return 0;
}

}
```

Measured before the change: 1.411 million.

## Fuse atmosphere sub-pixel phase interpolation into SH-WFS frame kernel behind opt-in flag

Adds a deferred atmosphere phase mode in which the sub-pixel shift and sum over layers is computed inside the n=6 Shack-Hartmann frame kernel, on a tile loaded into shared memory. The result is written out and reused from shared memory, which removes the separate phase kernel and its global round trip. The path is gated by AOENV_ATM_FUSED, which defaults to off, and it turns off early prefetch when enabled. The standalone phase kernel also gets a new 120x40 tile shape and FMA-based tap helpers, which do run by default.

Result: no change. 1.421 million (median of 6 runs) (+0.7%).

```diff
diff --git a/include/aoenv.h b/include/aoenv.h
--- a/include/aoenv.h
+++ b/include/aoenv.h
@@ -54,6 +54,15 @@
   int32_t cur;
   int32_t org[2];
 } aoenv_layer_state_t;
+
+typedef struct {
+  const void* canvas[AOENV_MAX_LAYERS];
+  void* out;
+  int32_t org[2 * AOENV_MAX_LAYERS];
+  int32_t row_off[AOENV_MAX_LAYERS], col_off[AOENV_MAX_LAYERS];
+  float wrow[4 * AOENV_MAX_LAYERS], wcol[4 * AOENV_MAX_LAYERS];
+  int32_t pending, reserved;
+} aoenv_atm_phase_t;
 
 typedef struct {
   int32_t nLayer, B, R, M, Mc, pitch, S, nI, nO, ldz, ldx, group_max, parts, fp_off, warp_kernel, use_tc;
@@ -71,9 +80,12 @@
   void* flag;
   const void* w_f32;
   aoenv_layer_state_t layer[AOENV_MAX_LAYERS];
+  int32_t defer_phase, reserved2;
+  aoenv_atm_phase_t phase;
 } aoenv_atm_state_t;
 
 int aoenv_atm_update(aoenv_atm_state_t* state, const void* w_planes, float* opd_out, void* stream);
+int aoenv_atm_resolve(aoenv_atm_state_t* state, void* stream);
 
 #define AOENV_SKINNY_MAX_ROWS 8
 int aoenv_gemm_tn(const float* X, int ldx, const float* W, int ldw, float* D, int ldd,
@@ -154,6 +166,7 @@
   const void* act_idx;
   void* dm_prev;
   const void *act_pos, *wx, *j0x;
+  aoenv_atm_state_t* atm;
 } aoenv_sh_step_t;
 
 int aoenv_sh_step(const aoenv_sh_step_t* c, int parts, const float* opd_a, const float* dm_rows_cur, const aoenv_detector_t* det,
diff --git a/rlao_b200/Atmosphere.py b/rlao_b200/Atmosphere.py
--- a/rlao_b200/Atmosphere.py
+++ b/rlao_b200/Atmosphere.py
@@ -386,11 +386,12 @@
                                                C.c_float(self.wavelength / 2 / math.pi), _lib.ptr(out),
                                                _lib.stream_ptr(self.device)), "atm_phase")
 
-    def _advance(self, out):
+    def _advance(self, out, defer=False):
         if (self.native_update and self.rng == "philox" and self.xi_queue is None and self.xi_log is None
                 and self._cstate.warp_kernel >= 0):
             tc = self._cstate.use_tc
             self._cstate.sampling_time, self._cstate.env_offset = float(self.telescope.samplingTime), self.env_offset
+            self._cstate.defer_phase = int(defer)
             _lib.check(_lib.load().aoenv_atm_update(C.byref(self._cstate), _lib.ptr(self._W_op.planes()) if tc else None,
                                                     _lib.ptr(out), _lib.stream_ptr(self.device)), "atm_update")
         else:
@@ -406,7 +407,7 @@
         return (self.rng == "philox" and self.xi_queue is None and self.xi_log is None
                 and not self.user_defined_opd and self._opd is not None and self._opd.is_cuda)
 
-    def prefetch(self):
+    def prefetch(self, defer=False):
         if self._prefetched:
             return True
         if not self.can_prefetch():
@@ -421,19 +422,37 @@
         main, side = torch.cuda.current_stream(dev), self._side_stream
         side.wait_event(main.record_event())
         with torch.cuda.stream(side):
-            self._advance(self._opd_next)
+            self._advance(self._opd_next, defer)
             self._prefetch_event = side.record_event()
         self._prefetched = True
         return True
 
-    def _join_prefetch(self, consume):
+    def _join_prefetch(self, consume, keep_pending=False):
+        if not consume:
+            self._cstate.phase.pending = 0
         if not self._prefetched:
             return False
         torch.cuda.current_stream(self.device).wait_event(self._prefetch_event)
         self._prefetched = False
         if consume:
             self._opd, self._opd_next = self._opd_next, self._opd
+            if not keep_pending:
+                self._resolve_phase()
         return True
+
+    def _resolve_phase(self):
+        if not self._cstate.phase.pending:
+            return
+        if self._prefetched:
+            torch.cuda.current_stream(self.device).wait_event(self._prefetch_event)
+        _lib.check(_lib.load().aoenv_atm_resolve(C.byref(self._cstate), _lib.stream_ptr(self.device)), "atm_resolve")
+
+    def _update_deferred(self):
+        self.user_defined_opd = False
+        if not self._join_prefetch(consume=True, keep_pending=True):
+            self._advance(self._opd, defer=True)
+        if self.telescope.isPaired:
+            self * self.telescope
 
     def update(self, OPD=None):
         if OPD is None:
diff --git a/rlao_b200/OOPAOEnv/OOPAOEnvRazor.py b/rlao_b200/OOPAOEnv/OOPAOEnvRazor.py
--- a/rlao_b200/OOPAOEnv/OOPAOEnvRazor.py
+++ b/rlao_b200/OOPAOEnv/OOPAOEnvRazor.py
@@ -58,6 +58,7 @@
         self.psf_reward = None
         self.native_step = os.environ.get("AOENV_STEP_NATIVE", "1") != "0"
         self.prefetch_early = os.environ.get("AOENV_PREFETCH_EARLY", "1") != "0"
+        self.atm_fused = os.environ.get("AOENV_ATM_FUSED", "0") == "1"
         self._native_key, self._native = None, None
 
     def set_params_file(self, param_file, oopao_path):
@@ -251,7 +252,7 @@
         if wfs._flux_version != getattr(src, "_flux_version", 0) or wfs.current_nPhoton != src.nPhoton:
             return None
         key = (wfs._flux_version, id(wfs._amp), id(wfs._ref_xy), wfs.slopes_units, wfs.threshold_cog, float(self.leak),
-               id(self._Rm_op), id(dm._sep), src.wavelength, id(self._coefs_buf))
+               id(self._Rm_op), id(dm._sep), src.wavelength, id(self._coefs_buf), self.atm_fused, self.atm.sm_partition is None)
         if self._native_key == key:
             return self._native
         self._native_key, self._native = key, None
@@ -277,6 +278,8 @@
         c.rec_planes = self._Rm_op.planes().data_ptr() if tc else None
         c.rec_f32, c.rec, c.act_idx, c.dm_prev = self._Rm.data_ptr(), self._rec.data_ptr(), self._act_idx.data_ptr(), self._dm_prev.data_ptr()
         c.act_pos, c.wx, c.j0x = tables["act_pos"].data_ptr(), tables["wx"].data_ptr(), tables["j0x"].data_ptr()
+        if self.atm_fused and c.n == 6 and self.atm.sm_partition is None:
+            c.atm = ctypes.addressof(self.atm._cstate)
         self._native = (c, keep)
         return self._native
 
@@ -284,7 +287,11 @@
         c = native[0]
         dm, wfs, atm, B, dev = self.dm, self.wfs, self.atm, self.n_envs, self.device
         slot = dm._slot
-        atm.update()
+        fused = bool(c.atm)
+        if fused:
+            atm._update_deferred()
+        else:
+            atm.update()
         self.tel._set_lazy(atm._opd, DMSurfaceRef(dm, slot))
         det = wfs.cam.as_struct(self.env_offset)
         nAct = self.nActuator
@@ -297,12 +304,13 @@
                 self._total_now.data_ptr(), self._residual_now.data_ptr(), _lib.stream_ptr(dev)]
         step, cref = _lib.load().aoenv_sh_step, ctypes.byref(c)
         if atm.can_prefetch() or after_observe is not None or action_ready is not None:
-            early = atm.sm_partition is not None or (self.prefetch_early and after_observe is None and action_ready is None)
+            early = not fused and (atm.sm_partition is not None
+                                   or (self.prefetch_early and after_observe is None and action_ready is None))
             if early:
                 atm.prefetch()
             _lib.check(step(cref, 1, *args), "sh_step")
             if not early:
-                atm.prefetch()
+                atm.prefetch(defer=fused)
             _lib.check(step(cref, 2, *args), "sh_step")
             if after_observe is not None:
                 after_observe(self._sq(obs), self._sq(reward), self._sq(strehl))
@@ -388,6 +396,7 @@
 
     def state_dict(self):
         atm = self.atm
+        atm._resolve_phase()
         nxt = None
         if atm._prefetched:
             torch.cuda.current_stream(self.device).wait_event(atm._prefetch_event)
diff --git a/rlao_b200/_lib.py b/rlao_b200/_lib.py
--- a/rlao_b200/_lib.py
+++ b/rlao_b200/_lib.py
@@ -44,7 +44,15 @@
         ("n_pupil", C.c_double)] + [(k, C.c_void_p) for k in ("pupil", "amp", "valid", "order", "valid_idx", "ref_xy", "frame",
                                                               "envmax", "stats", "slopes", "slope_planes")] + [
         ("dm", DmSepStruct)] + [(k, C.c_void_p) for k in ("rec_planes", "rec_f32", "rec", "act_idx", "dm_prev", "act_pos",
-                                                           "wx", "j0x")]
+                                                           "wx", "j0x", "atm")]
+
+
+class AtmPhaseStruct(C.Structure):
+    _fields_ = [
+        ("canvas", C.c_void_p * MAX_LAYERS), ("out", C.c_void_p), ("org", C.c_int32 * (2 * MAX_LAYERS)),
+        ("row_off", C.c_int32 * MAX_LAYERS), ("col_off", C.c_int32 * MAX_LAYERS), ("wrow", C.c_float * (4 * MAX_LAYERS)),
+        ("wcol", C.c_float * (4 * MAX_LAYERS)), ("pending", C.c_int32), ("reserved", C.c_int32),
+    ]
 
 
 class AtmState(C.Structure):
@@ -54,7 +62,7 @@
         ("opd_scale", C.c_float), ("reserved", C.c_float), ("weight", C.c_float * MAX_LAYERS),
         ("maps", (C.c_void_p * 2) * MAX_LAYERS), ("ext", C.c_void_p * MAX_LAYERS), ("inner_rc", C.c_void_p),
         ("zx", C.c_void_p), ("zx_planes", C.c_void_p), ("X", C.c_void_p), ("flag", C.c_void_p), ("w_f32", C.c_void_p),
-        ("layer", LayerState * MAX_LAYERS),
+        ("layer", LayerState * MAX_LAYERS), ("defer_phase", C.c_int32), ("reserved2", C.c_int32), ("phase", AtmPhaseStruct),
     ]
 
 _vp, _i, _f, _u64, _d, _i64 = C.c_void_p, C.c_int, C.c_float, C.c_uint64, C.c_double, C.c_int64
@@ -68,6 +76,7 @@
     "aoenv_vk_screens": [_u64, C.c_uint32, _i, _i, _vp, _vp, _vp, _vp, _i, _i, _vp, _vp, _vp, _vp, _vp, _vp, _vp, _i, _vp, _i,
                          _vp, _i, _i64, _vp],
     "aoenv_atm_update": [_vp, _vp, _vp, _vp],
+    "aoenv_atm_resolve": [_vp, _vp],
     "aoenv_sh_step": [_vp, _i] + [_vp] * 12,
     "aoenv_atm_phase": [_vp, _vp, _vp, _i, _i, _i, _i, _i, _i, _i, _vp, _vp, _vp, _vp, _vp, _f, _vp, _vp],
     "aoenv_gemm_tn": [_vp, _i, _vp, _i, _vp, _i, _i, _i, _i, _f, _vp],
diff --git a/rlao_b200/csrc/atm.cu b/rlao_b200/csrc/atm.cu
--- a/rlao_b200/csrc/atm.cu
+++ b/rlao_b200/csrc/atm.cu
@@ -1,3 +1,4 @@
+#include "atm_interp.cuh"
 #include "common.cuh"
 #include "tma.cuh"
 
@@ -41,9 +42,6 @@
 }
 
 __device__ __forceinline__ uint32_t key_of(float f) { return (uint32_t)float_to_ordered(f) ^ 0x80000000u; }
-__device__ __forceinline__ float value_of(unsigned long long packed) {
-  return ordered_to_float((int32_t)((uint32_t)(packed >> 32) ^ 0x80000000u));
-}
 __device__ __forceinline__ unsigned long long pack(float f, uint32_t pos) { return ((unsigned long long)key_of(f) << 32) | pos; }
 
 __device__ __forceinline__ void block_reduce_ext(unsigned long long& lo, unsigned long long& hi) {
@@ -260,10 +258,12 @@
   int nLayer;
 };
 
-constexpr int kPhTileW = 128, kPhTileH = 32, kPhThreadsX = 32, kPhThreadsY = 4, kPhRows = 8;
+constexpr int kPhTileW = 120, kPhTileH = 40, kPhThreadsX = 30, kPhThreadsY = 5, kPhRows = 8;
 constexpr int kPhBoxW = kPhTileW + 8, kPhBoxH = kPhTileH + 3;
 constexpr uint32_t kPhBoxBytes = kPhBoxW * kPhBoxH * sizeof(float);
 constexpr int kPhBufFloats = (kPhBoxW * kPhBoxH + 31) / 32 * 32;
+static_assert(kPhTileW == 4 * kPhThreadsX && kPhTileH == kPhRows * kPhThreadsY, "register blocks tile the CTA's tile");
+static_assert(2 * kPhBufFloats * sizeof(float) + 16 <= 48 * 1024, "two input boxes fit the static shared memory");
 
 __device__ __forceinline__ const CUtensorMap* layer_map(const AtmPhaseParams& p, int l) {
   switch (l) {
@@ -290,7 +290,7 @@
     const float v[12] = {a.x, a.y, a.z, a.w, b.x, b.y, b.z, b.w, c.x, c.y, c.z, c.w};
 #pragma unroll
     for (int k = 0; k < 4; ++k)
-      h[t][k] = wc0 * v[MIS + k] + wc1 * v[MIS + k + 1] + wc2 * v[MIS + k + 2] + wc3 * v[MIS + k + 3];
+      h[t][k] = atm_tap4(wc0, wc1, wc2, wc3, v[MIS + k], v[MIS + k + 1], v[MIS + k + 2], v[MIS + k + 3]);
   }
 }
 
@@ -325,8 +325,8 @@
       tma::mbar_expect_tx(&bar[buf ^ 1], kPhBoxBytes);
       tma::load_3d(layer_map(p, l + 1), &bar[buf ^ 1], &tile[buf ^ 1][0], (p.col0[l + 1] + j0) & ~3, p.row0[l + 1] + i0, b);
     }
-    const float lo = value_of(__ldg(&p.ext[l][2 * b + 0]));
-    const float hi = value_of(__ldg(&p.ext[l][2 * b + 1]));
+    const float lo = atm_extremum(__ldg(&p.ext[l][2 * b + 0]));
+    const float hi = atm_extremum(__ldg(&p.ext[l][2 * b + 1]));
     const float wc0 = p.wcol[l][0], wc1 = p.wcol[l][1], wc2 = p.wcol[l][2], wc3 = p.wcol[l][3];
     const float wr0 = p.wrow[l][0], wr1 = p.wrow[l][1], wr2 = p.wrow[l][2], wr3 = p.wrow[l][3];
     const float w = p.weight[l];
@@ -343,9 +343,8 @@
     for (int t = 0; t < kPhRows; ++t)
 #pragma unroll
       for (int c = 0; c < 4; ++c) {
-        float v = wr0 * h[t][c] + wr1 * h[t + 1][c] + wr2 * h[t + 2][c] + wr3 * h[t + 3][c];
-        v = fminf(fmaxf(v, lo), hi);
-        acc[t][c] += w * v;
+        const float v = atm_tap4(wr0, wr1, wr2, wr3, h[t][c], h[t + 1][c], h[t + 2][c], h[t + 3][c]);
+        acc[t][c] = atm_accumulate(acc[t][c], v, lo, hi, w);
       }
     __syncthreads();
   }
diff --git a/rlao_b200/csrc/atm_interp.cuh b/rlao_b200/csrc/atm_interp.cuh
--- /dev/null
+++ b/rlao_b200/csrc/atm_interp.cuh
@@ -0,0 +1,40 @@
+#pragma once
+#include "common.cuh"
+
+namespace aoenv {
+
+__device__ __forceinline__ float atm_tap4(float w0, float w1, float w2, float w3, float v0, float v1, float v2, float v3) {
+  return fmaf(w3, v3, fmaf(w2, v2, fmaf(w0, v0, w1 * v1)));
+}
+__device__ __forceinline__ float2 atm_tap4(float w0, float w1, float w2, float w3, float2 v0, float2 v1, float2 v2, float2 v3) {
+  return fma2(dup2(w3), v3, fma2(dup2(w2), v2, fma2(dup2(w0), v0, mul2(dup2(w1), v1))));
+}
+
+__device__ __forceinline__ float atm_accumulate(float acc, float v, float lo, float hi, float w) {
+  return fmaf(w, fminf(fmaxf(v, lo), hi), acc);
+}
+__device__ __forceinline__ float2 atm_accumulate(float2 acc, float2 v, float lo, float hi, float w) {
+  return fma2(dup2(w), make_float2(fminf(fmaxf(v.x, lo), hi), fminf(fmaxf(v.y, lo), hi)), acc);
+}
+
+__device__ __forceinline__ float atm_extremum(unsigned long long packed) {
+  return ordered_to_float((int32_t)((uint32_t)(packed >> 32) ^ 0x80000000u));
+}
+
+struct AtmInPlace {
+  const float* win[AOENV_MAX_LAYERS];
+  const unsigned long long* ext[AOENV_MAX_LAYERS];
+  float wrow[AOENV_MAX_LAYERS][4];
+  float wcol[AOENV_MAX_LAYERS][4];
+  float weight[AOENV_MAX_LAYERS];
+  long long env_stride;
+  int pitch, nLayer;
+  float opd_scale;
+  float* out;
+};
+
+int shwfs_frame_atm(const AtmInPlace& atm, const aoenv_dm_sep_t* dm, const float* pupil, const float* amp,
+                    const uint8_t* valid, int B, int nS, int n, float phase_scale, const aoenv_detector_t* det,
+                    float* frame, int32_t* envmax, double* stats, void* stream);
+
+}
diff --git a/rlao_b200/csrc/step.cu b/rlao_b200/csrc/step.cu
--- a/rlao_b200/csrc/step.cu
+++ b/rlao_b200/csrc/step.cu
@@ -1,6 +1,7 @@
 #include <math.h>
 #include <string.h>
 
+#include "atm_interp.cuh"
 #include "common.cuh"
 
 using namespace aoenv;
@@ -131,6 +132,7 @@
   const int L = st.nLayer;
   AOENV_CHECK_ARG(L >= 1 && L <= AOENV_MAX_LAYERS && st.group_max >= 1, "atm_update: %d layers", L);
   AOENV_CHECK_ARG(!st.use_tc || w_planes != nullptr, "atm_update: the operator planes are missing");
+  AOENV_CHECK_ARG(!st.phase.pending, "atm_update: the sub-pixel shift of the previous frame is still pending");
   constexpr int kMaxSteps = 64;
   static thread_local Step plans[AOENV_MAX_LAYERS][kMaxSteps];
   int count[AOENV_MAX_LAYERS], rounds = 0;
@@ -153,21 +155,65 @@
       if (rc) return rc;
     }
   }
+  aoenv_atm_phase_t& ph = st.phase;
+  for (int i = 0; i < L; ++i) {
+    const aoenv_layer_state_t& ly = st.layer[i];
+    ph.canvas[i] = st.maps[i][ly.cur];
+    ph.org[2 * i] = ly.org[0];
+    ph.org[2 * i + 1] = ly.org[1];
+    tap_weights(ly.buff[0], st.warp_kernel, &ph.col_off[i], &ph.wcol[4 * i]);
+    tap_weights(ly.buff[1], st.warp_kernel, &ph.row_off[i], &ph.wrow[4 * i]);
+  }
+  ph.out = opd_out;
+  ph.pending = 1;
+  return st.defer_phase ? 0 : aoenv_atm_resolve(&st, stream);
+}
+
+int aoenv_atm_resolve(aoenv_atm_state_t* state, void* stream) {
+  AOENV_CHECK_ARG(state != nullptr, "atm_resolve: null state");
+  aoenv_atm_state_t& st = *state;
+  aoenv_atm_phase_t& ph = st.phase;
+  if (!ph.pending) return 0;
+  ph.pending = 0;
   const float* canv[AOENV_MAX_LAYERS];
   const uint64_t* exts[AOENV_MAX_LAYERS];
-  int32_t org[2 * AOENV_MAX_LAYERS], roff[AOENV_MAX_LAYERS], coff[AOENV_MAX_LAYERS];
-  float wr[4 * AOENV_MAX_LAYERS], wc[4 * AOENV_MAX_LAYERS];
-  for (int i = 0; i < L; ++i) {
-    const aoenv_layer_state_t& ly = st.layer[i];
-    canv[i] = (const float*)st.maps[i][ly.cur];
+  for (int i = 0; i < st.nLayer; ++i) {
+    canv[i] = (const float*)ph.canvas[i];
     exts[i] = (const uint64_t*)st.ext[i];
-    org[2 * i] = ly.org[0];
-    org[2 * i + 1] = ly.org[1];
-    tap_weights(ly.buff[0], st.warp_kernel, &coff[i], &wc[4 * i]);
-    tap_weights(ly.buff[1], st.warp_kernel, &roff[i], &wr[4 * i]);
-  }
-  return aoenv_atm_phase(canv, exts, org, L, st.B, st.R, st.M, st.Mc, st.pitch, st.fp_off, roff, coff, wr, wc, st.weight,
-                         st.opd_scale, opd_out, stream);
+  }
+  return aoenv_atm_phase(canv, exts, ph.org, st.nLayer, st.B, st.R, st.M, st.Mc, st.pitch, st.fp_off, ph.row_off, ph.col_off,
+                         ph.wrow, ph.wcol, st.weight, st.opd_scale, (float*)ph.out, stream);
+}
+
+}
+
+namespace {
+
+int in_place_params(const aoenv_atm_state_t& st, AtmInPlace& p) {
+  const aoenv_atm_phase_t& ph = st.phase;
+  const int R = st.R, M = st.M;
+  AOENV_CHECK_ARG(st.nLayer >= 1 && st.nLayer <= AOENV_MAX_LAYERS && st.pitch >= st.Mc && st.Mc >= M, "sh_step: bad atmosphere state");
+  p = AtmInPlace{};
+  for (int l = 0; l < st.nLayer; ++l) {
+    const int oy = ph.org[2 * l], ox = ph.org[2 * l + 1];
+    AOENV_CHECK_ARG(oy >= 0 && ox >= 0 && oy + M <= st.Mc && ox + M <= st.pitch, "sh_step: window of layer %d leaves the canvas", l);
+    const int lo_r = st.fp_off + ph.row_off[l], hi_r = st.fp_off + R - 1 + ph.row_off[l] + 3;
+    const int lo_c = st.fp_off + ph.col_off[l], hi_c = st.fp_off + R - 1 + ph.col_off[l] + 3;
+    AOENV_CHECK_ARG(lo_r >= 0 && lo_c >= 0 && hi_r < M && hi_c < M, "sh_step: taps of layer %d leave the map", l);
+    p.win[l] = (const float*)ph.canvas[l] + ((size_t)(oy + lo_r) * st.pitch + (ox + lo_c));
+    p.ext[l] = (const unsigned long long*)st.ext[l];
+    for (int k = 0; k < 4; ++k) {
+      p.wrow[l][k] = ph.wrow[4 * l + k];
+      p.wcol[l][k] = ph.wcol[4 * l + k];
+    }
+    p.weight[l] = st.weight[l];
+  }
+  p.env_stride = st.env_stride;
+  p.pitch = st.pitch;
+  p.nLayer = st.nLayer;
+  p.opd_scale = st.opd_scale;
+  p.out = (float*)ph.out;
+  return 0;
 }
 
 }
@@ -184,9 +230,25 @@
   if (parts & 1) {
     aoenv_dm_sep_t dm = c->dm;
     dm.rows = dm_rows_cur;
-    rc = aoenv_shwfs_frame_dm(opd_a, nullptr, &dm, (const int32_t*)c->order, (const float*)c->pupil, (const float*)c->amp,
-                              (const uint8_t*)c->valid, c->B, c->nS, c->n, c->phase_scale, det, 0, (float*)c->frame,
-                              (int32_t*)c->envmax, (double*)c->stats, stream);
+    aoenv_atm_state_t* atm = c->atm;
+    if (atm != nullptr && atm->phase.pending) {
+      AOENV_CHECK_ARG(atm->phase.out == opd_a, "sh_step: the pending atmosphere frame belongs to another OPD buffer");
+      AOENV_CHECK_ARG(atm->B == c->B && atm->R == c->nS * c->n, "sh_step: atmosphere of another shape");
+    }
+    if (atm != nullptr && atm->phase.pending && c->n == 6) {
+      AtmInPlace p;
+      rc = in_place_params(*atm, p);
+      if (rc) return rc;
+      atm->phase.pending = 0;
+      rc = shwfs_frame_atm(p, &dm, (const float*)c->pupil, (const float*)c->amp, (const uint8_t*)c->valid, c->B, c->nS, c->n,
+                           c->phase_scale, det, (float*)c->frame, (int32_t*)c->envmax, (double*)c->stats, stream);
+    } else {
+      if (atm != nullptr) rc = aoenv_atm_resolve(atm, stream);
+      if (rc) return rc;
+      rc = aoenv_shwfs_frame_dm(opd_a, nullptr, &dm, (const int32_t*)c->order, (const float*)c->pupil, (const float*)c->amp,
+                                (const uint8_t*)c->valid, c->B, c->nS, c->n, c->phase_scale, det, 0, (float*)c->frame,
+                                (int32_t*)c->envmax, (double*)c->stats, stream);
+    }
     if (rc) return rc;
     rc = aoenv_shwfs_slopes((const float*)c->frame, (const int32_t*)c->envmax, 0, (const int32_t*)c->valid_idx, c->nV,
                             (const float*)c->ref_xy, c->inv_units, c->threshold_cog, c->B, c->nS, c->n, (float*)c->slopes, c->lds,
diff --git a/rlao_b200/csrc/wfs.cu b/rlao_b200/csrc/wfs.cu
--- a/rlao_b200/csrc/wfs.cu
+++ b/rlao_b200/csrc/wfs.cu
@@ -1,6 +1,7 @@
 #include <stdlib.h>
 #include <mutex>
 
+#include "atm_interp.cuh"
 #include "common.cuh"
 #include "wfs_twiddles.inc"
 
@@ -258,23 +259,150 @@
   }
 }
 
-template <int n, int WL = 0>
-__global__ void __launch_bounds__(128)
+constexpr int frame_threads(int ty, int tx) { return ty > 0 ? ty * tx : 128; }
+constexpr int frame_min_ctas(int ty, int tx) { return ty > 0 ? 384 / (ty * tx) : 0; }
+template <int n, int WL = 0, int TY = 0, int TX = 0>
+__global__ void __launch_bounds__(frame_threads(TY, TX), frame_min_ctas(TY, TX))
 shwfs_frame_kernel(const float* __restrict__ opd_a, const float* __restrict__ opd_b, const float* __restrict__ pupil,
                    const float* __restrict__ amp, const uint8_t* __restrict__ valid, int nS, float phase_scale,
                    int track_max, int shared_max, float* __restrict__ frame,
                    int32_t* __restrict__ envmax, double* __restrict__ stats, const __grid_constant__ aoenv_dm_sep_t dm,
-                   const int32_t* __restrict__ order) {
+                   const int32_t* __restrict__ order, const __grid_constant__ AtmInPlace atm) {
   constexpr int N = 2 * n;
+  constexpr bool kAtm = TY > 0;
   pdl_enter();
   const int R = nS * n;
   const int b = blockIdx.y;
-  const int k0 = blockIdx.x * blockDim.x + threadIdx.x;
-  const bool active = k0 < nS * nS;
-  const int k = (active && order != nullptr) ? __ldg(&order[k0]) : k0;
+  int k, ty0 = 0, tx0 = 0;
+  bool active;
+  if constexpr (!kAtm) {
+    const int k0 = blockIdx.x * blockDim.x + threadIdx.x;
+    active = k0 < nS * nS;
+    k = (active && order != nullptr) ? __ldg(&order[k0]) : k0;
+  } else {
+    constexpr int kT = TY * TX, kW = kT / 32;
+    static_assert(kT % 32 == 0, "whole warps per tile");
+    __shared__ int s_perm[kT], s_cnt[2][kW];
+    const int tiles_x = (nS + TX - 1) / TX;
+    ty0 = (blockIdx.x / tiles_x) * TY;
+    tx0 = (blockIdx.x % tiles_x) * TX;
+    const int t = threadIdx.x, w = t >> 5, lane = t & 31;
+    const int gi = ty0 + t / TX, gj = tx0 + t % TX;
+    const bool in = gi < nS && gj < nS;
+    const bool lt = in && valid[gi * nS + gj] != 0;
+    const unsigned m_lit = __ballot_sync(0xffffffffu, lt), m_in = __ballot_sync(0xffffffffu, in);
+    if (lane == 0) { s_cnt[0][w] = __popc(m_lit); s_cnt[1][w] = __popc(m_in); }
+    __syncthreads();
+    int p_lit = 0, p_in = 0, n_lit = 0, n_in = 0;
+#pragma unroll
+    for (int v = 0; v < kW; ++v) {
+      if (v < w) { p_lit += s_cnt[0][v]; p_in += s_cnt[1][v]; }
+      n_lit += s_cnt[0][v];
+      n_in += s_cnt[1][v];
+    }
+    const unsigned below = (1u << lane) - 1u;
+    const int rank = lt ? p_lit + __popc(m_lit & below)
+                        : in ? n_lit + (p_in - p_lit) + __popc(m_in & ~m_lit & below)
+                             : n_in + (32 * w - p_in) + __popc(~m_in & below);
+    s_perm[rank] = t;
+    __syncthreads();
+    const int slot = s_perm[t];
+    const int li_ = ty0 + slot / TX, lj_ = tx0 + slot % TX;
+    active = li_ < nS && lj_ < nS;
+    k = li_ * nS + lj_;
+  }
   const int li = active ? k / nS : 0, lj = active ? k % nS : 0;
   const bool lit = active && valid[k] != 0;
   const float phase_turns = phase_scale * 0.15915494309189535f;
+
+  constexpr int IH = TY * n + 3, IW = TX * n + 3, OW = TX * n;
+  __shared__ __align__(16) float s_in[kAtm ? IH * IW : 1];
+  float ka_in_place = 0.f;
+  const float* s_opd = s_in;
+  if constexpr (kAtm) {
+    constexpr int kT = TY * TX;
+    __shared__ float s_ka;
+    float2 opd2[n][n / 2];
+    const int i0 = ty0 * n, j0 = tx0 * n;
+    const int rows = min(IH, R + 3 - i0), cols = min(IW, R + 3 - j0);
+    const int lr = (li - ty0) * n, lc = (lj - tx0) * n;
+    if (stats != nullptr && threadIdx.x == 0) {
+      float acc = 0.f;
+      for (int l = 0; l < atm.nLayer; ++l) {
+        const float* __restrict__ p0 = atm.win[l] + (size_t)b * atm.env_stride + (size_t)(R / 2) * atm.pitch + R / 2;
+        float h[4];
+#pragma unroll
+        for (int t = 0; t < 4; ++t) {
+          const float* __restrict__ q = p0 + (size_t)t * atm.pitch;
+          h[t] = atm_tap4(atm.wcol[l][0], atm.wcol[l][1], atm.wcol[l][2], atm.wcol[l][3], __ldg(q), __ldg(q + 1), __ldg(q + 2), __ldg(q + 3));
+        }
+        const float v = atm_tap4(atm.wrow[l][0], atm.wrow[l][1], atm.wrow[l][2], atm.wrow[l][3], h[0], h[1], h[2], h[3]);
+        acc = atm_accumulate(acc, v, atm_extremum(__ldg(&atm.ext[l][2 * b])), atm_extremum(__ldg(&atm.ext[l][2 * b + 1])),
+                             atm.weight[l]);
+      }
+      s_ka = acc * atm.opd_scale;
+    }
+#pragma unroll
+    for (int r = 0; r < n; ++r)
+#pragma unroll
+      for (int c2 = 0; c2 < n / 2; ++c2) opd2[r][c2] = make_float2(0.f, 0.f);
+    constexpr int kLd = (IH * IW + kT - 1) / kT;
+    float ld[kLd];
+    auto load_layer = [&](int l) {
+      const float* __restrict__ src = atm.win[l] + (size_t)b * atm.env_stride + (size_t)i0 * atm.pitch + j0;
+#pragma unroll
+      for (int u = 0; u < kLd; ++u) {
+        const int e = threadIdx.x + u * kT, r = e / IW, c = e - r * IW;
+        ld[u] = (e < IH * IW && r < rows && c < cols) ? __ldg(src + (size_t)r * atm.pitch + c) : 0.f;
+      }
+    };
+    load_layer(0);
+    for (int l = 0; l < atm.nLayer; ++l) {
+#pragma unroll
+      for (int u = 0; u < kLd; ++u)
+        if (threadIdx.x + u * kT < IH * IW) s_in[threadIdx.x + u * kT] = ld[u];
+      if (l + 1 < atm.nLayer) load_layer(l + 1);
+      const float lo = atm_extremum(__ldg(&atm.ext[l][2 * b])), hi = atm_extremum(__ldg(&atm.ext[l][2 * b + 1]));
+      const float wc0 = atm.wcol[l][0], wc1 = atm.wcol[l][1], wc2 = atm.wcol[l][2], wc3 = atm.wcol[l][3];
+      const float wr0 = atm.wrow[l][0], wr1 = atm.wrow[l][1], wr2 = atm.wrow[l][2], wr3 = atm.wrow[l][3];
+      const float wl = atm.weight[l];
+      __syncthreads();
+      if (active) {
+        float2 h[n + 3][n / 2];
+#pragma unroll
+        for (int t = 0; t < n + 3; ++t) {
+          const float* __restrict__ q = s_in + (lr + t) * IW + lc;
+          float v[n + 3];
+#pragma unroll
+          for (int c = 0; c < n + 3; ++c) v[c] = q[c];
+#pragma unroll
+          for (int c2 = 0; c2 < n / 2; ++c2)
+            h[t][c2] = make_float2(atm_tap4(wc0, wc1, wc2, wc3, v[2 * c2], v[2 * c2 + 1], v[2 * c2 + 2], v[2 * c2 + 3]),
+                                   atm_tap4(wc0, wc1, wc2, wc3, v[2 * c2 + 1], v[2 * c2 + 2], v[2 * c2 + 3], v[2 * c2 + 4]));
+        }
+#pragma unroll
+        for (int r = 0; r < n; ++r)
+#pragma unroll
+          for (int c2 = 0; c2 < n / 2; ++c2)
+            opd2[r][c2] = atm_accumulate(opd2[r][c2], atm_tap4(wr0, wr1, wr2, wr3, h[r][c2], h[r + 1][c2], h[r + 2][c2], h[r + 3][c2]),
+                                         lo, hi, wl);
+      }
+      __syncthreads();
+    }
+    if (active) {
+      float* __restrict__ o = atm.out + (size_t)b * R * R + (size_t)(li * n) * R + lj * n;
+#pragma unroll
+      for (int r = 0; r < n; ++r)
+#pragma unroll
+        for (int c2 = 0; c2 < n / 2; ++c2) {
+          const float2 v = mul2(opd2[r][c2], dup2(atm.opd_scale));
+          *reinterpret_cast<float2*>(o + (size_t)r * R + 2 * c2) = v;
+          *reinterpret_cast<float2*>(s_in + (lr + r) * OW + lc + 2 * c2) = v;
+        }
+    }
+    if (stats != nullptr) ka_in_place = s_ka;
+    s_opd = s_in + lr * OW + lc;
+  }
 
   float2 er2[n][n / 2], ei2[n][n / 2];
   float f0 = 0.f, f1 = 0.f, f2 = 0.f, f3 = 0.f;
@@ -283,7 +411,7 @@
     const float* __restrict__ pa = opd_a + (size_t)b * R * R + tile;
     const float* __restrict__ pb = (WL == 0 && opd_b) ? opd_b + (size_t)b * R * R + tile : nullptr;
     const size_t centre = (size_t)b * R * R + (size_t)(R / 2) * R + R / 2;
-    const float ka = stats ? __ldg(opd_a + centre) : 0.f;
+    const float ka = stats ? (kAtm ? ka_in_place : __ldg(opd_a + centre)) : 0.f;
     const float kt = stats ? (pb ? ka + __ldg(opd_b + centre) : ka) : 0.f;
     float2 dmv[WL > 0 ? n : 1][n / 2];
     if (WL > 0) {
@@ -322,7 +450,7 @@
 #pragma unroll
       for (int a2 = 0; a2 < n / 2; ++a2) {
         const int o2 = bb * R + 2 * a2;
-        const float2 av = __ldg(reinterpret_cast<const float2*>(pa + o2));
+        const float2 av = kAtm ? *reinterpret_cast<const float2*>(s_opd + bb * OW + 2 * a2) : __ldg(reinterpret_cast<const float2*>(pa + o2));
         const float2 bv = WL > 0 ? dmv[WL > 0 ? bb : 0][a2]
                                  : (pb ? __ldg(reinterpret_cast<const float2*>(pb + o2)) : make_float2(0.f, 0.f));
         const float2 pv = __ldg(reinterpret_cast<const float2*>(pupil + tile + o2));
@@ -1051,6 +1179,7 @@
 using namespace aoenv;
 
 constexpr int kDefaultFrameVariant = 0;
+constexpr int kAtmTile = 8;
 static std::atomic<int> g_wfs6_factorised{[] {
   const char* e = getenv("AOENV_WFS_FRAME");
   if (e && e[0] == 'f') return 1;
@@ -1068,8 +1197,9 @@
 static int shwfs_frame_impl(const float* opd_a, const float* opd_b, const aoenv_dm_sep_t* dm_in, const int32_t* order, const float* pupil,
                             const float* amp, const uint8_t* valid, int B, int nS, int n, float phase_scale,
                             const aoenv_detector_t* det, int shared_max, float* frame, int32_t* envmax, double* stats,
-                            void* stream) {
+                            void* stream, const AtmInPlace* atm = nullptr) {
   AOENV_CHECK_ARG(B > 0 && B <= 65535 && nS > 0, "shwfs_frame: bad shape B=%d nS=%d", B, nS);
+  const AtmInPlace noatm{};
   aoenv_dm_sep_t dm{};
   if (dm_in != nullptr) {
     dm = *dm_in;
@@ -1102,25 +1232,33 @@
   case NN:                                                                                                   \
     if (dm.WL == 14)                                                                                         \
       AOENV_LAUNCH((shwfs_frame_kernel<NN, 14>), grid, 128, 0, s, opd_a, opd_b, pupil, amp, valid, nS, phase_scale, \
-                   (int)(det == nullptr), shared_max, frame, envmax, stats, dm, order);                             \
+                   (int)(det == nullptr), shared_max, frame, envmax, stats, dm, order, noatm);                             \
     else if (dm.WL == 18)                                                                                    \
       AOENV_LAUNCH((shwfs_frame_kernel<NN, 18>), grid, 128, 0, s, opd_a, opd_b, pupil, amp, valid, nS, phase_scale, \
-                   (int)(det == nullptr), shared_max, frame, envmax, stats, dm, order);                             \
+                   (int)(det == nullptr), shared_max, frame, envmax, stats, dm, order, noatm);                             \
     else                                                                                                     \
       AOENV_LAUNCH((shwfs_frame_kernel<NN, 0>), grid, 128, 0, s, opd_a, opd_b, pupil, amp, valid, nS, phase_scale,  \
-                   (int)(det == nullptr), shared_max, frame, envmax, stats, dm, order);                             \
+                   (int)(det == nullptr), shared_max, frame, envmax, stats, dm, order, noatm);                             \
     break;
   switch (n) {
     AOENV_WFS_CASE(4)
     AOENV_WFS_CASE(8)
     case 6:
-      if (dm.WL != 0) {
+      if (atm != nullptr) {
+        dim3 ga(((nS + kAtmTile - 1) / kAtmTile) * ((nS + kAtmTile - 1) / kAtmTile), B);
+        if (dm.WL == 14)
+          AOENV_LAUNCH((shwfs_frame_kernel<6, 14, kAtmTile, kAtmTile>), ga, kAtmTile * kAtmTile, 0, s, atm->out, opd_b, pupil, amp,
+                       valid, nS, phase_scale, (int)(det == nullptr), shared_max, frame, envmax, stats, dm, order, *atm);
+        else
+          AOENV_LAUNCH((shwfs_frame_kernel<6, 18, kAtmTile, kAtmTile>), ga, kAtmTile * kAtmTile, 0, s, atm->out, opd_b, pupil, amp,
+                       valid, nS, phase_scale, (int)(det == nullptr), shared_max, frame, envmax, stats, dm, order, *atm);
+      } else if (dm.WL != 0) {
         if (dm.WL == 14) {
           AOENV_LAUNCH((shwfs_frame_kernel<6, 14>), grid, 128, 0, s, opd_a, opd_b, pupil, amp, valid, nS, phase_scale,
-                       (int)(det == nullptr), shared_max, frame, envmax, stats, dm, order);
+                       (int)(det == nullptr), shared_max, frame, envmax, stats, dm, order, noatm);
         } else
           AOENV_LAUNCH((shwfs_frame_kernel<6, 18>), grid, 128, 0, s, opd_a, opd_b, pupil, amp, valid, nS, phase_scale,
-                       (int)(det == nullptr), shared_max, frame, envmax, stats, dm, order);
+                       (int)(det == nullptr), shared_max, frame, envmax, stats, dm, order, noatm);
       } else if (variant == 2) {
         dim3 g3((nS * nS + kS6Warps * kS6Lenslets - 1) / (kS6Warps * kS6Lenslets), B);
         shwfs_frame6s_kernel<<<g3, kS6Warps * 32, 0, s>>>(opd_a, opd_b, pupil, amp, valid, nS, phase_scale, det == nullptr,
@@ -1130,7 +1268,7 @@
                                                  frame, envmax, stats);
       else
         AOENV_LAUNCH((shwfs_frame_kernel<6, 0>), grid, 128, 0, s, opd_a, opd_b, pupil, amp, valid, nS, phase_scale,
-                     (int)(det == nullptr), shared_max, frame, envmax, stats, dm, order);
+                     (int)(det == nullptr), shared_max, frame, envmax, stats, dm, order, noatm);
       break;
   }
 #undef AOENV_WFS_CASE
@@ -1144,6 +1282,21 @@
   }
   return 0;
 }
+
+}
+
+namespace aoenv {
+int shwfs_frame_atm(const AtmInPlace& atm, const aoenv_dm_sep_t* dm, const float* pupil, const float* amp,
+                    const uint8_t* valid, int B, int nS, int n, float phase_scale, const aoenv_detector_t* det,
+                    float* frame, int32_t* envmax, double* stats, void* stream) {
+  AOENV_CHECK_ARG(n == 6 && dm != nullptr && (dm->WL == 14 || dm->WL == 18), "shwfs_frame_atm: n = 6 with the separable DM only");
+  AOENV_CHECK_ARG(atm.nLayer >= 1 && atm.nLayer <= AOENV_MAX_LAYERS && atm.out != nullptr, "shwfs_frame_atm: bad atmosphere");
+  return shwfs_frame_impl(nullptr, nullptr, dm, nullptr, pupil, amp, valid, B, nS, n, phase_scale, det, 0, frame, envmax, stats,
+                          stream, &atm);
+}
+}
+
+extern "C" {
 
 int aoenv_shwfs_frame(const float* opd_a, const float* opd_b, const float* pupil, const float* amp,
                       const uint8_t* valid, int B, int nS, int n, float phase_scale, const aoenv_detector_t* det,
```
